# wusize/CLIPSelf

Measured on AMD Instinct MI355X. Metric: images/sec (student+teacher distill step), ViT-B/16 32 crops/img, higher is better.
Workload: dtype bf16; 1 GPU; EVA02-CLIP-B-16 CLIPSelf image-patches step, 64 images x 32 crops per GPU, 224^2 (BASELINE configs[1]); global_batch=64, crops_per_image=32, image_size=224, parallelism=dp1, teacher_chunk=2048, teacher_last_block=cls_query_only, teacher_schedule=one_batch_ahead_on_side_stream

## Files before the change

### clipself_amd/csrc/attention.hip

```cpp
#include <type_traits>
#include "cs_common.h"
#include <cstdlib>

namespace {

constexpr int HD = 64;
constexpr float LOG2E = 1.4426950408889634f;


#define Z16 (f32x16{0.f, 0.f, 0.f, 0.f, 0.f, 0.f, 0.f, 0.f, 0.f, 0.f, 0.f, 0.f, 0.f, 0.f, 0.f, 0.f})
__device__ __forceinline__ f32x16 zero16() {
    f32x16 z;
#pragma unroll
    for (int e = 0; e < 16; ++e) z[e] = 0.f;
    return z;
}

__device__ __forceinline__ void rope8(U128& v, const float* __restrict__ cs, const float* __restrict__ sn) {
    const float4 c0 = *(const float4*)cs, c1 = *(const float4*)(cs + 4);
    const float4 s0 = *(const float4*)sn, s1 = *(const float4*)(sn + 4);
    const float c[8] = {c0.x, c0.y, c0.z, c0.w, c1.x, c1.y, c1.z, c1.w};
    const float s[8] = {s0.x, s0.y, s0.z, s0.w, s1.x, s1.y, s1.z, s1.w};
#pragma unroll
    for (int j = 0; j < 4; ++j) {
// ... 89 lines not shown
__device__ __forceinline__ void stage_rows(const __bf16* __restrict__ src, size_t rowbase, int ld, int coloff, int tok0, int Ntok,
                                           const float* cos_t, const float* sin_t, char* tile, __bf16* tile_t, int ldt, int tid) {
    for (int idx = tid; idx < CHK * 8; idx += 512) {
        const int r = idx >> 3, c = idx & 7, tok = tok0 + r;
        U128 v;
        if (tok < Ntok) {
            v.u = *(const uint4*)(src + (rowbase + tok) * ld + coloff + c * 8);
            if (ROPE && tok > 0) rope8(v, cos_t + (size_t)(tok - 1) * HD + c * 8, sin_t + (size_t)(tok - 1) * HD + c * 8);
        } else {
            v.u = make_uint4(0, 0, 0, 0);
        }
        if (tile) *(uint4*)(tile + r * 128 + ((c ^ (r & 7)) << 4)) = v.u;
        if (WITH_T) {
#pragma unroll
            for (int e = 0; e < 8; ++e) tile_t[(c * 8 + e) * ldt + r] = v.e[e];
        }
    }
}

__device__ __forceinline__ bf16x8 lds_frag(const char* tile, int row, int ks, int hf) {
    return *(const bf16x8*)(tile + row * 128 + ((((ks << 1) + hf) ^ (row & 7)) << 4));
}

constexpr int VT_LD = 264;

__device__ __forceinline__ int k_off(int r, int c) { return ((r >> 1) << 8) + (((((r & 1) << 3) | c) ^ ((r >> 1) & 15)) << 4); }

typedef short s16x4v __attribute__((ext_vector_type(4)));

__device__ __forceinline__ int tr_lane_off(int rr, int d0, int lane) {
    const int li = lane & 15, g1 = (lane >> 4) & 1;
    const int col = d0 + 16 * g1 + 4 * (li & 3);
    return k_off(rr + (li >> 2), col >> 3) + ((col >> 2) & 1) * 8;
}
__device__ __forceinline__ bf16x8 tr_join2(s16x4v lo, s16x4v hi) {
    typedef short s16x8v __attribute__((ext_vector_type(8)));
    const s16x8v v = __builtin_shufflevector(lo, hi, 0, 1, 2, 3, 4, 5, 6, 7);
    return __builtin_bit_cast(bf16x8, v);
}
__device__ __forceinline__ s16x4v tr_read4(const char* addr) {
    return __builtin_amdgcn_ds_read_tr16_b64_v4i16((__attribute__((address_space(3))) s16x4v*)addr);
}

template <int CHK, int NT = 512>
struct RowRegs {
    static constexpr int ITEMS = (CHK * 8 + NT - 1) / NT;
    uint4 v[ITEMS];
    __device__ __forceinline__ void load(const __bf16* __restrict__ src, size_t rowbase, int ld, int coloff, int tok0, int Ntok, int tid) {
#pragma unroll
        for (int it = 0; it < ITEMS; ++it) {
            const int idx = min(tid + it * NT, CHK * 8 - 1), tok = min(tok0 + (idx >> 3), Ntok - 1);
            v[it] = *(const uint4*)(src + (rowbase + tok) * ld + coloff + (idx & 7) * 8);
        }
    }
    template <bool ROPE, bool ZPAD = false>
    __device__ __forceinline__ void store(char* tile, const float* rt, int g, float inv_g, int tok0, int Ntok, int tid) {
#pragma unroll
        for (int it = 0; it < ITEMS; ++it) {
            const int idx = tid + it * NT, r = idx >> 3, c = idx & 7, tok = tok0 + r;
            if (idx < CHK * 8) {
                U128 t;
                t.u = v[it];
                if (ROPE && tok > 0 && tok < Ntok) rope8_lds(t, rt, g, inv_g, tok, c);
                if (ZPAD && tok >= Ntok) t.u = make_uint4(0, 0, 0, 0);
                *(uint4*)(tile + k_off(r, c)) = t.u;
            }
        }
    }
};

__device__ __forceinline__ bf16x8 pack8_swapped(const f32x16& a, int c2) {
    union { bf16x2 h; unsigned u; } x0, x1, y0, y1;
    x0.h[0] = f2bf(a[c2 * 8 + 0]); x0.h[1] = f2bf(a[c2 * 8 + 1]);
    x1.h[0] = f2bf(a[c2 * 8 + 2]); x1.h[1] = f2bf(a[c2 * 8 + 3]);
    y0.h[0] = f2bf(a[c2 * 8 + 4]); y0.h[1] = f2bf(a[c2 * 8 + 5]);
    y1.h[0] = f2bf(a[c2 * 8 + 6]); y1.h[1] = f2bf(a[c2 * 8 + 7]);
    const auto r0 = __builtin_amdgcn_permlane32_swap(x0.u, y0.u, false, false);
    const auto r1 = __builtin_amdgcn_permlane32_swap(x1.u, y1.u, false, false);
    union { unsigned u[4]; bf16x8 v; } out;
    out.u[0] = r0[0]; out.u[1] = r1[0]; out.u[2] = r0[1]; out.u[3] = r1[1];
    return out.v;
}

__device__ __forceinline__ void load_q_frags(const AttnArgs& p, const float* rt, size_t rowbase, int qc, int h, int hf, bf16x8 (&qf)[4]) {
    U128 t[4];
#pragma unroll
    for (int ks = 0; ks < 4; ++ks) t[ks].u = *(const uint4*)(p.qkv + (rowbase + qc) * p.ldqkv + h * HD + ks * 16 + hf * 8);
#pragma unroll
    for (int ks = 0; ks < 4; ++ks) {
        if (qc > 0) rope8_lds(t[ks], rt, p.grid, p.inv_grid, qc, ks * 2 + hf);
        qf[ks] = t[ks].h;
    }
}

template <int CH, bool TAIL, bool VROW = false>
__device__ __forceinline__ void attend_chunk(const char* Kl, const __bf16* Vt, const bf16x8 (&qf)[4], int key0, int Ntok, float sl2,
                                             int lane, bool first, float& m, float& l, f32x16 (&o)[2], int t0 = 0) {
    const int hf = lane >> 5, l31 = lane & 31;
    const int k_base = (l31 >> 1) << 8, par8 = (l31 & 1) << 3, sw = l31 >> 1;
    f32x16 s[CH];
#pragma unroll
    for (int t = 0; t < CH; ++t) {
        s[t] = zero16();
#pragma unroll
        for (int ks = 0; ks < 4; ++ks) {
            const bf16x8 kfrag = *(const bf16x8*)(Kl + (t0 + t) * (16 * 256) + k_base + (((par8 | (ks * 2 + hf)) ^ sw) << 4));
            s[t] = __builtin_amdgcn_mfma_f32_32x32x16_bf16(kfrag, qf[ks], s[t], 0, 0, 0);
        }
    }
    const int rem_last = Ntok - key0 - (CH - 1) * 32;
    const bool short_tail = TAIL && rem_last <= 8;
    float mx = -INFINITY;
#pragma unroll
    for (int t = 0; t < CH; ++t) {
        if (TAIL && t == CH - 1 && short_tail) {
#pragma unroll
            for (int e = 0; e < 4; ++e) {
                if (e + 4 * hf >= rem_last) s[t][e] = -INFINITY;
                mx = fmaxf(mx, s[t][e]);
            }
            continue;
        }
        if ((!TAIL || t == CH - 1) && key0 + t * 32 + 32 > Ntok) {
#pragma unroll
            for (int e = 0; e < 16; ++e)
                if (key0 + t * 32 + mfma32_row(e, lane) >= Ntok) s[t][e] = -INFINITY;
        }
#pragma unroll
        for (int e = 0; e < 16; ++e) mx = fmaxf(mx, s[t][e]);
    }
    mx = fmaxf(mx, __shfl_xor(mx, 32, 64));
    const float m_new = fmaxf(m, mx);
    const float alpha = exp2f((m - m_new) * sl2);
    const float msc = m_new * sl2;
    float rs = 0.f;
#pragma unroll
    for (int t = 0; t < CH; ++t) {
        if (TAIL && t == CH - 1 && short_tail) {
#pragma unroll
            for (int e = 0; e < 4; ++e) {
                const float pv = __builtin_amdgcn_exp2f(s[t][e] * sl2 - msc);
                s[t][e] = pv;
                rs += pv;
            }
#pragma unroll
            for (int e = 4; e < 8; ++e) s[t][e] = 0.f;
            continue;
        }
#pragma unroll
        for (int e = 0; e < 16; ++e) {
            const float pv = __builtin_amdgcn_exp2f(s[t][e] * sl2 - msc);
            s[t][e] = pv;
            rs += pv;
        }
    }
    rs += __shfl_xor(rs, 32, 64);
    l = l * alpha + rs;
    m = m_new;
    if (!first) {
#pragma unroll
        for (int e = 0; e < 16; ++e) { o[0][e] *= alpha; o[1][e] *= alpha; }
    }
#pragma unroll
    for (int t = 0; t < CH; ++t)
#pragma unroll
        for (int c2 = 0; c2 < 2; ++c2) {
            if (TAIL && t == CH - 1 && c2 == 1 && rem_last <= 16) continue;
            const bf16x8 pb = pack8_swapped(s[t], c2);
            const int kb = (t0 + t) * 4 + c2 * 2 + hf;
#pragma unroll
            for (int dt = 0; dt < 2; ++dt) {
                bf16x8 vfrag;
                if constexpr (VROW) {
                    const char* Vl = (const char*)Vt + (t0 + t) * (16 * 256);
                    vfrag = tr_join2(tr_read4(Vl + tr_lane_off(c2 * 16 + 8 * hf, dt * 32, lane)), tr_read4(Vl + tr_lane_off(c2 * 16 + 8 * hf + 4, dt * 32, lane)));
                } else {
                    const int d = dt * 32 + l31;
                    vfrag = *(const bf16x8*)(Vt + d * VT_LD + ((kb ^ ((d >> 3) & 7)) << 3));
                }
                o[dt] = __builtin_amdgcn_mfma_f32_32x32x16_bf16(vfrag, pb, o[dt], 0, 0, 0);
            }
        }
}

__device__ __forceinline__ void store_o(const AttnArgs& p, size_t rowbase, int q, int h, int bh, int hf, float m, float l, const f32x16 (&o)[2]) {
    const float inv = 1.f / l;
    __bf16* orow = p.out + (rowbase + q) * p.ldo + h * HD;
    float ps = 0.f, pq = 0.f;
#pragma unroll
    for (int dt = 0; dt < 2; ++dt) {
        U64 t[4];
#pragma unroll
        for (int g4 = 0; g4 < 4; ++g4)
#pragma unroll
            for (int i = 0; i < 4; ++i) {
                t[g4].e[i] = f2bf(o[dt][g4 * 4 + i] * inv);
                const float r = bf2f(t[g4].e[i]);
                ps += r;
                pq += r * r;
            }
#pragma unroll
        for (int a = 0; a < 4; a += 2) {
            const auto r0 = __builtin_amdgcn_permlane32_swap(t[a].u.x, t[a + 1].u.x, false, false);
            const auto r1 = __builtin_amdgcn_permlane32_swap(t[a].u.y, t[a + 1].u.y, false, false);
            if (!ATT_ABL(p, 4)) *(uint4*)(orow + dt * 32 + (a + hf) * 8) = make_uint4(r0[0], r1[0], r0[1], r1[1]);
        }
    }
    if (p.lse_out && hf == 0) p.lse_out[(size_t)bh * p.Ntok + q] = m * p.scale + logf(l);
    if (p.stats_part) {
        ps += __shfl_xor(ps, 32);
        pq += __shfl_xor(pq, 32);
        if (hf == 0) *(float2*)(p.stats_part + ((size_t)h * p.Mtot + rowbase + q) * 2) = make_float2(ps, pq);
    }
}

template <int CH, int CH1>
__global__ __launch_bounds__(512, 2) void attn_fwd2_kernel(AttnArgs p) {
    constexpr int CHK = CH * 32;
    extern __shared__ __attribute__((aligned(16))) char smem[];
    char* Kl = smem;
    char* Vl = smem + CHK * 128;
    float* rt = (float*)(smem + 2 * CHK * 128);

    const int tid = threadIdx.x, lane = tid & 63, wave = tid >> 6, hf = lane >> 5, l31 = lane & 31;
    const RowBlock rb = map_block(p, 8);
    const int bh = rb.bh, b = bh / p.H, h = bh - b * p.H;
    const int C = p.H * HD;
    const size_t rowbase = (size_t)b * p.Ntok;
    const float sl2 = p.scale * LOG2E;
    const int q0 = (rb.tile0 + wave) * 32, q = q0 + l31, qc = min(q, p.Ntok - 1);
    const bool active = wave < rb.nt && q0 < p.Ntok;
    RowRegs<CHK> kr, vr;
    kr.load(p.qkv, rowbase, p.ldqkv, C + h * HD, 0, p.Ntok, tid);
    vr.load(p.qkv, rowbase, p.ldqkv, 2 * C + h * HD, 0, p.Ntok, tid);
    load_rope_tables<512>(rt, p.cos_t, p.sin_t, p.grid, tid);
    __syncthreads();
    bf16x8 qf[4];
    load_q_frags(p, rt, rowbase, qc, h, hf, qf);
    float m = -INFINITY, l = 0.f;
    f32x16 o[2] = {zero16(), zero16()};
    for (int key0 = 0; key0 < p.Ntok; key0 += CHK) {
        if (key0) __syncthreads();
        kr.template store<true>(Kl, rt, p.grid, p.inv_grid, key0, p.Ntok, tid);
        vr.template store<false>(Vl, rt, p.grid, p.inv_grid, key0, p.Ntok, tid);
        __syncthreads();
        if (key0 + CHK < p.Ntok) {
            kr.load(p.qkv, rowbase, p.ldqkv, C + h * HD, key0 + CHK, p.Ntok, tid);
            vr.load(p.qkv, rowbase, p.ldqkv, 2 * C + h * HD, key0 + CHK, p.Ntok, tid);
        }
        if (!active) continue;
        attend_chunk<CH1, false, true>(Kl, (const __bf16*)Vl, qf, key0, p.Ntok, sl2, lane, key0 == 0, m, l, o, 0);
        if (key0 + CH1 * 32 < p.Ntok)
            attend_chunk<CH - CH1, false, true>(Kl, (const __bf16*)Vl, qf, key0 + CH1 * 32, p.Ntok, sl2, lane, false, m, l, o, CH1);
    }
    if (active && q < p.Ntok) store_o(p, rowbase, q, h, bh, hf, m, l, o);
}

template <bool TAIL>
__global__ __launch_bounds__(512, 4) void attn_fwd8_kernel(AttnArgs p) {
    constexpr int CH = 7, CHK = CH * 32, NT = 512;
    extern __shared__ __attribute__((aligned(16))) char smem[];
    char* Kl = smem;
    __bf16* Vt = (__bf16*)(smem + CHK * 128);
    float* rt = (float*)(smem + CHK * 128 + HD * VT_LD * 2);
    const int tid = threadIdx.x, lane = tid & 63, wave = tid >> 6, hf = lane >> 5, l31 = lane & 31;
    const int bh = blockIdx.y, b = bh / p.H, h = bh - b * p.H;
    const int C = p.H * HD;
    const size_t rowbase = (size_t)b * p.Ntok;
    const float sl2 = p.scale * LOG2E;
    const int last = p.Ntok - 1;
    float tab[4];
    {
        const int i = min(tid, p.grid * 32 - 1), r = i >> 5, d = i & 31;
        tab[0] = p.cos_t[(size_t)(r * p.grid) * HD + d];
        tab[1] = p.sin_t[(size_t)(r * p.grid) * HD + d];
        tab[2] = p.cos_t[(size_t)r * HD + 32 + d];
        tab[3] = p.sin_t[(size_t)r * HD + 32 + d];
    }
    __builtin_amdgcn_sched_barrier(0);
    constexpr int KI = (CHK * 8 + NT - 1) / NT;
    U128 kr[KI], vin[8], qraw[4];
    const __bf16* kbase = p.qkv + C + h * HD;
    const __bf16* vbase = p.qkv + 2 * C + h * HD;
    const int vkb = min(tid, CHK - 1) >> 3, vc = tid & 7;
#pragma unroll
    for (int it = 0; it < KI; ++it) {
        const int idx = min(tid + it * NT, CHK * 8 - 1), tok = min(idx >> 3, last);
        kr[it].u = *(const uint4*)(kbase + (rowbase + tok) * p.ldqkv + (idx & 7) * 8);
    }
#pragma unroll
    for (int i = 0; i < 8; ++i) {
        const int tok = min(vkb * 8 + i, last);
        vin[i].u = *(const uint4*)(vbase + (rowbase + tok) * p.ldqkv + vc * 8);
    }
    const int q0 = wave * 32, q = q0 + l31, qc = min(q, last);
#pragma unroll
    for (int ks = 0; ks < 4; ++ks) qraw[ks].u = *(const uint4*)(p.qkv + (rowbase + qc) * p.ldqkv + h * HD + ks * 16 + hf * 8);
    if (tid < p.grid * 32) {
        rt[tid] = tab[0];
        rt[(p.grid << 5) + tid] = tab[1];
        rt[(2 * p.grid << 5) + tid] = tab[2];
        rt[(3 * p.grid << 5) + tid] = tab[3];
    }
    __syncthreads();
#pragma unroll
    for (int it = 0; it < KI; ++it) {
        const int idx = tid + it * NT, r = idx >> 3, c = idx & 7;
        if (idx < CHK * 8) {
            if (r > 0 && r < p.Ntok && !ATT_ABL(p, 2)) rope8_lds(kr[it], rt, p.grid, p.inv_grid, r, c);
            *(uint4*)(Kl + k_off(r, c)) = kr[it].u;
        }
    }
    if (tid < CHK) {
        const int pos = (vkb ^ vc) * 8;
#pragma unroll
        for (int j = 0; j < 8; ++j) {
            U128 o;
#pragma unroll
            for (int i = 0; i < 8; ++i) o.e[i] = vin[i].e[j];
            *(uint4*)(Vt + (vc * 8 + j) * VT_LD + pos) = o.u;
        }
    }
    __syncthreads();
    if (q0 >= p.Ntok) return;
    bf16x8 qf[4];
#pragma unroll
    for (int ks = 0; ks < 4; ++ks) {
        if (qc > 0 && !ATT_ABL(p, 2)) rope8_lds(qraw[ks], rt, p.grid, p.inv_grid, qc, ks * 2 + hf);
        qf[ks] = qraw[ks].h;
    }
    float m = -INFINITY, l = 0.f;
    f32x16 o[2] = {zero16(), zero16()};
    if (ATT_ABL(p, 1)) { l = 1.f; m = 0.f; o[0][0] = bf2f(qf[0][0]); }
    else if (TAIL) {
        attend_chunk<3, false>(Kl, Vt, qf, 0, p.Ntok, sl2, lane, true, m, l, o, 0);
        attend_chunk<3, false>(Kl, Vt, qf, 96, p.Ntok, sl2, lane, false, m, l, o, 3);
        attend_chunk<1, true>(Kl, Vt, qf, 192, p.Ntok, sl2, lane, false, m, l, o, 6);
    } else {
        attend_chunk<3, false>(Kl, Vt, qf, 0, p.Ntok, sl2, lane, true, m, l, o, 0);
        if (p.Ntok > 96) attend_chunk<3, false>(Kl, Vt, qf, 96, p.Ntok, sl2, lane, false, m, l, o, 3);
        if (p.Ntok > 192) attend_chunk<1, false>(Kl, Vt, qf, 192, p.Ntok, sl2, lane, false, m, l, o, 6);
    }
    if (q < p.Ntok) store_o(p, rowbase, q, h, bh, hf, m, l, o);
}

__global__ __launch_bounds__(256) void attn_bwd_prep_kernel(const __bf16* __restrict__ o, const __bf16* __restrict__ dout, float* __restrict__ dsum,
                                                            int B, int Ntok, int H, int ldo) {
    const long idx = (long)blockIdx.x * blockDim.x + threadIdx.x;
    const long total = (long)B * Ntok * H * 8;
    float s = 0.f;
    long row = 0; int h = 0;
    const bool ok = idx < total;
    if (ok) {
        const int c = (int)(idx & 7);
        h = (int)((idx >> 3) % H);
        row = (idx >> 3) / H;
        U128 a, g;
        a.u = *(const uint4*)(o + row * ldo + h * HD + c * 8);
        g.u = *(const uint4*)(dout + row * ldo + h * HD + c * 8);
#pragma unroll
        for (int e = 0; e < 8; ++e) s += bf2f(a.e[e]) * bf2f(g.e[e]);
    }
    s += __shfl_xor(s, 1, 64);
    s += __shfl_xor(s, 2, 64);
    s += __shfl_xor(s, 4, 64);
    if (ok && (idx & 7) == 0) {
        const long b = row / Ntok, n = row - b * Ntok;
        dsum[((size_t)b * H + h) * Ntok + n] = s;
    }
}

__global__ __launch_bounds__(256) void rope_qk_kernel(const __bf16* __restrict__ qkv, const float* __restrict__ cos_t, const float* __restrict__ sin_t,
                                                      __bf16* __restrict__ out, long rows, int Ntok, int C, int ldqkv) {
    const long idx = (long)blockIdx.x * blockDim.x + threadIdx.x;
    const int cpr = C >> 2;
    if (idx >= rows * cpr) return;
    const long row = idx / cpr;
    const int c = (int)(idx - row * cpr), col = c * 8, tok = (int)(row % Ntok);
    U128 v;
    v.u = *(const uint4*)(qkv + row * ldqkv + col);
    if (tok > 0) rope8(v, cos_t + (size_t)(tok - 1) * HD + (col & 63), sin_t + (size_t)(tok - 1) * HD + (col & 63));
    *(uint4*)(out + row * (2 * C) + col) = v.u;
}

__device__ __forceinline__ void store_grad_tile(const f32x16 (&g)[2], __bf16* dst, bool rope, const float* cs, const float* sn, int hf) {
#pragma unroll
    for (int dt = 0; dt < 2; ++dt)
#pragma unroll
        for (int g4 = 0; g4 < 4; ++g4) {
            const int d = dt * 32 + g4 * 8 + hf * 4;
            float v[4] = {g[dt][g4 * 4], g[dt][g4 * 4 + 1], g[dt][g4 * 4 + 2], g[dt][g4 * 4 + 3]};
            if (rope) {
                const float4 c = *(const float4*)(cs + d), s = *(const float4*)(sn + d);
                const float a0 = __builtin_fmaf(v[0], c.x, v[1] * s.y), a1 = __builtin_fmaf(v[1], c.y, -(v[0] * s.x));
                const float a2 = __builtin_fmaf(v[2], c.z, v[3] * s.w), a3 = __builtin_fmaf(v[3], c.w, -(v[2] * s.z));
                v[0] = a0; v[1] = a1; v[2] = a2; v[3] = a3;
            }
            U64 t;
#pragma unroll
            for (int i = 0; i < 4; ++i) t.e[i] = f2bf(v[i]);
            *(uint2*)(dst + d) = t.u;
        }
}

template <int CH>
__global__ __launch_bounds__(512) void attn_bwd_dq_kernel(AttnArgs p) {
    constexpr int CHK = CH * 32, VLD = CHK + 4;
    extern __shared__ __attribute__((aligned(16))) char smem[];
    char* Kl = smem;
    char* Vl = smem + CHK * 128;
    __bf16* Kt = (__bf16*)(smem + 2 * CHK * 128);
// ... 412 lines not shown
#pragma unroll
        for (int j = 0; j < 8; ++j) qf[h][j] = bf2f(t.e[j]);
    }
    const float sl2 = scale * LOG2E;
    for (int key = kg; key < Ntok; key += 32) {
        U128 kk[HG];
#pragma unroll
        for (int h = 0; h < HG; ++h) kk[h].u = *(const uint4*)(kbase + (size_t)key * ldkv + h * HD);
        if (key > 0 && cos_t) {
            const float* cs = cos_t + (size_t)(key - 1) * HD + c * 8;
            const float* sn = sin_t + (size_t)(key - 1) * HD + c * 8;
#pragma unroll
            for (int h = 0; h < HG; ++h) rope8(kk[h], cs, sn);
        }
#pragma unroll
        for (int h = 0; h < HG; ++h) {
            float dot = 0.f;
#pragma unroll
            for (int j = 0; j < 8; ++j) dot += qf[h][j] * bf2f(kk[h].e[j]);
            dot += __shfl_xor(dot, 1);
            dot += __shfl_xor(dot, 2);
            dot += __shfl_xor(dot, 4);
            if (c == 0) sm[h * Npad + key] = (arow && !arow[key]) ? -INFINITY : dot * sl2;
        }
    }
    __syncthreads();
    for (int h = wave; h < HG; h += 4) {
        float* row = sm + h * Npad;
        float mx = -INFINITY;
        for (int key = lane; key < Ntok; key += 64) mx = fmaxf(mx, row[key]);
        mx = wave_max(mx);
        if (mx == -INFINITY) mx = 0.f;
        float sum = 0.f;
        for (int key = lane; key < Ntok; key += 64) {
            const float e = __builtin_amdgcn_exp2f(row[key] - mx);
            sum += e;
            row[key] = bf2f(f2bf(e));
        }
        sum = wave_sum(sum);
        if (lane == 0) rsum[h] = sum > 0.f ? sum : 1.f;
    }
    __syncthreads();
    float acc[HG][8];
#pragma unroll
    for (int h = 0; h < HG; ++h)
#pragma unroll
        for (int j = 0; j < 8; ++j) acc[h][j] = 0.f;
    for (int key = kg; key < Ntok; key += 32) {
        U128 vv[HG];
#pragma unroll
        for (int h = 0; h < HG; ++h) vv[h].u = *(const uint4*)(vbase + (size_t)key * ldkv + h * HD);
#pragma unroll
        for (int h = 0; h < HG; ++h) {
            const float pk = sm[h * Npad + key];
#pragma unroll
            for (int j = 0; j < 8; ++j) acc[h][j] += pk * bf2f(vv[h].e[j]);
        }
    }
#pragma unroll
    for (int h = 0; h < HG; ++h)
#pragma unroll
        for (int j = 0; j < 8; ++j) {
            float v = acc[h][j];
            v += __shfl_xor(v, 8);
            v += __shfl_xor(v, 16);
            v += __shfl_xor(v, 32);
            if (lane < 8) part[wave * (HG * HD) + h * HD + c * 8 + j] = v;
        }
    __syncthreads();
    for (int o = tid; o < HG * HD; o += 256) {
        const float v = (part[o] + part[HG * HD + o]) + (part[2 * HG * HD + o] + part[3 * HG * HD + o]);
        out[(size_t)b * ldo + h0 * HD + o] = f2bf(v / rsum[o / HD]);
    }
}

}

static int attn_fwd_impl(const void* qkv, const float* cos_t, const float* sin_t, void* out, float* lse, float* stats_part, int B, int Ntok,
                         int H, int ldqkv, int ldo, float scale, hipStream_t stream) {
    if (check_common("cs_attn_fwd", B, Ntok, H, ldqkv, ldo)) return -1;
    AttnArgs a{};
    a.qkv = (const __bf16*)qkv; a.cos_t = cos_t; a.sin_t = sin_t; a.out = (__bf16*)out; a.lse_out = lse;
    a.stats_part = stats_part; a.Mtot = (long)B * Ntok;
    int g = (int)(sqrtf((float)(Ntok - 1)) + 0.5f);
    CS_CHECK_ARG(g * g == Ntok - 1, "cs_attn_fwd: Ntok - 1 = %d is not a square token grid (the RoPE tables are read separably)", Ntok - 1);
    a.grid = g; a.inv_grid = 1.f / (float)g;
#ifdef CS_ABLATION_SWITCHES
    static const int dbg_env = getenv("CS_ATTN_DBG") ? atoi(getenv("CS_ATTN_DBG")) : 0;
    a.dbg = dbg_env;
#else
    a.dbg = 0;
#endif
    a.Ntok = Ntok; a.H = H; a.ldqkv = ldqkv; a.ldo = ldo; a.scale = scale;
    constexpr int CH = 7;
    const size_t lds = (size_t)CH * 32 * 128 + (size_t)HD * VT_LD * 2 + (size_t)4 * g * 32 * sizeof(float);
    CS_CHECK_ARG(lds <= 160 * 1024, "cs_attn_fwd: token grid %d too large for the LDS RoPE tables", g);
    if (Ntok <= CH * 32) {
        static bool once = (set_lds(attn_fwd8_kernel<false>, 160 * 1024), set_lds(attn_fwd8_kernel<true>, 160 * 1024), true);
        (void)once;
        if (Ntok > (CH - 1) * 32) hipLaunchKernelGGL((attn_fwd8_kernel<true>), dim3(1, B * H), dim3(512), lds, stream, a);
        else hipLaunchKernelGGL((attn_fwd8_kernel<false>), dim3(1, B * H), dim3(512), lds, stream, a);
    } else {
        static bool once = (set_lds(attn_fwd2_kernel<CH, 4>, 160 * 1024), true);
        (void)once;
        const size_t lds2 = (size_t)2 * CH * 32 * 128 + (size_t)4 * g * 32 * sizeof(float);
        dim3 grid2;
        set_schedule(a, B, Ntok, H, grid2);
        hipLaunchKernelGGL((attn_fwd2_kernel<CH, 4>), grid2, dim3(512), lds2, stream, a);
    }
    CS_LAUNCH_CHECK();
    return 0;
}

extern "C" int cs_attn_fwd(const void* qkv, const float* cos_t, const float* sin_t, void* out, float* lse, int B, int Ntok, int H,
                           int ldqkv, int ldo, float scale, hipStream_t stream) {
    return attn_fwd_impl(qkv, cos_t, sin_t, out, lse, nullptr, B, Ntok, H, ldqkv, ldo, scale, stream);
}

extern "C" int cs_attn_fwd_stats(const void* qkv, const float* cos_t, const float* sin_t, void* out, float* lse, float* stats_part, int B,
                                 int Ntok, int H, int ldqkv, int ldo, float scale, hipStream_t stream) {
    CS_CHECK_ARG(stats_part != nullptr && ((uintptr_t)stats_part % 8) == 0, "cs_attn_fwd_stats: stats_part must be an 8-byte aligned buffer");
    return attn_fwd_impl(qkv, cos_t, sin_t, out, lse, stats_part, B, Ntok, H, ldqkv, ldo, scale, stream);
}

static size_t bwd_dsum_bytes(int B, int Ntok, int H) { return (((size_t)B * H * Ntok * sizeof(float)) + 255) & ~(size_t)255; }
extern "C" size_t cs_attn_bwd_workspace(int B, int Ntok, int H) {
    return bwd_dsum_bytes(B, Ntok, H) + (Ntok > 7 * 32 ? (size_t)B * Ntok * 2 * H * HD * sizeof(__bf16) : 0);
}

extern "C" int cs_attn_bwd(const void* qkv, const void* o, const void* dout, const float* lse, const float* cos_t, const float* sin_t,
                           void* dqkv, void* workspace, int B, int Ntok, int H, int ldqkv, int ldo, float scale, hipStream_t stream) {
    if (check_common("cs_attn_bwd", B, Ntok, H, ldqkv, ldo)) return -1;
    CS_CHECK_ARG(workspace != nullptr && lse != nullptr, "cs_attn_bwd: workspace and lse are required");
    float* dsum = (float*)workspace;
    const long total = (long)B * Ntok * H * 8;
    hipLaunchKernelGGL(attn_bwd_prep_kernel, dim3((int)((total + 255) / 256)), dim3(256), 0, stream, (const __bf16*)o, (const __bf16*)dout, dsum, B, Ntok, H, ldo);
    CS_LAUNCH_CHECK();
    AttnArgs a{};
    a.qkv = (const __bf16*)qkv; a.dout = (const __bf16*)dout; a.cos_t = cos_t; a.sin_t = sin_t; a.lse_in = lse; a.dsum = dsum;
    a.out = (__bf16*)dqkv; a.Ntok = Ntok; a.H = H; a.ldqkv = ldqkv; a.ldo = ldo; a.scale = scale;
    dim3 grid((Ntok + 255) / 256, B * H), block(512);
    constexpr int CH = 7;
    constexpr int CHK = CH * 32, VLD = CHK + 4;
    const int g = (int)(sqrtf((float)(Ntok - 1)) + 0.5f);
    const bool v1 = getenv("CS_ATTN_BWD_V1") != nullptr || g * g != Ntok - 1;
    if (!v1) {
        a.grid = g; a.inv_grid = 1.f / (float)g;
        const size_t rope = (size_t)4 * g * 32 * sizeof(float);
        const size_t lds_dq = (size_t)2 * CHK * 128 + rope, lds_dkv = (size_t)2 * CHK * 128 + (size_t)2 * CHK * sizeof(float) + rope;
        CS_CHECK_ARG(lds_dkv <= 160 * 1024, "cs_attn_bwd: token grid %d too large for the LDS RoPE tables", g);
        static bool once = (set_lds(attn_bwd_dq2_kernel<CH, true>, 160 * 1024), set_lds(attn_bwd_dkv2_kernel<CH, true>, 160 * 1024),
                            set_lds(attn_bwd_dq2_kernel<CH, false, true>, 160 * 1024), set_lds(attn_bwd_dkv2_kernel<CH, false, true>, 160 * 1024), true);
        (void)once;
        if (Ntok <= CHK) {
            hipLaunchKernelGGL((attn_bwd_dq2_kernel<CH, true>), grid, block, lds_dq, stream, a);
            CS_LAUNCH_CHECK();
            hipLaunchKernelGGL((attn_bwd_dkv2_kernel<CH, true>), grid, block, lds_dkv, stream, a);
        } else {
            dim3 grid2;
            set_schedule(a, B, Ntok, H, grid2);
            const int C2 = 2 * H * HD;
            __bf16* qk = (__bf16*)((char*)workspace + bwd_dsum_bytes(B, Ntok, H));
            const long items = (long)B * Ntok * (C2 / 8);
            hipLaunchKernelGGL(rope_qk_kernel, dim3((unsigned)((items + 255) / 256)), dim3(256), 0, stream, (const __bf16*)qkv, cos_t, sin_t, qk,
                               (long)B * Ntok, Ntok, H * HD, ldqkv);
            CS_LAUNCH_CHECK();
            a.qk = qk; a.ldqk = C2;
            hipLaunchKernelGGL((attn_bwd_dq2_kernel<CH, false, true>), grid2, block, lds_dq - rope, stream, a);
            CS_LAUNCH_CHECK();
            hipLaunchKernelGGL((attn_bwd_dkv2_kernel<CH, false, true>), grid2, block, lds_dkv - rope, stream, a);
        }
        CS_LAUNCH_CHECK();
        return 0;
    }
    const size_t lds_dq = (size_t)2 * CHK * 128 + (size_t)HD * VLD * 2;
    const size_t lds_dkv = (size_t)2 * CHK * 128 + (size_t)2 * HD * VLD * 2 + (size_t)2 * CHK * sizeof(float);
    static bool once = (set_lds(attn_bwd_dq_kernel<CH>, lds_dq), set_lds(attn_bwd_dkv_kernel<CH>, lds_dkv), true);
    (void)once;
    hipLaunchKernelGGL((attn_bwd_dq_kernel<CH>), grid, block, lds_dq, stream, a);
    CS_LAUNCH_CHECK();
    hipLaunchKernelGGL((attn_bwd_dkv_kernel<CH>), grid, block, lds_dkv, stream, a);
    CS_LAUNCH_CHECK();
    return 0;
}

static int attn_cls_launch(const void* q, const void* kv, const float* cos_t, const float* sin_t, void* out, int rows, int Ntok, int H,
                           int ldq, int ldkv, int ldo, float scale, int qpb, const unsigned char* allow, hipStream_t stream) {
    const int HG = H % 6 == 0 ? 6 : (H % 4 == 0 ? 4 : (H % 3 == 0 ? 3 : (H % 2 == 0 ? 2 : 1)));
    const size_t lds = ((size_t)HG * ((Ntok + 3) & ~3) + 8 + (size_t)4 * HG * HD) * sizeof(float);
    CS_CHECK_ARG(lds <= 160 * 1024, "cs_attn_cls_fwd: Ntok=%d too large", Ntok);
    const dim3 grid(rows, H / HG), block(256);
// ... 39 lines not shown
```

### clipself_amd/csrc/gemm.hip

```cpp
#include "gemm_common.h"
#include <hip/amd_detail/amd_hip_unsafe_atomics.h>

namespace {

constexpr int EP_LD = 68;
constexpr int EP_BYTES = 32 * EP_LD * 4;

template <int FM, int BN>
__device__ __forceinline__ void epilogue_swiglu(const GemmArgs& p, const f32x16 (&acc)[FM][2], char* slab_bytes, char* rowst_bytes, int lane,
                                                int row0, int tn, int wn) {
    const int l31 = lane & 31, hf = lane >> 5;
    uint32_t* slab = (uint32_t*)slab_bytes;
    const int hbase = tn * (BN / 2) + wn * 32;
    const int hl = hbase + l31;
    float b1 = 0.f, b2 = 0.f;
    if (p.bias && hl < p.group) { b1 = p.bias[hl]; b2 = p.bias[p.group + hl]; }
    const bool ln = p.ln_mean != nullptr;
    float c1 = 0.f, c2 = 0.f;
    float2* rowst = (float2*)rowst_bytes;
    if (ln) {
        if (hl < p.group) { c1 = p.ln_colsum[hl]; c2 = p.ln_colsum[p.group + hl]; }
        for (int r = lane; r < FM * 32; r += 64) {
            const int row = min(row0 + r, p.M - 1);
            const float rs = p.ln_rstd[row];
// ... 551 lines not shown
    double c1, c2, c3;
    const int sp[4] = {0, best_split(128, 128, 2, 1.3, c1), best_split(256, 128, 1, 0.95, c2), best_split(256, 256, 1, 1.4, c3)};
    int cfg = force_cfg;
    if (cfg == 0) {
        if (a.M < 256 || ncols < 256) c3 = 1e30;
        if (a.M < 256 || ncols < 128) c2 = 1e30;
        cfg = (c3 <= c2 && c3 <= c1) ? 3 : (c2 <= c1 ? 2 : 1);
        if (cfg == 3 && use_glds) cfg = 11;
    }
    if (cfg != 1 && cfg != 2 && cfg != 3 && cfg != 7 && cfg != 9 && cfg != 11) {
        cs_set_error("cs_gemm_nt: schedule %d does not exist (flags bits 4-7: 0 heuristic, 1, 2, 3, 7, 9, 11)", cfg);
        return -1;
    }
    const int ns = sp[cfg >= 7 ? 3 : cfg];
    a.ktiles_per_split = (ktiles + ns - 1) / ns;
    if (cfg == 11) {
        if (use_glds && ns == 1) {
            const int rc = cs_gemm_stream_launch(a, EPI, a.reserve, stream);
            if (rc <= 0) return rc;
        }
        cfg = 9;
    }
    switch (cfg) {
        case 9:
            if constexpr (epi_is_bf16(EPI) || EPI == EPI_SWIGLU_BF16 || EPI == EPI_RESID_F32 || EPI == EPI_RESID_LN_F32) {
                if (use_glds && ns == 1) return launch_persist<EPI>(a, stream);
            }
            return launch_cfg<EPI, 256, 256, 2, 4, 32>(a, ns, use_glds, stream);
        case 7: return launch_cfg<EPI, 256, 256, 2, 4, 32>(a, ns, use_glds, stream);
        case 3: return launch_cfg<EPI, 256, 256, 2, 4, 2>(a, ns, use_glds, stream);
        case 2: return launch_cfg<EPI, 256, 128, 4, 2, 2>(a, ns, use_glds, stream);
        default: return launch_cfg<EPI, 128, 128, 2, 2, 2>(a, ns, use_glds, stream);
    }
}

}

static int gemm_nt_impl(const void* A, const void* B, void* C, const float* bias, const float* extra, const float* ln_mean,
                        const float* ln_rstd, const float* ln_colsum, float* stats_part, void* xb_out, int ldxb, int M, int N, int K, int lda,
                        int ldb, int ldc, int epi, int splits, int group, int flags, hipStream_t stream) {
    CS_CHECK_ARG(M > 0 && N > 0 && K > 0, "cs_gemm_nt: empty problem M=%d N=%d K=%d", M, N, K);
    CS_CHECK_ARG(K % BK == 0, "cs_gemm_nt: K=%d must be a multiple of %d", K, BK);
    CS_CHECK_ARG((lda % 8) == 0 && (ldb % 8) == 0, "cs_gemm_nt: lda/ldb must be multiples of 8 (16-byte rows)");
    CS_CHECK_ARG(((uintptr_t)A % 16) == 0 && ((uintptr_t)B % 16) == 0, "cs_gemm_nt: operands must be 16-byte aligned");
    CS_CHECK_ARG(splits == 1 || epi == EPI_ATOMIC_F32, "cs_gemm_nt: split-K (splits != 1; <= 0 = automatic) needs the atomic epilogue");
    CS_CHECK_ARG((epi == EPI_SWIGLU_BF16 ? group : N) % 4 == 0 && ldc % 4 == 0 && ((uintptr_t)C % 16) == 0,
                 "cs_gemm_nt: N, ldc must be multiples of 4 and C 16-byte aligned (vector epilogue)");
    CS_CHECK_ARG(bias == nullptr || ((uintptr_t)bias % 16) == 0, "cs_gemm_nt: bias must be 16-byte aligned");
    GemmArgs a;
    a.A = (const __bf16*)A; a.B = (const __bf16*)B; a.C = C; a.bias = bias; a.extra = extra;
    a.M = M; a.N = N; a.K = K; a.lda = lda; a.ldb = ldb; a.ldc = ldc; a.group = group;
    a.split_stride = 0;
    a.ln_mean = ln_mean; a.ln_rstd = ln_rstd; a.ln_colsum = ln_colsum; a.stats_part = stats_part;
    a.xb_out = (__bf16*)xb_out; a.ldxb = ldxb;
    a.tiles_m = a.tiles_n = 0;
    a.gm = ((flags >> 8) & 15) ? ((flags >> 8) & 15) : 8;
    a.rm = (flags >> 16) & 3;
    a.nsplit = 1;
    if (a.rm == 1 || a.rm == 2) {
        const int f = (flags >> 8) & 15;
        CS_CHECK_ARG(f == 0 || f == 1 || f == 2 || f == 4 || f == 8, "cs_gemm_nt: B-stationary raster needs 1, 2, 4 or 8 N parts (got %d)", f);
        int parts = f;
        if (parts == 0) for (parts = 1; parts < 8 && (double)N * K * 2 / parts > 3.3e6; parts *= 2) {}
        a.nsplit = parts;
        a.gm = 8;
    }
    if (epi == EPI_SWIGLU_BF16) CS_CHECK_ARG(group > 0 && N == 2 * group, "cs_gemm_nt: swiglu epilogue needs N == 2*group");
    if (epi == EPI_RESID_LN_F32) CS_CHECK_ARG(ln_mean && ln_rstd && ln_colsum && ((uintptr_t)ln_colsum % 16) == 0, "cs_gemm_nt_ln: epilogue 6 needs mean, rstd and a 16-byte aligned column-sum vector");
    CS_CHECK_ARG(stats_part == nullptr || epi == EPI_SWIGLU_BF16 || epi == EPI_RESID_F32 || epi == EPI_RESID_LN_F32,
                 "cs_gemm_nt_ln: statistics output exists for the SwiGLU and residual epilogues");
    CS_CHECK_ARG(xb_out == nullptr || ((epi == EPI_RESID_F32 || epi == EPI_RESID_LN_F32) && ldxb % 4 == 0 && ((uintptr_t)xb_out % 8) == 0),
                 "cs_gemm_nt_ln: the bf16 copy exists for the residual epilogues (8-byte aligned, ldxb %% 4 == 0)");
    CS_CHECK_ARG((ln_mean == nullptr) == (ln_rstd == nullptr) && (ln_mean == nullptr || ln_colsum != nullptr),
                 "cs_gemm_nt_ln: mean, rstd and the column-sum vector come together");
    CS_CHECK_ARG(ln_mean == nullptr || epi_is_bf16(epi) || epi == EPI_SWIGLU_BF16 || epi == EPI_RESID_LN_F32,
                 "cs_gemm_nt_ln: a folded LayerNorm exists for epilogues 0, 3, 6, 7 and 8");
    if (epi == EPI_PATCH_F32 || epi == EPI_RESID_F32 || epi == EPI_RESID_LN_F32) CS_CHECK_ARG(extra != nullptr && ((uintptr_t)extra % 16) == 0, "cs_gemm_nt: epilogue %d needs 16-byte aligned extra", epi);
    if (epi == EPI_PATCH_F32) CS_CHECK_ARG(group > 0, "cs_gemm_nt: patch epilogue needs group");
    a.ktiles_per_split = K / BK;
    const int glds = (flags & 1) ? 0 : 1;
    const int force = (flags >> 4) & 15;
    a.dbg = (flags >> 12) & 15;
    a.reserve = (flags >> 20) & 255;
    switch (epi) {
        case EPI_BF16: return launch<EPI_BF16>(a, splits, glds, force, stream);
        case EPI_F32: return launch<EPI_F32>(a, splits, glds, force, stream);
        case EPI_RESID_F32: return launch<EPI_RESID_F32>(a, splits, glds, force, stream);
        case EPI_SWIGLU_BF16: return launch<EPI_SWIGLU_BF16>(a, splits, glds, force, stream);
        case EPI_ATOMIC_F32: return launch<EPI_ATOMIC_F32>(a, splits, glds, force, stream);
        case EPI_PATCH_F32: return launch<EPI_PATCH_F32>(a, splits, glds, force, stream);
        case EPI_RESID_LN_F32: return launch<EPI_RESID_LN_F32>(a, splits, glds, force, stream);
        case EPI_GELU_BF16: return launch<EPI_GELU_BF16>(a, splits, glds, force, stream);
        case EPI_QGELU_BF16: return launch<EPI_QGELU_BF16>(a, splits, glds, force, stream);
    }
    cs_set_error("cs_gemm_nt: unknown epilogue %d", epi);
    return -1;
}

static int gemm_nt_split_f32(const void* A, const void* B, float* C, int M, int N, int K, int lda, int ldb, int cfg, int splits, hipStream_t stream) {
    CS_CHECK_ARG(M > 0 && N > 0 && K > 0 && K % BK == 0 && N % 4 == 0, "cs_gemm_wgrad: bad problem M=%d N=%d K=%d", M, N, K);
    CS_CHECK_ARG((lda % 8) == 0 && (ldb % 8) == 0 && ((uintptr_t)A % 16) == 0 && ((uintptr_t)B % 16) == 0, "cs_gemm_wgrad: operands must be 16-byte aligned rows");
    GemmArgs a;
    a.A = (const __bf16*)A; a.B = (const __bf16*)B; a.C = C; a.bias = nullptr; a.extra = nullptr;
    a.M = M; a.N = N; a.K = K; a.lda = lda; a.ldb = ldb; a.ldc = N; a.group = 0;
    a.split_stride = (long)M * N;
    a.ln_mean = a.ln_rstd = a.ln_colsum = nullptr; a.stats_part = nullptr; a.xb_out = nullptr; a.ldxb = 0;
    a.tiles_m = a.tiles_n = 0; a.gm = 8; a.dbg = 0; a.rm = 0; a.nsplit = 1; a.reserve = 0;
    a.ktiles_per_split = K / BK;
    return launch<EPI_F32>(a, splits, 1, cfg, stream);
}

extern "C" int cs_gemm_nt(const void* A, const void* B, void* C, const float* bias, const float* extra, int M, int N, int K,
                          int lda, int ldb, int ldc, int epi, int splits, int group, int flags, hipStream_t stream) {
    CS_CHECK_ARG(epi != EPI_RESID_LN_F32, "cs_gemm_nt: epilogue 6 (folded LayerNorm) is reached through cs_gemm_nt_ln");
    return gemm_nt_impl(A, B, C, bias, extra, nullptr, nullptr, nullptr, nullptr, nullptr, 0, M, N, K, lda, ldb, ldc, epi, splits, group, flags, stream);
}

extern "C" int cs_gemm_nt_ln(const void* A, const void* B, void* C, const float* bias, const float* extra, const float* ln_mean,
                             const float* ln_rstd, const float* ln_colsum, float* stats_part, void* xb_out, int ldxb, int M, int N, int K,
                             int lda, int ldb, int ldc, int epi, int splits, int group, int flags, hipStream_t stream) {
    return gemm_nt_impl(A, B, C, bias, extra, ln_mean, ln_rstd, ln_colsum, stats_part, xb_out, ldxb, M, N, K, lda, ldb, ldc, epi, splits, group,
                        flags, stream);
}


namespace {

__global__ __launch_bounds__(256) void splitk_reduce_kernel(const float* __restrict__ ws, int splits, long stride, float* __restrict__ dst,
                                                            int M, int N, int ldc) {
    const long i = (long)blockIdx.x * 256 + threadIdx.x;
    const int n4 = N >> 2;
    if (i >= (long)M * n4) return;
    const int row = (int)(i / n4), c = (int)(i - (long)row * n4) * 4;
    float4 acc = *(const float4*)(ws + (size_t)row * N + c);
    for (int s = 1; s < splits; ++s) {
        const float4 t = *(const float4*)(ws + (size_t)s * stride + (size_t)row * N + c);
        acc.x += t.x; acc.y += t.y; acc.z += t.z; acc.w += t.w;
    }
    float4* d = (float4*)(dst + (size_t)row * ldc + c);
    const float4 o = *d;
    *d = make_float4(o.x + acc.x, o.y + acc.y, o.z + acc.z, o.w + acc.w);
}

typedef __attribute__((ext_vector_type(4))) short s16x4;

__device__ __forceinline__ int tn_swz(int tok) { return (tok & 3) << 1; }
typedef short s16x8 __attribute__((ext_vector_type(8)));
struct TrFrag { s16x4 lo, hi; };
__device__ __forceinline__ void tr_read(TrFrag& f, const char* tile, int tok, int colbyte) {
    const int a0 = tok * 512 + (colbyte ^ (tn_swz(tok) << 5)), a1 = (tok + 4) * 512 + (colbyte ^ (tn_swz(tok + 4) << 5));
    const unsigned base = (unsigned)(uintptr_t)(__attribute__((address_space(3))) const char*)tile;
    asm volatile("ds_read_b64_tr_b16 %0, %1" : "=v"(f.lo) : "v"(base + (unsigned)a0));
    asm volatile("ds_read_b64_tr_b16 %0, %1" : "=v"(f.hi) : "v"(base + (unsigned)a1));
}
__device__ __forceinline__ bf16x8 tr_join(const TrFrag& f) {
    const s16x8 v = __builtin_shufflevector(f.lo, f.hi, 0, 1, 2, 3, 4, 5, 6, 7);
    return __builtin_bit_cast(bf16x8, v);
}

template <bool RAGGED>
__global__ __launch_bounds__(512) void gemm_tn_kernel(GemmArgs p) {
    constexpr int BM = 256, BN = 256, WN = 4, TM = 128, TN = 64, FM = 4, FN = 2;
    constexpr int T_BYTES = 64 * 512;
    extern __shared__ __attribute__((aligned(16))) char smem[];
    const int tid = threadIdx.x, lane = tid & 63;
    const int wave = __builtin_amdgcn_readfirstlane(tid >> 6);
// ... 193 lines not shown
```

### clipself_amd/csrc/gemm_common.h

```cpp
#pragma once
#include "cs_common.h"
#include <cstdio>
#include <cstdlib>
#include <type_traits>

#ifdef CS_ABLATION_SWITCHES
#define CS_ABL(p, bit) ((p).dbg & (bit))
#else
#define CS_ABL(p, bit) false
#endif

constexpr int BK = 64;
enum Epi { EPI_BF16 = 0, EPI_F32 = 1, EPI_RESID_F32 = 2, EPI_SWIGLU_BF16 = 3, EPI_ATOMIC_F32 = 4, EPI_PATCH_F32 = 5, EPI_RESID_LN_F32 = 6,
           EPI_GELU_BF16 = 7, EPI_QGELU_BF16 = 8 };
constexpr bool epi_is_bf16(int e) { return e == EPI_BF16 || e == EPI_GELU_BF16 || e == EPI_QGELU_BF16; }
constexpr int epi_act(int e) { return e == EPI_GELU_BF16 ? 1 : (e == EPI_QGELU_BF16 ? 2 : 0); }

struct GemmArgs {
    const __bf16* A;
    const __bf16* B;
    void* C;
    const float* bias;
    const float* extra;
    int M, N, K;
    int lda, ldb, ldc;
    int tiles_m, tiles_n;
    int ktiles_per_split;
    long split_stride;
    int group;
    int gm;
    int rm;
    int nsplit;
    const float* ln_mean;
    const float* ln_rstd;
    const float* ln_colsum;
    float* stats_part;
    __bf16* xb_out;
    int ldxb;
    unsigned short* lo = nullptr;
    int split = 0;
    int reserve;
    int dbg;
};

inline int cs_num_cus() {
    static const int n = [] {
        int dev = 0, v = 0;
        if (hipGetDevice(&dev) != hipSuccess || hipDeviceGetAttribute(&v, hipDeviceAttributeMultiprocessorCount, dev) != hipSuccess || v <= 0) v = 256;
        return v;
    }();
    return n;
}
inline long cs_persistent_cap(int reserve) {
    const int n = cs_num_cus();
    return n - (reserve > 0 && reserve <= n - 8 ? reserve : 0);
}

int cs_gemm_stream_launch(GemmArgs a, int epi, int reserve, hipStream_t stream);
int cs_gemm_stream_launch_f8(GemmArgs a, int epi, int reserve, hipStream_t stream);

namespace {

__device__ __forceinline__ void lane_source(int rg, int lane, int& tile_row, int& chunk) {
    const int lrow = rg * 4 + (lane >> 4);
    const int c16 = (lane & 15) ^ (lrow & 15);
    tile_row = lrow * 2 + (c16 >> 3);
    chunk = c16 & 7;
}

template <int NINSTR, bool GLDS, int AUX = 0>
__device__ __forceinline__ void stage_tile(const __bf16* __restrict__ src, int ld, int k0, char* lds_tile, int rg0, int lane,
                                           const int (&grow)[NINSTR], const int (&gchunk)[NINSTR]) {
#pragma unroll
    for (int i = 0; i < NINSTR; ++i) {
        const __bf16* g = src + (size_t)grow[i] * ld + k0 + gchunk[i] * 8;
        char* dst = lds_tile + (rg0 + i) * 1024;
        if (GLDS) {
            __builtin_amdgcn_global_load_lds((const __attribute__((address_space(1))) void*)g,
                                             (__attribute__((address_space(3))) void*)dst, 16, 0, AUX);
        } else {
            *(uint4*)(dst + lane * 16) = *(const uint4*)g;
        }
    }
}

__device__ __forceinline__ void tile_of_id(const GemmArgs& p, int bid, int nwg, int& tm, int& tn);
__device__ __forceinline__ void tile_of_block(const GemmArgs& p, int& tm, int& tn) { tile_of_id(p, blockIdx.x, gridDim.x, tm, tn); }
__device__ __forceinline__ void tile_of_id(const GemmArgs& p, int bid, int nwg, int& tm, int& tn) {
    const int xcd = bid & 7, q = nwg >> 3, r = nwg & 7;
    const int swz = (xcd < r ? xcd * (q + 1) : r * (q + 1) + (xcd - r) * q) + (bid >> 3);
    const int per_group = p.gm * p.tiles_n;
    const int grp = swz / per_group, rem = swz - grp * per_group;
    const int rows = min(p.gm, p.tiles_m - grp * p.gm);
    tn = rem / rows;
    tm = grp * p.gm + (rem - tn * rows);
}

__device__ __forceinline__ bool tile_bstat(const GemmArgs& p, int xcd, int lt, int& tm, int& tn) {
    const int NP = p.nsplit, MP = 8 / NP;
    const int np = xcd % NP, mp = xcd / NP;
    const int n_lo = np * p.tiles_n / NP, nn = (np + 1) * p.tiles_n / NP - n_lo;
    const int m_lo = mp * p.tiles_m / MP, mm = (mp + 1) * p.tiles_m / MP - m_lo;
    if (lt >= mm * nn) return false;
    const int q = lt / nn;
    tm = m_lo + q;
    tn = n_lo + (lt - q * nn);
    return true;
}

template <int EPI, int BM, int BN, int NW, int A_INSTR, int B_INSTR>
__device__ __forceinline__ void source_rows(const GemmArgs& p, int wave, int lane, int m0, int n0, int tn, int (&arow)[A_INSTR],
                                            int (&achk)[A_INSTR], int (&brow)[B_INSTR], int (&bchk)[B_INSTR]) {
#pragma unroll
    for (int i = 0; i < A_INSTR; ++i) {
        int tr;
        lane_source(wave * A_INSTR + i, lane, tr, achk[i]);
        arow[i] = min(m0 + tr, p.M - 1);
    }
#pragma unroll
    for (int i = 0; i < B_INSTR; ++i) {
        int tr;
        lane_source(wave * B_INSTR + i, lane, tr, bchk[i]);
        if (EPI == EPI_SWIGLU_BF16) {
            const int hidx = tn * (BN / 2) + (tr >> 6) * 32 + (tr & 31);
            brow[i] = ((tr >> 5) & 1) * p.group + min(hidx, p.group - 1);
        } else {
            brow[i] = min(n0 + tr, p.N - 1);
        }
    }
}

}
```

### clipself_amd/csrc/gemm_stream.hip

```cpp
#include <vector>
#include <cstdio>
#include "gemm_common.h"

namespace {

typedef __attribute__((ext_vector_type(2))) unsigned u32x2;
typedef __attribute__((ext_vector_type(4))) unsigned u32x4;

constexpr unsigned OOB = 0xfffffff0u;

__device__ __forceinline__ float lane_bcast(int src_lane_x4, float v) {
    return __int_as_float(__builtin_amdgcn_ds_bpermute(src_lane_x4, __float_as_int(v)));
}
__device__ __forceinline__ unsigned pack2(float a, float b) {
    union { bf16x2 v; unsigned u; } pk;
    pk.v[0] = f2bf(a);
    pk.v[1] = f2bf(b);
    return pk.u;
}
__device__ __forceinline__ void swap32(unsigned& x, unsigned& y) {
    const u32x2 r = __builtin_amdgcn_permlane32_swap(x, y, false, false);
    x = r[0];
    y = r[1];
}
// ... 25 lines not shown
    return v;
}

struct EpiOps {
    float mean[4], rstd[4];
    float cb, cc;
};

template <bool LN, bool AUX, int CP, int FM = 4>
__device__ __forceinline__ void epi_swiglu(const GemmArgs& p, const f32x16 (&acc)[FM][2], int lane, int row0, int tn, int wn, const EpiOps& eo) {
    const int l31 = lane & 31, hf = lane >> 5;
    const int hbase = tn * 128 + wn * 32;
    const bool colok = hbase < p.group;
    float nm[FM], rs[FM];
#pragma unroll
    for (int i = 0; i < FM; ++i) {
        rs[i] = LN ? eo.rstd[i] : 1.f;
        nm[i] = LN ? -eo.rstd[i] * eo.mean[i] : 0.f;
    }
    unsigned pk[FM][4][2];
    float ssum[4] = {0.f, 0.f, 0.f, 0.f}, ssq[4] = {0.f, 0.f, 0.f, 0.f};
    const int sl0 = hf << 4;
#pragma unroll
    for (int q = 0; q < 4; ++q) {
        float hv[FM][4];
#pragma unroll
        for (int r = 0; r < 4; ++r) {
            const int e = q * 4 + r;
            const int sl = sl0 + ((8 * q + r) << 2);
            const float b1 = lane_bcast(sl, eo.cb), b2 = lane_bcast(sl + 128, eo.cb);
            float c1 = 0.f, c2 = 0.f;
            if (LN) { c1 = lane_bcast(sl, eo.cc); c2 = lane_bcast(sl + 128, eo.cc); }
#pragma unroll
            for (int i = 0; i < FM; ++i) {
                float u = acc[i][0][e], v = acc[i][1][e];
                if (LN) {
                    u = fmaf(rs[i], u, fmaf(nm[i], c1, b1));
                    v = fmaf(rs[i], v, fmaf(nm[i], c2, b2));
                } else {
                    u += b1;
                    v += b2;
                }
                hv[i][r] = silu_mul(u, v);
            }
        }
#pragma unroll
        for (int i = 0; i < FM; ++i) {
            pk[i][q][0] = pack2(hv[i][0], hv[i][1]);
            pk[i][q][1] = pack2(hv[i][2], hv[i][3]);
            if (AUX) {
#pragma unroll
                for (int d = 0; d < 2; ++d) {
                    ssum[i] = dot2_bf16(pk[i][q][d], 0x3f803f80u, ssum[i]);
                    ssq[i] = dot2_bf16(pk[i][q][d], pk[i][q][d], ssq[i]);
                }
            }
        }
    }
    const __amdgpu_buffer_rsrc_t rc = make_rsrc((const __bf16*)p.C + (size_t)row0 * p.ldc + hbase);
#pragma unroll
    for (int i = 0; i < FM; ++i) {
        const bool ok = colok && row0 + i * 32 + l31 < p.M && !CS_ABL(p, 8);
        const unsigned rowoff = (unsigned)((i * 32 + l31) * p.ldc + 8 * hf) * 2u;
#pragma unroll
        for (int pr = 0; pr < 2; ++pr) {
            unsigned x0 = pk[i][2 * pr][0], x1 = pk[i][2 * pr][1], y0 = pk[i][2 * pr + 1][0], y1 = pk[i][2 * pr + 1][1];
            swap32(x0, y0);
            swap32(x1, y1);
            store16<CP>(u32x4{x0, x1, y0, y1}, rc, ok ? rowoff + 32u * pr : OOB);
        }
    }
    if (AUX) {
        const size_t slice = (size_t)tn * 4 + wn;
        const __amdgpu_buffer_rsrc_t rst = make_rsrc(p.stats_part + (slice * p.M + row0) * 2);
#pragma unroll
        for (int i = 0; i < FM; ++i) {
            const float s = both_halves(ssum[i]), q2 = both_halves(ssq[i]);
            const bool ok = colok && hf == 0 && row0 + i * 32 + l31 < p.M;
            store8<CP>(u32x2{__float_as_uint(s), __float_as_uint(q2)}, rst, ok ? (unsigned)(i * 32 + l31) * 8u : OOB);
        }
    }
}

template <int ACT, bool LN, int CP, bool F8 = false, int FM = 4>
__device__ __forceinline__ void epi_bf16(const GemmArgs& p, const f32x16 (&acc)[FM][2], int lane, int row0, int colw, const EpiOps& eo) {
    const int l31 = lane & 31, hf = lane >> 5;
    float nm[FM], rs[FM];
#pragma unroll
    for (int i = 0; i < FM; ++i) {
        rs[i] = (LN || F8) ? eo.rstd[i] : 1.f;
        nm[i] = LN ? -eo.rstd[i] * eo.mean[i] : 0.f;
    }
    const __amdgpu_buffer_rsrc_t rc = make_rsrc((const __bf16*)p.C + (size_t)row0 * p.ldc + colw);
    const int sl0 = hf << 4;
    unsigned pk[2][FM][4][2];
#pragma unroll
    for (int j = 0; j < 2; ++j) {
#pragma unroll
        for (int q = 0; q < 4; ++q) {
            float ov[FM][4];
#pragma unroll
            for (int r = 0; r < 4; ++r) {
                const int sl = sl0 + ((j * 32 + 8 * q + r) << 2);
                const float b = lane_bcast(sl, eo.cb);
                const float c = (LN || F8) ? lane_bcast(sl, eo.cc) : 0.f;
#pragma unroll
                for (int i = 0; i < FM; ++i) {
                    const float a = acc[i][j][q * 4 + r];
                    ov[i][r] = activate_s<ACT>(F8 ? fmaf(rs[i] * c, a, b) : LN ? fmaf(rs[i], a, fmaf(nm[i], c, b)) : a + b);
                }
            }
#pragma unroll
            for (int i = 0; i < FM; ++i) {
                pk[j][i][q][0] = pack2(ov[i][0], ov[i][1]);
                pk[j][i][q][1] = pack2(ov[i][2], ov[i][3]);
            }
        }
    }
#pragma unroll
    for (int i = 0; i < FM; ++i) {
        const bool rowok = row0 + i * 32 + l31 < p.M && !CS_ABL(p, 8);
#pragma unroll
        for (int j = 0; j < 2; ++j) {
            const bool ok = rowok && colw + j * 32 < p.N;
            const unsigned rowoff = (unsigned)((i * 32 + l31) * p.ldc + j * 32 + 8 * hf) * 2u;
#pragma unroll
            for (int pr = 0; pr < 2; ++pr) {
                unsigned x0 = pk[j][i][2 * pr][0], x1 = pk[j][i][2 * pr][1], y0 = pk[j][i][2 * pr + 1][0], y1 = pk[j][i][2 * pr + 1][1];
                swap32(x0, y0);
                swap32(x1, y1);
                store16<CP>(u32x4{x0, x1, y0, y1}, rc, ok ? rowoff + 32u * pr : OOB);
            }
        }
    }
}


template <int ACT, bool LN, int CP>
__device__ __forceinline__ void epi_bf16_slab(const GemmArgs& p, const f32x16 (&acc)[4][2], int lane, int row0, int colw, const EpiOps& eo, char* slab) {
    const int l31 = lane & 31, hf = lane >> 5;
    float nm[4], rs[4];
#pragma unroll
    for (int i = 0; i < 4; ++i) {
        rs[i] = LN ? eo.rstd[i] : 1.f;
        nm[i] = LN ? -eo.rstd[i] * eo.mean[i] : 0.f;
    }
    const __amdgpu_buffer_rsrc_t rc = make_rsrc((const __bf16*)p.C + (size_t)row0 * p.ldc + colw);
    const int sl0 = hf << 4;
    const int piece = lane & 7, col = colw + piece * 8;
#pragma unroll
    for (int half = 0; half < 2; ++half) {
#pragma unroll
        for (int j = 0; j < 2; ++j)
#pragma unroll
            for (int q = 0; q < 4; ++q) {
                float bq[4], cq[4];
#pragma unroll
                for (int r = 0; r < 4; ++r) {
                    const int sl = sl0 + ((j * 32 + 8 * q + r) << 2);
                    bq[r] = lane_bcast(sl, eo.cb);
                    cq[r] = LN ? lane_bcast(sl, eo.cc) : 0.f;
                }
#pragma unroll
                for (int ii = 0; ii < 2; ++ii) {
                    const int i = half * 2 + ii, lrow = ii * 32 + l31;
                    float ov[4];
#pragma unroll
                    for (int r = 0; r < 4; ++r) {
                        const float a = acc[i][j][q * 4 + r];
                        ov[r] = activate_s<ACT>(LN ? fmaf(rs[i], a, fmaf(nm[i], cq[r], bq[r])) : a + bq[r]);
                    }
                    const int s8 = (j * 8 + 2 * q + hf) ^ ((lrow & 7) << 1);
                    *(uint2*)(slab + lrow * 128 + s8 * 8) = make_uint2(pack2(ov[0], ov[1]), pack2(ov[2], ov[3]));
                }
            }
#pragma unroll
        for (int k = 0; k < 8; ++k) {
            const int lrow = (lane >> 3) + 8 * k, rrel = half * 64 + lrow;
            const uint4 w = *(const uint4*)(slab + lrow * 128 + ((piece ^ (lrow & 7)) << 4));
            const bool ok = row0 + rrel < p.M && col < p.N && !CS_ABL(p, 8);
            store16<CP>(u32x4{w.x, w.y, w.z, w.w}, rc, ok ? (unsigned)(rrel * p.ldc + piece * 8) * 2u : OOB);
        }
    }
}

template <bool LN, bool AUX, int CP>
__device__ __forceinline__ void epi_swiglu_slab(const GemmArgs& p, const f32x16 (&acc)[4][2], int lane, int row0, int tn, int wn, const EpiOps& eo,
                                                char* slab) {
    const int l31 = lane & 31, hf = lane >> 5;
    const int hbase = tn * 128 + wn * 32;
    const bool colok = hbase < p.group;
    float nm[4], rs[4];
#pragma unroll
    for (int i = 0; i < 4; ++i) {
        rs[i] = LN ? eo.rstd[i] : 1.f;
        nm[i] = LN ? -eo.rstd[i] * eo.mean[i] : 0.f;
    }
    float ssum[4] = {0.f, 0.f, 0.f, 0.f}, ssq[4] = {0.f, 0.f, 0.f, 0.f};
    const int sl0 = hf << 4;
#pragma unroll
// ... 121 lines not shown
        EPI_TRACE(1 + 3 * i);
        EPI_TRACE_WAIT();
        EPI_TRACE(2 + 3 * i);
        const int sel = lane & 7;
        float st_s = 0.f, st_q = 0.f;
#pragma unroll
        for (int it = 0; it < 4; ++it) {
            const int lrow = rrow + 8 * it, rrel = i * 32 + lrow;
            const bool ok = colok && row0 + rrel < p.M;
            float rs = 1.f, nm = 0.f;
            if (LN || F8) rs = lane_bcast(lrow << 2, rs_row);
            if (LN) nm = lane_bcast(lrow << 2, nm_row);
            f32x4 o[2];
#pragma unroll
            for (int h = 0; h < 2; ++h) {
                const f32x4 sv = *(const f32x4*)(slab + lrow * 256 + (((2 * piece + h) ^ (lrow & 15)) << 4));
                if (LN) {
#pragma unroll
                    for (int t = 0; t < 4; ++t) o[h][t] = xin[it][h][t] + fmaf(rs, sv[t], fmaf(nm, cc4[h][t], cb4[h][t]));
                } else if (F8) {
#pragma unroll
                    for (int t = 0; t < 4; ++t) o[h][t] = xin[it][h][t] + fmaf(rs * cc4[h][t], sv[t], cb4[h][t]);
                } else {
                    o[h] = xin[it][h] + (sv + cb4[h]);
                }
            }
            if constexpr (SPLIT & 2) {
                const unsigned off = ok ? (unsigned)(rrel * p.ldxb + piece * 8) * 2u : OOB;
                unsigned y[8];
#pragma unroll
                for (int t = 0; t < 8; ++t) y[t] = __float_as_uint(o[t >> 2][t & 3]) + 0x8000u;
                store16<CP>(u32x4{__builtin_amdgcn_perm(y[1], y[0], 0x07060302u), __builtin_amdgcn_perm(y[3], y[2], 0x07060302u),
                                  __builtin_amdgcn_perm(y[5], y[4], 0x07060302u), __builtin_amdgcn_perm(y[7], y[6], 0x07060302u)}, rb, off);
                store16<CP>(u32x4{__builtin_amdgcn_perm(y[1], y[0], 0x05040100u), __builtin_amdgcn_perm(y[3], y[2], 0x05040100u),
                                  __builtin_amdgcn_perm(y[5], y[4], 0x05040100u), __builtin_amdgcn_perm(y[7], y[6], 0x05040100u)}, rl, off);
            } else {
                const unsigned off = ok ? (unsigned)(rrel * p.ldc + piece * 8) * 4u : OOB;
                store16<CP>(__builtin_bit_cast(u32x4, o[0]), rc, off);
                store16<CP>(__builtin_bit_cast(u32x4, o[1]), rc, ok ? off + 16u : OOB);
            }
            if (AUX) {
                if constexpr (!(SPLIT & 2))
                    store16<CP>(u32x4{pack2(o[0][0], o[0][1]), pack2(o[0][2], o[0][3]), pack2(o[1][0], o[1][1]), pack2(o[1][2], o[1][3])}, rb,
                                ok ? (unsigned)(rrel * p.ldxb + piece * 8) * 2u : OOB);
                float ps = 0.f, pq = 0.f;
                if (colok) {
#pragma unroll
                    for (int t = 0; t < 8; ++t) { ps += o[t >> 2][t & 3]; pq = fmaf(o[t >> 2][t & 3], o[t >> 2][t & 3], pq); }
                }
                const float a = sum_lanes8(ps), b = sum_lanes8(pq);
                if (sel == it) { st_s = a; st_q = b; }
            }
        }
        if (AUX) {
            const int rrel = i * 32 + rrow + 8 * sel;
            const bool ok = sel < 4 && row0 + rrel < p.M && colw < p.N;
            store8<CP>(u32x2{__float_as_uint(st_s), __float_as_uint(st_q)}, rst, ok ? (unsigned)rrel * 8u : OOB);
        }
        EPI_TRACE(3 + 3 * i);
        __builtin_amdgcn_sched_barrier(0);
    }
}

template <int EPI, bool AUX, bool SLAB, int SPLIT = 0, int FM = 4>
constexpr int epi_stores() {
    if (EPI == EPI_SWIGLU_BF16) return FM * (2 + (AUX ? 1 : 0));
    if (EPI == EPI_RESID_F32) return FM * (8 + (AUX ? ((SPLIT & 2) ? 0 : 4) + 1 : 0));
    return FM * 4;
}

#ifndef CS_DMA_AUX_A
#define CS_DMA_AUX_A 0
#endif
#ifndef CS_DMA_AUX_B
#define CS_DMA_AUX_B 0
#endif
#define CS_VMCNT(N) asm volatile("s_waitcnt vmcnt(%0)" ::"n"(N) : "memory")

inline bool getenv_flag(const char* name) {
    const char* v = getenv(name);
    return v && v[0] && v[0] != '0';
}

template <int EPI, bool LN, bool AUX, bool SLAB, bool F8 = false, int SPLIT = 0, int BMT = 256>
__global__ __launch_bounds__(512) void gemm_stream_kernel(GemmArgs p) {
    static_assert(BMT == 256 || (BMT == 192 && !F8 && SPLIT == 0 && !LN && !AUX), "192-row tiles: the training schedule's plain epilogues");
    static_assert(SPLIT == 0 || (EPI == EPI_RESID_F32 && LN && !F8), "the split stream belongs to the folded-LayerNorm residual epilogue");
    static_assert(SLAB || EPI != EPI_RESID_F32, "the fp32 residual epilogue exists in the slab form only (whole-line traffic)");
    static_assert(!F8 || (!LN && !AUX && (EPI == EPI_BF16 || EPI == EPI_RESID_F32)), "fp8 operands: bf16 and fp32-residual outputs");
    constexpr int ES = F8 ? 1 : 2;
    constexpr int CP = 0;
    constexpr bool SWI = EPI == EPI_SWIGLU_BF16, RES = EPI == EPI_RESID_F32;
    static_assert(SWI || RES || epi_is_bf16(EPI), "register epilogues");
    constexpr int BM = BMT, BN = 256, WN = 4, TM = BM / 2, TN = 64, FM = TM / 32, FN = 2;
    constexpr int A_BYTES = BM * BK * 2, B_BYTES = BN * BK * 2;
    constexpr int NPA = BM / 32;
    constexpr int NM = FM * FN, NR = FM + FN;
    constexpr int S = epi_stores<EPI, AUX, SLAB, SPLIT, FM>() < 55 ? epi_stores<EPI, AUX, SLAB, SPLIT, FM>() : 55;
    extern __shared__ __attribute__((aligned(16))) char smem[];
    const int tid = threadIdx.x, lane = tid & 63;
    const int wave = __builtin_amdgcn_readfirstlane(tid >> 6);
    const int wm = wave / WN, wn = wave - wm * WN;
    const int hf = lane >> 5, l31 = lane & 31;
    char* const b_ring = smem + 3 * A_BYTES;
    const int ntiles = p.tiles_m * p.tiles_n, ktiles = p.K / (F8 ? 128 : BK);
    const int a_base = ((wm * TM + l31) >> 1) << 8, b_base = ((wn * TN + l31) >> 1) << 8;
    const int par8 = (l31 & 1) << 3, sw = l31 >> 1;
    const int G = gridDim.x;
#ifndef CS_NO_DMA_ROLES
    constexpr bool ROLES = !F8;
#else
    constexpr bool ROLES = false;
#endif
    const bool role_a = ROLES && wave >= 4;
#ifndef CS_NO_MID_BARRIER
    constexpr bool MID = ROLES && !SLAB && !F8;
#else
    constexpr bool MID = false;
#endif

    unsigned avoff[ROLES ? 8 : 4], bvoff[ROLES ? 1 : 4];
    const char *a_src = nullptr, *b_src = nullptr;
    int a_tile = blockIdx.x, a_kt = 0, b_tile = blockIdx.x, b_kt = 0;
    auto set_a = [&](int tile) {
        int tm, tn;
        tile_of_id(p, tile, ntiles, tm, tn);
        a_src = (const char*)p.A + (size_t)tm * BM * p.lda * ES;
#pragma unroll
        for (int i = 0; i < (ROLES ? NPA : 4); ++i) {
            int tr, chk;
            lane_source(ROLES ? (wave & 3) * NPA + i : wave * 4 + i, lane, tr, chk);
            avoff[i] = (unsigned)(min(tr, p.M - 1 - tm * BM) * p.lda * ES + chk * 16);
        }
    };
    auto set_b = [&](int tile) {
        int tm, tn;
        tile_of_id(p, tile, ntiles, tm, tn);
        if (SWI) {
            b_src = (const char*)p.B + (size_t)tn * (BN / 2) * p.ldb * ES;
        } else {
            b_src = (const char*)p.B + (size_t)tn * BN * p.ldb * ES;
        }
#pragma unroll
        for (int i = 0; i < (ROLES ? 8 : 4); ++i) {
            int tr, chk;
            lane_source(ROLES ? (wave & 3) * 8 + i : wave * 4 + i, lane, tr, chk);
            int rel;
            if (SWI) {
                const int hrel = (tr >> 6) * 32 + (tr & 31);
                rel = ((tr >> 5) & 1) * p.group + min(hrel, p.group - 1 - tn * (BN / 2));
            } else {
                rel = min(tr, p.N - 1 - tn * BN);
            }
            (ROLES ? avoff : bvoff)[i] = (unsigned)(rel * p.ldb * ES + chk * 16);
        }
    };
    auto adv_a = [&]() {
        if (++a_kt == ktiles) {
            a_kt = 0;
            if (a_tile + G < ntiles) {
                a_tile += G;
                set_a(a_tile);
            }
        }
    };
    auto adv_b = [&]() {
        if (++b_kt == ktiles) {
            b_kt = 0;
// ... 280 lines not shown
                constexpr int SS = S + KEEP > 63 ? 63 - KEEP : S;
                if (after_epi) CS_VMCNT(KEEP + SS);
                else CS_VMCNT(KEEP);
                after_epi = false;
                asm volatile("s_waitcnt lgkmcnt(0)" ::: "memory");
                __builtin_amdgcn_s_barrier();
            }
            {
                const int off = ((par8 | hf) ^ sw) << 4;
#pragma unroll
                for (int x = 0; x < 8; ++x) {
                    if (x < FM) fa[0][x] = *(const bf16x8*)(la_n + x * (16 * 256) + off);
                    else if (x < NR) fb[0][x - FM] = *(const bf16x8*)(lb_n + (x - FM) * (16 * 256) + off);
                    if constexpr (ROLE == 1) ISSUE_RB(x, slot_b2);
                }
            }
            mfmas(1, false);
#pragma unroll
            for (int m = 0; m < NM; ++m) {
                __builtin_amdgcn_sched_group_barrier(0x008, 1, 0);
                if (m < NR) __builtin_amdgcn_sched_group_barrier(0x100, 1, 0);
                if (ROLE == 1 && m < NM - 1) __builtin_amdgcn_sched_group_barrier(0x010, 1, 0);
                if (ROLE == 1 && m == NM - 1) __builtin_amdgcn_sched_group_barrier(0x010, 1 + 8 - NM, 0);
            }
            if (ROLE == 1) adv_b();
            else adv_a();
            curA = nextA;
            gpar ^= 1;
        };
        if constexpr (MID) {
            if (role_a) {
                ktile_mid(std::true_type{}, std::integral_constant<int, 2>{});
                for (int kt = 1; kt < ktiles; ++kt) ktile_mid(std::false_type{}, std::integral_constant<int, 2>{});
            } else {
                ktile_mid(std::true_type{}, std::integral_constant<int, 1>{});
                for (int kt = 1; kt < ktiles; ++kt) ktile_mid(std::false_type{}, std::integral_constant<int, 1>{});
            }
        } else if constexpr (ROLES) {
            if (role_a) {
                ktile(std::true_type{}, std::integral_constant<int, 2>{});
                for (int kt = 1; kt < ktiles; ++kt) ktile(std::false_type{}, std::integral_constant<int, 2>{});
            } else {
                ktile(std::true_type{}, std::integral_constant<int, 1>{});
                for (int kt = 1; kt < ktiles; ++kt) ktile(std::false_type{}, std::integral_constant<int, 1>{});
            }
        } else {
            ktile(std::true_type{}, std::integral_constant<int, 0>{});
            for (int kt = 1; kt < ktiles; ++kt) ktile(std::false_type{}, std::integral_constant<int, 0>{});
        }
        if (CS_ABL(p, 4)) continue;
        after_epi = true;
        int lane_e = lane;
        asm volatile("" : "+v"(lane_e));
        if constexpr (SLAB) {
            asm volatile("s_waitcnt lgkmcnt(0)" ::: "memory");
            __builtin_amdgcn_s_barrier();
            char* const slab = wave >= 4 ? b_ring + (gpar ^ 1) * B_BYTES + (wave - 4) * 8192
                               : (BM == 192 && wave == 3) ? b_ring + 2 * B_BYTES
                                                          : smem + (curA == 0 ? 2 : curA - 1) * A_BYTES + wave * 8192;
            load_epi_ops(lane_e);
#ifndef CS_NO_KERNARG_RELOAD
            constexpr bool RELOAD = RES && LN && AUX;
#else
            constexpr bool RELOAD = false;
#endif
            if constexpr (RELOAD) {
                const __attribute__((address_space(4))) GemmArgs* pk = (const __attribute__((address_space(4))) GemmArgs*)__builtin_amdgcn_kernarg_segment_ptr();
                asm volatile("" : "+s"(pk));
                GemmArgs pe;
                pe.A = pk->A; pe.C = pk->C; pe.bias = pk->bias; pe.extra = pk->extra; pe.M = pk->M; pe.N = pk->N; pe.ldc = pk->ldc;
                pe.ln_colsum = pk->ln_colsum; pe.stats_part = pk->stats_part; pe.xb_out = pk->xb_out; pe.ldxb = pk->ldxb; pe.lo = pk->lo;
                pe.dbg = pk->dbg;
                epi_resid_slab<LN, AUX, CP, F8, SPLIT, FM>(pe, acc, lane_e, row0, colw, tn, wn, eo, slab);
            } else if constexpr (RES) {
                epi_resid_slab<LN, AUX, CP, F8, SPLIT, FM>(p, acc, lane_e, row0, colw, tn, wn, eo, slab);
            } else {
                static_assert(FM == 4, "the slab forms of the bf16 / SwiGLU epilogues exist for 256-row tiles");
                if constexpr (SWI) epi_swiglu_slab<LN, AUX, CP>(p, acc, lane_e, row0, tn, wn, eo, slab);
                else epi_bf16_slab<epi_act(EPI), LN, CP>(p, acc, lane_e, row0, colw, eo, slab);
            }
        } else {
            load_epi_ops(lane_e);
            if constexpr (SWI) epi_swiglu<LN, AUX, CP, FM>(p, acc, lane_e, row0, tn, wn, eo);
            else epi_bf16<epi_act(EPI), LN, CP, F8, FM>(p, acc, lane_e, row0, colw, eo);
        }
    }
    CS_VMCNT(0);
#undef ISSUE_A
#undef ISSUE_B
#undef ISSUE_RA
#undef ISSUE_RB
}

template <int EPI, bool LN, bool AUX, bool SLAB, int BMT = 256>
int launch_stream_v(const GemmArgs& a, unsigned grid, hipStream_t stream) {
    constexpr size_t lds = 160 * 1024;
    static bool once = ((void)hipFuncSetAttribute((const void*)gemm_stream_kernel<EPI, LN, AUX, SLAB, false, 0, BMT>, hipFuncAttributeMaxDynamicSharedMemorySize, (int)lds), true);
    (void)once;
    hipLaunchKernelGGL((gemm_stream_kernel<EPI, LN, AUX, SLAB, false, 0, BMT>), dim3(grid), dim3(512), lds, stream, a);
    CS_LAUNCH_CHECK();
    return 0;
}

template <int EPI, bool LN, bool AUX>
int launch_stream_t(const GemmArgs& a, unsigned grid, hipStream_t stream) {
    if constexpr (EPI == EPI_RESID_F32) return launch_stream_v<EPI, LN, AUX, true>(a, grid, stream);
    else return (a.dbg & 1) ? launch_stream_v<EPI, LN, AUX, true>(a, grid, stream) : launch_stream_v<EPI, LN, AUX, false>(a, grid, stream);
}

template <bool AUX, int SPLIT>
int launch_stream_split(const GemmArgs& a, unsigned grid, hipStream_t stream) {
    constexpr size_t lds = 160 * 1024;
    static bool once = ((void)hipFuncSetAttribute((const void*)gemm_stream_kernel<EPI_RESID_F32, true, AUX, true, false, SPLIT>,
                                                  hipFuncAttributeMaxDynamicSharedMemorySize, (int)lds), true);
    (void)once;
    hipLaunchKernelGGL((gemm_stream_kernel<EPI_RESID_F32, true, AUX, true, false, SPLIT>), dim3(grid), dim3(512), lds, stream, a);
    CS_LAUNCH_CHECK();
    return 0;
}

template <int EPI>
int launch_stream_bf16(const GemmArgs& a, unsigned grid, hipStream_t stream) {
    return a.ln_mean ? launch_stream_t<EPI, true, false>(a, grid, stream) : launch_stream_t<EPI, false, false>(a, grid, stream);
}

template <int EPI, bool SLAB>
int launch_stream_f8(const GemmArgs& a, unsigned grid, hipStream_t stream) {
    constexpr size_t lds = 160 * 1024;
    static bool once = ((void)hipFuncSetAttribute((const void*)gemm_stream_kernel<EPI, false, false, SLAB, true>, hipFuncAttributeMaxDynamicSharedMemorySize, (int)lds), true);
    (void)once;
    hipLaunchKernelGGL((gemm_stream_kernel<EPI, false, false, SLAB, true>), dim3(grid), dim3(512), lds, stream, a);
    CS_LAUNCH_CHECK();
    return 0;
}

}

int cs_gemm_stream_launch_f8(GemmArgs a, int epi, int reserve, hipStream_t stream) {
    a.tiles_m = (a.M + 255) / 256;
    a.tiles_n = (a.N + 255) / 256;
    const long ntiles = (long)a.tiles_m * a.tiles_n;
    const long cap = cs_persistent_cap(reserve);
    const unsigned grid = (unsigned)(ntiles < cap ? ntiles : cap);
    if (epi == EPI_BF16) return launch_stream_f8<EPI_BF16, false>(a, grid, stream);
    return launch_stream_f8<EPI_RESID_F32, true>(a, grid, stream);
}

#ifdef CS_ABLATION_SWITCHES
static int stream_launch_impl(GemmArgs a, int epi, int reserve, hipStream_t stream);
int cs_gemm_stream_launch(GemmArgs a, int epi, int reserve, hipStream_t stream) {
    static const char* path = getenv("CS_GEMM_TRACE");
    static unsigned long long* buf = nullptr;
    constexpr size_t WORDS = 256 * 8 * 16;
    if (path && !buf && hipMalloc((void**)&buf, WORDS * 8) == hipSuccess) {
        (void)hipMemset(buf, 0, WORDS * 8);
        (void)hipMemcpyToSymbol(HIP_SYMBOL(g_epi_trace), &buf, sizeof(buf));
    }
    const int rc = stream_launch_impl(a, epi, reserve, stream);
    if (path && buf && rc == 0 && (epi == EPI_RESID_F32 || epi == EPI_RESID_LN_F32)) {
        (void)hipStreamSynchronize(stream);
        std::vector<unsigned long long> host(WORDS);
        (void)hipMemcpy(host.data(), buf, WORDS * 8, hipMemcpyDeviceToHost);
        if (FILE* f = fopen(path, "wb")) { fwrite(host.data(), 8, WORDS, f); fclose(f); }
    }
    return rc;
}
static int stream_launch_impl(GemmArgs a, int epi, int reserve, hipStream_t stream) {
#else
int cs_gemm_stream_launch(GemmArgs a, int epi, int reserve, hipStream_t stream) {
#endif
    const bool swi = epi == EPI_SWIGLU_BF16, res = epi == EPI_RESID_F32 || epi == EPI_RESID_LN_F32;
    if (!(swi || res || epi == EPI_BF16 || epi == EPI_QGELU_BF16)) return 1;
    if (a.M < 1 || a.K % BK != 0) return 1;
    if (swi ? (a.group % 32 != 0) : (a.N % 32 != 0)) return 1;
    if ((long)a.ldc * 128 * 4 >= 0x70000000L || (long)a.ldxb * 128 * 2 >= 0x70000000L) return 1;
    const bool ln = a.ln_mean != nullptr;
    if ((epi == EPI_RESID_LN_F32) != (res && ln)) return 1;
    bool aux = false;
    if (swi) aux = a.stats_part != nullptr;
    else if (res) {
        if ((a.stats_part != nullptr) != (a.xb_out != nullptr)) return 1;
        aux = a.stats_part != nullptr;
        if (aux && (a.ldxb % 8 != 0 || ((uintptr_t)a.xb_out % 16) != 0)) return 1;
    } else if (a.stats_part || a.xb_out) return 1;
    a.tiles_m = (a.M + 255) / 256;
    a.tiles_n = swi ? (a.group + 127) / 128 : (a.N + 255) / 256;
    long ntiles = (long)a.tiles_m * a.tiles_n;
    const long cap = cs_persistent_cap(reserve);
    unsigned grid = (unsigned)(ntiles < cap ? ntiles : cap);
    if (!ln && !aux && !(a.dbg & 1) && a.M >= 192 && (swi || res || epi == EPI_BF16) && !getenv_flag("CS_NO_BM192")) {
        const long t192 = (long)((a.M + 191) / 192) * a.tiles_n;
        const long c256 = ((ntiles + cap - 1) / cap) * 256, c192 = ((t192 + cap - 1) / cap) * 192;
        if (c192 * 10 < c256 * 9) {
            a.tiles_m = (a.M + 191) / 192;
            ntiles = t192;
            grid = (unsigned)(ntiles < cap ? ntiles : cap);
            if (swi) return launch_stream_v<EPI_SWIGLU_BF16, false, false, false, 192>(a, grid, stream);
            if (res) return launch_stream_v<EPI_RESID_F32, false, false, true, 192>(a, grid, stream);
            return launch_stream_v<EPI_BF16, false, false, false, 192>(a, grid, stream);
        }
    }
    if (swi) {
        if (ln) return aux ? launch_stream_t<EPI_SWIGLU_BF16, true, true>(a, grid, stream) : launch_stream_t<EPI_SWIGLU_BF16, true, false>(a, grid, stream);
        return aux ? launch_stream_t<EPI_SWIGLU_BF16, false, true>(a, grid, stream) : launch_stream_t<EPI_SWIGLU_BF16, false, false>(a, grid, stream);
    }
    if (res) {
        if (ln) return aux ? launch_stream_t<EPI_RESID_F32, true, true>(a, grid, stream) : launch_stream_t<EPI_RESID_F32, true, false>(a, grid, stream);
        if (aux) return 1;
        return launch_stream_t<EPI_RESID_F32, false, false>(a, grid, stream);
    }
    if (epi == EPI_BF16) return launch_stream_bf16<EPI_BF16>(a, grid, stream);
    return launch_stream_bf16<EPI_QGELU_BF16>(a, grid, stream);
}

extern "C" int cs_gemm_nt_ln_split(const void* A, const void* B, const float* bias, const float* ln_mean, const float* ln_rstd,
                                   const float* ln_colsum, const float* x_in, float* x_out, void* hi, void* lo, int ldxb, float* stats_part,
                                   int M, int N, int K, int lda, int ldb, int ldc, int flags, hipStream_t stream) {
    CS_CHECK_ARG(M > 0 && N > 0 && K > 0 && K % BK == 0 && N % 32 == 0, "cs_gemm_nt_ln_split: M=%d N=%d (%% 32) K=%d (%% 64)", M, N, K);
    CS_CHECK_ARG((lda % 8) == 0 && (ldb % 8) == 0 && ((uintptr_t)A % 16) == 0 && ((uintptr_t)B % 16) == 0, "cs_gemm_nt_ln_split: operands must be 16-byte aligned rows");
    CS_CHECK_ARG(ln_mean && ln_rstd && ln_colsum && bias && ((uintptr_t)ln_colsum % 16) == 0 && ((uintptr_t)bias % 16) == 0,
                 "cs_gemm_nt_ln_split: mean, rstd, column sums and bias are required (16-byte aligned vectors)");
    CS_CHECK_ARG(x_in == nullptr || x_out == nullptr, "cs_gemm_nt_ln_split: fp32 in and fp32 out is cs_gemm_nt_ln");
    CS_CHECK_ARG(hi && lo && ((uintptr_t)hi % 16) == 0 && ((uintptr_t)lo % 16) == 0 && ldxb % 8 == 0 && ldxb >= N, "cs_gemm_nt_ln_split: hi / lo planes: 16-byte aligned, ldxb %% 8 == 0");
    CS_CHECK_ARG((x_in == nullptr || (((uintptr_t)x_in % 16) == 0 && ldc % 4 == 0)) && (x_out == nullptr || (((uintptr_t)x_out % 16) == 0 && ldc % 4 == 0)),
                 "cs_gemm_nt_ln_split: the fp32 stream must be 16-byte aligned with ldc %% 4 == 0");
    CS_CHECK_ARG(x_out != nullptr || stats_part != nullptr, "cs_gemm_nt_ln_split: a stream that leaves split leaves with its row statistics");
    CS_CHECK_ARG(x_out == nullptr || stats_part == nullptr, "cs_gemm_nt_ln_split: fp32 out takes no stats_part (hi / lo are only read then; the statistics epilogue would overwrite hi)");
    CS_CHECK_ARG(!(x_in != nullptr && stats_part == nullptr), "cs_gemm_nt_ln_split: fp32 in -> split out needs stats_part");
    CS_CHECK_ARG((long)ldc * 128 * 4 < 0x70000000L && (long)ldxb * 128 * 2 < 0x70000000L, "cs_gemm_nt_ln_split: row stride too large");
    GemmArgs a;
    a.A = (const __bf16*)A; a.B = (const __bf16*)B; a.C = x_out; a.bias = bias; a.extra = x_in;
    a.M = M; a.N = N; a.K = K; a.lda = lda; a.ldb = ldb; a.ldc = ldc; a.group = 0;
    a.ktiles_per_split = K / BK; a.split_stride = 0; a.gm = 8; a.rm = 0; a.nsplit = 1;
    a.ln_mean = ln_mean; a.ln_rstd = ln_rstd; a.ln_colsum = ln_colsum; a.stats_part = stats_part; a.xb_out = (__bf16*)hi; a.ldxb = ldxb;
    a.lo = (unsigned short*)lo;
    a.split = (x_in == nullptr ? 1 : 0) | (x_out == nullptr ? 2 : 0);
    a.reserve = (flags >> 20) & 255;
    a.dbg = (flags >> 12) & 15;
    a.tiles_m = (M + 255) / 256;
    a.tiles_n = (N + 255) / 256;
    const long ntiles = (long)a.tiles_m * a.tiles_n;
    const long cap = cs_persistent_cap(a.reserve);
    const unsigned grid = (unsigned)(ntiles < cap ? ntiles : cap);
    if (a.split == 3) return launch_stream_split<true, 3>(a, grid, stream);
    if (a.split == 2) return launch_stream_split<true, 2>(a, grid, stream);
    return launch_stream_split<false, 1>(a, grid, stream);
}

extern "C" int cs_gemm_nt_f8(const void* A8, const void* B8, void* C, const float* bias, const float* extra, const float* row_scale,
                             const float* col_scale, int M, int N, int K8, int lda, int ldb, int ldc, int epi, int flags, hipStream_t stream) {
    CS_CHECK_ARG(M > 0 && N > 0 && K8 > 0 && K8 % 128 == 0, "cs_gemm_nt_f8: K8=%d must be a positive multiple of 128 (M=%d N=%d)", K8, M, N);
    CS_CHECK_ARG(epi == EPI_BF16 || epi == EPI_RESID_F32, "cs_gemm_nt_f8: epilogue %d (0 = bf16 out, 2 = fp32 residual)", epi);
    CS_CHECK_ARG(N % 32 == 0 && ldc % 4 == 0 && lda >= K8 && ldb >= K8 && lda % 16 == 0 && ldb % 16 == 0,
                 "cs_gemm_nt_f8: N %% 32, ldc %% 4, lda/ldb >= K8 and multiples of 16 bytes");
    CS_CHECK_ARG(((uintptr_t)A8 % 16) == 0 && ((uintptr_t)B8 % 16) == 0 && ((uintptr_t)C % 16) == 0, "cs_gemm_nt_f8: operands must be 16-byte aligned");
    CS_CHECK_ARG(row_scale && col_scale, "cs_gemm_nt_f8: row and column scales are required");
    CS_CHECK_ARG(epi != EPI_RESID_F32 || (extra && ((uintptr_t)extra % 16) == 0), "cs_gemm_nt_f8: epilogue 2 needs 16-byte aligned extra");
    CS_CHECK_ARG((long)ldc * 128 * 4 < 0x70000000L, "cs_gemm_nt_f8: ldc too large");
    GemmArgs a;
    a.A = (const __bf16*)A8; a.B = (const __bf16*)B8; a.C = C; a.bias = bias; a.extra = extra;
    a.M = M; a.N = N; a.K = K8; a.lda = lda; a.ldb = ldb; a.ldc = ldc; a.group = 0;
    a.tiles_m = a.tiles_n = 0; a.ktiles_per_split = K8 / 128; a.split_stride = 0; a.gm = 8; a.rm = 0; a.nsplit = 1;
    a.ln_mean = nullptr; a.ln_rstd = row_scale; a.ln_colsum = col_scale; a.stats_part = nullptr; a.xb_out = nullptr; a.ldxb = 0;
    a.reserve = (flags >> 20) & 255;
    a.dbg = (flags >> 12) & 15;
    return cs_gemm_stream_launch_f8(a, epi, a.reserve, stream);
}
```

### clipself_amd/engine.py

```python
from __future__ import annotations

import math
import os
from collections import OrderedDict

import torch
import torch.nn.functional as F

from .config import TowerCfg

BF16, F32 = torch.bfloat16, torch.float32
EPI_BF16, EPI_F32, EPI_RESID_F32, EPI_SWIGLU_BF16, EPI_ATOMIC_F32, EPI_PATCH_F32, EPI_RESID_LN_F32, EPI_GELU_BF16, EPI_QGELU_BF16 = range(9)
DX_BF16, DX_F32_ASSIGN, DX_F32_ACCUM = range(3)
ALIGN = 64


def _round_up(x: int, m: int) -> int:
    return (x + m - 1) // m * m


def padded_hidden(cfg: TowerCfg) -> int:
    return _round_up(cfg.hidden, 64)


# ... 7 lines not shown
        b = f"{prefix}blocks.{i}."
        groups += [
            [t(b + "norm1.weight", (C,))], [t(b + "norm1.bias", (C,))],
            [t(b + "attn.q_proj.weight", (C, C)), t(b + "attn.k_proj.weight", (C, C)), t(b + "attn.v_proj.weight", (C, C))],
            [t(b + "attn.q_bias", (C,)), t(b + "attn._k_bias_zero", (C,)), t(b + "attn.v_bias", (C,))],
            [t(b + "attn.inner_attn_ln.weight", (C,))], [t(b + "attn.inner_attn_ln.bias", (C,))],
            [t(b + "attn.proj.weight", (C, C))], [t(b + "attn.proj.bias", (C,))],
            [t(b + "norm2.weight", (C,))], [t(b + "norm2.bias", (C,))],
            [t(b + "mlp.w1.weight", (Hd, C), (Hp, C)), t(b + "mlp.w2.weight", (Hd, C), (Hp, C))],
            [t(b + "mlp.w1.bias", (Hd,), (Hp,)), t(b + "mlp.w2.bias", (Hd,), (Hp,))],
            [t(b + "mlp.ffn_ln.weight", (Hd,), (Hp,))], [t(b + "mlp.ffn_ln.bias", (Hd,), (Hp,))],
            [t(b + "mlp.w3.weight", (C, Hd), (C, Hp))], [t(b + "mlp.w3.bias", (C,))],
        ]
    groups += [[t(prefix + "norm.weight", (C,))], [t(prefix + "norm.bias", (C,))],
               [t(prefix + "head.weight", (E, C))], [t(prefix + "head.bias", (E,))]]
    return groups


def is_no_decay(name: str, ndim: int) -> bool:
    return ndim < 2 or "bn" in name or "ln" in name or "bias" in name or "logit_scale" in name


class EvaEngine:
    BLOCK_TAG = "blocks."
    FP8_MAX_ROW = 8192

    def _layout(self):
        return param_groups_layout(self.cfg, self.prefix)

    def block_index(self, name: str):
        tag = self.prefix + self.BLOCK_TAG
        return int(name[len(tag):].split(".")[0]) if name.startswith(tag) else None

    def _never_reached(self, i: int, name: str) -> bool:
        return i == self.cfg.layers - 1 and (name.rsplit(".", 2)[-2:] in (["q_proj", "weight"], ["k_proj", "weight"])
                                             or name.endswith("attn.q_bias"))

    def __init__(self, cfg: TowerCfg, ops, trainable: bool = False, prefix: str = "visual."):
        self.cfg, self.ops, self.prefix, self.trainable = cfg, ops, prefix, trainable
        self.offsets = OrderedDict()
        self.logical = {}
        off = 0
        self.block_ranges = []
        cur_block, blk_begin = None, 0
        for grp in self._layout():
            off = _round_up(off, ALIGN)
            blk = self.block_index(grp[0][0])
            if blk != cur_block:
                if cur_block is not None:
                    self.block_ranges.append((blk_begin, off))
                cur_block, blk_begin = blk, off
            for name, shape, storage in grp:
                self.offsets[name] = (off, storage)
                self.logical[name] = shape
                off += math.prod(storage)
        self.numel = _round_up(off, 256)
        self.stem_range = (0, self.block_ranges[0][0]) if self.block_ranges else (0, 0)
        self.head_range = (self.block_ranges[-1][1], self.numel) if self.block_ranges else (0, self.numel)
        self.master = ops.zeros((self.numel,), F32)
        self.shadow = ops.zeros((self.numel,), BF16)
        self.device = self.master.device
        self.Hp = padded_hidden(cfg)
        self.Kpe = _round_up(3 * cfg.patch_size * cfg.patch_size, 64)
        self.p = {n: self.view_of(self.master, n) for n in self.offsets}
        self.w = {n: self.view_of(self.shadow, n) for n in self.offsets}
        self._tables = {}
        self._pos_cache = {}
        self.grad = self.exp_avg = self.exp_avg_sq = self.flags = None
        self.g = {}
        self.wt = {}
        self.first_trainable = cfg.layers
        self.train_all = False
        self.flags_version = 0
        self.grad_ready_hook = None
        self._ctx = None
        self._wgrad_ws = None
        self.cls_only_last_block = True
        self.fold_sub_ln = not trainable
        self.fold_block_ln = not trainable
        self.block_fold_guard = not trainable
        self.block_fold_limit = 2.0
        self.block_fold_ratio = None
        self.split_stream = not trainable
        self.fold = {}
        self.fp8_forward = False
        self.w8 = {}
        self.fp8_dgrad = False
        self.wt8 = {}
        self.rccl_window = (0, 0)
        self.wgrad_tn = True
        self.fused_swiglu_colsum = os.environ.get("CLIPSELF_NO_FUSED_SWIGLU_COLSUM") != "1"
        if trainable:
            self.grad = ops.zeros((self.numel,), F32)
            self.exp_avg = ops.zeros((self.numel,), F32)
            self.exp_avg_sq = ops.zeros((self.numel,), F32)
            self.g = {n: self.view_of(self.grad, n) for n in self.offsets}
            self.flags = torch.zeros(self.numel // 64, dtype=torch.uint8, device=self.device)

    def storage_of(self, buf, name):
        o, st = self.offsets[name]
        return buf[o:o + math.prod(st)].view(st)

    def view_of(self, buf, name):
        o, st = self.offsets[name]
        shape = self.logical[name]
        flat = buf[o:o + math.prod(st)]
        if tuple(st) == tuple(shape) or math.prod(st) == math.prod(shape):
            return flat.view(shape)
        if len(st) == 1:
            return flat[:shape[0]]
        if len(shape) == 2:
            return flat.view(st)[:shape[0], :shape[1]]
        inner = [1]
        for d in reversed(shape[2:]):
            inner.insert(0, inner[0] * d)
        return torch.as_strided(flat, shape, (st[1], *inner))

    def public_names(self):
        return [n for n in self.offsets if "._" not in n]

    def load_state(self, sd: dict, strict: bool = True):
        missing = []
        with torch.no_grad():
            for n in self.public_names():
                if n in sd:
                    self.p[n].copy_(sd[n].to(self.device, F32).reshape(self.p[n].shape))
                else:
                    missing.append(n)
        if strict and missing:
            raise KeyError(f"missing keys: {missing[:5]}... ({len(missing)})")
        self.sync_shadow()
        return missing

    def sync_shadow(self):
        self.ops.cast_f32_bf16(self.master, self.shadow)
        self._pos_cache.clear()
        self.block_fold_ratio = None
        if self.trainable:
            self.sync_transposed()
        if self.fold_sub_ln:
            self._build_folds()
        if self.fp8_forward:
            self.sync_fp8()

    def _build_folds(self):
        cfg, C, Hl = self.cfg, self.cfg.width, self.cfg.hidden
        self.fold = {}
        with torch.no_grad():
            for i in range(cfg.layers):
                b = f"{self.prefix}blocks.{i}."
                out = {}
                for key, wname, ln, bname, K in (("proj", "attn.proj.weight", "attn.inner_attn_ln", "attn.proj.bias", C),
                                                 ("w3", "mlp.w3.weight", "mlp.ffn_ln", "mlp.w3.bias", Hl)):
                    W = self.storage_of(self.master, b + wname)
                    g, beta = self.p[b + ln + ".weight"][:K], self.p[b + ln + ".bias"][:K]
                    Wf = torch.zeros_like(W, dtype=BF16)
                    Wf[:, :K] = (W[:, :K] * g[None, :]).to(BF16)
                    out[key] = (Wf, Wf.float().sum(dim=1).contiguous(), (W[:, :K] @ beta + self.p[b + bname]).contiguous())
                if self.fold_block_ln:
                    Hd = self.Hp
                    for key, wname, bias_name, ln, rows in (("qkv", "attn.q_proj.weight", "attn.q_bias", "norm1", 3 * C),
                                                           ("w12", "mlp.w1.weight", "mlp.w1.bias", "norm2", 2 * Hd)):
                        o, ob = self.offsets[b + wname][0], self.offsets[b + bias_name][0]
                        W, bias = self.master[o:o + rows * C].view(rows, C), self.master[ob:ob + rows]
                        g, beta = self.p[b + ln + ".weight"], self.p[b + ln + ".bias"]
                        Wf = (W * g[None, :]).to(BF16).contiguous()
# ... 68 lines not shown

    def _ln(self, x, gamma, beta, y, mean, rstd, eps):
        if not self.fp8_forward:
            self.ops.layernorm_fwd(x, gamma, beta, y, mean, rstd, eps)
            return None
        M = x.shape[0]
        q = self.ops.empty((M, _round_up(y.shape[1], 128)), torch.uint8)
        sc = self.ops.empty((M,), F32)
        self.ops.layernorm_fwd(x, gamma, beta, y, mean, rstd, eps, q8=q, q_scale=sc)
        return q, sc

    def _linear(self, i, key, X, W, out, bias, extra=None, epi=EPI_BF16, rows=None, xq=None):
        if not self.fp8_forward:
            self.ops.gemm_nt(X, W, out, bias=bias, extra=extra, epi=epi)
            return
        xq, sx = xq if xq is not None else self._fp8_rows(X)
        w8, sw = self.w8[(i, key)]
        if rows is not None:
            w8, sw = w8[rows[0]:rows[1]], sw[rows[0]:rows[1]]
        self.ops.gemm_nt_f8(xq, w8, out, sx, sw, bias=bias, extra=extra, epi=epi)

    def set_trainable_blocks(self, unlocked_groups: int):
        L = self.cfg.layers
        self.first_trainable = L - unlocked_groups if 0 < unlocked_groups <= L else 0
        self.train_all = False
        self._set_flags()

    def set_trainable_all(self):
        self.first_trainable = 0
        self.train_all = True
        self._set_flags()

    def _set_flags(self):
        if not self.trainable:
            return
        self.flags.zero_()
        names = list(self.offsets)
        for k, name in enumerate(names):
            o, s = self.offsets[name]
            i = self.block_index(name)
            if "._" in name or (i is None and not self._nonblock_trains(name)) or (i is not None and (i < self.first_trainable or self._never_reached(i, name))):
                continue
            n = math.prod(s)
            nxt = self.offsets[names[k + 1]][0] if k + 1 < len(names) else self.numel
            n64 = _round_up(n, 64)
            assert o % 64 == 0 and (n % 64 == 0 or o + n64 <= nxt), f"{name}: flag granularity"
            self.flags[o // 64:(o + n64) // 64] = 1 | (0 if is_no_decay(name, len(self.logical[name])) else 2)
        self.flags_version += 1
        for key in [k for k in self.wt if isinstance(k, tuple) and k[0] < self.first_trainable]:
            del self.wt[key]
        for key in [k for k in self.wt8 if k[0] < self.first_trainable]:
            del self.wt8[key]
        self.sync_transposed()
        if self.fp8_forward and self.fp8_dgrad:
            self.sync_fp8(range(self.first_trainable, self.cfg.layers))

    def _nonblock_trains(self, name):
        return self.train_all

    def _pos_trains(self):
        return self.train_all

    def trainable_names(self):
        if self.train_all:
            return self.public_names()
        return [n for n in self.public_names()
                if (self.block_index(n) >= self.first_trainable if self.block_index(n) is not None else self._nonblock_trains(n))]

    def bucket_range(self, key):
        return self.head_range if key == "head" else self.stem_range if key == "stem" else self.block_ranges[key]

    def rope_tables(self, grid: int):
        key = ("rope", grid)
        if key not in self._tables:
            half = self.cfg.head_width // 2
            freqs = 1.0 / (10000.0 ** (torch.arange(0, half, 2)[: half // 2].float() / half))
            t = torch.arange(grid).float() / grid * self.cfg.pt_hw_seq_len
            ang = (t[:, None] * freqs[None, :]).repeat_interleave(2, dim=-1)
            full = torch.cat([ang[:, None, :].expand(grid, grid, half), ang[None, :, :].expand(grid, grid, half)], dim=-1)
            full = full.reshape(grid * grid, self.cfg.head_width)
            self._tables[key] = (full.cos().contiguous().to(self.device), full.sin().contiguous().to(self.device))
        return self._tables[key]

    def pos_for(self, grid: int):
        if grid not in self._pos_cache:
            pe = self.p[self.prefix + "pos_embed"][0]
            if grid != self.cfg.grid:
                C = pe.shape[1]
                pe2 = pe[1:].T.contiguous().view(1, C, self.cfg.grid, self.cfg.grid)
                pe2 = F.interpolate(pe2, (grid, grid), mode="bicubic", align_corners=False).view(C, grid * grid)
                pe = torch.cat([pe[:1], pe2.T], dim=0)
            self._pos_cache[grid] = pe.contiguous()
        return self._pos_cache[grid]

    def _stem(self, images, keep=None):
        ops, cfg, P = self.ops, self.cfg, self.prefix
        B, _, S, _ = images.shape
        p, C = cfg.patch_size, cfg.width
        g = S // p
        N, Kpe = g * g + 1, self.Kpe
        A = ops.empty((B * g * g, Kpe), BF16)
        ops.im2row(images.contiguous(), A, p)
        x = ops.empty((B, N, C), F32)
        pos = self.pos_for(g)
        ops.gemm_nt(A, self.storage_of(self.shadow, P + "patch_embed.proj.weight"), x.view(B * N, C),
                    bias=self.p[P + "patch_embed.proj.bias"], extra=pos, epi=EPI_PATCH_F32, group=g * g)
        ops.cls_row(x, self.p[P + "cls_token"].view(C), pos)
        if keep is not None:
            keep["patches"] = A
        return x, g

    def _qkv_w(self, b):
        C = self.cfg.width
        o = self.offsets[b + "attn.q_proj.weight"][0]
        ob = self.offsets[b + "attn.q_bias"][0]
        return self.shadow[o:o + 3 * C * C].view(3 * C, C), self.master[ob:ob + 3 * C]

    def _w12(self, b):
        C, Hd = self.cfg.width, self.Hp
        o = self.offsets[b + "mlp.w1.weight"][0]
        ob = self.offsets[b + "mlp.w1.bias"][0]
        return self.shadow[o:o + 2 * Hd * C].view(2 * Hd, C), self.master[ob:ob + 2 * Hd]

    def _block_fwd(self, i, x, B, N, cos, sin, with_attn=True, save=None, inplace=True):
        ops, cfg = self.ops, self.cfg
        C, Hd, Hl, H, eps = cfg.width, self.Hp, cfg.hidden, cfg.heads, cfg.ln_eps
        padded = Hd != Hl
        b = f"{self.prefix}blocks.{i}."
        M = B * N
        keep = save is not None
        st = (lambda: (ops.empty((M,), F32), ops.empty((M,), F32))) if keep else (lambda: (None, None))

        ln1 = ops.empty((M, C), BF16)
        m1, r1 = st()
        q1 = self._ln(x, self.p[b + "norm1.weight"], self.p[b + "norm1.bias"], ln1, m1, r1, eps)
        wqkv, bqkv = self._qkv_w(b)
        qkv = lse = None
        if with_attn and not keep and inplace and self.fold_sub_ln:
            qkv = ops.empty((M, 3 * C), BF16)
            ops.gemm_nt(ln1, wqkv, qkv, bias=bqkv, epi=EPI_BF16)
            att = ops.empty((M, C), BF16)
            part = ops.empty((H, M, 2), F32)
            ops.attn_fwd_stats(qkv, cos, sin, att, None, part, B, N, H, cfg.head_width ** -0.5)
            return self._block_post_folded(i, b, x, att, part, M)
        if with_attn:
            qkv = ops.empty((M, 3 * C), BF16)
            self._linear(i, "qkv", ln1, wqkv, qkv, bqkv, xq=q1)
            att = ops.empty((M, C), BF16)
            lse = ops.empty((B * H, N), F32) if keep else None
            ops.attn_fwd(qkv, cos, sin, att, lse, B, N, H, cfg.head_width ** -0.5)
        else:
            att = ops.empty((M, C), BF16)
            self._linear(i, "qkv", ln1, wqkv[2 * C:], att, bqkv[2 * C:], rows=(2 * C, 3 * C), xq=q1)
        x2 = self._block_post(i, b, x, att, M, st, save, inplace)
        if keep:
            save.update(x0=x, ln1=ln1, st1=(m1, r1), qkv=qkv, lse=lse, att=att, with_attn=with_attn)
        return x2

    def _block_post(self, i, b, x, att, M, st, save, inplace):
        ops, cfg = self.ops, self.cfg
        C, Hd, Hl, eps = cfg.width, self.Hp, cfg.hidden, cfg.ln_eps
        padded = Hd != Hl
        keep = save is not None
        iln = ops.empty((M, C), BF16)
        m2, r2 = st()
        q2 = self._ln(att, self.p[b + "attn.inner_attn_ln.weight"], self.p[b + "attn.inner_attn_ln.bias"], iln, m2, r2, eps)
        x1 = x if inplace else ops.empty((M, C), F32)
        self._linear(i, "proj", iln, self.w[b + "attn.proj.weight"], x1, self.p[b + "attn.proj.bias"], extra=x, epi=EPI_RESID_F32, xq=q2)

        ln2 = ops.empty((M, C), BF16)
        m3, r3 = st()
        q3 = self._ln(x1, self.p[b + "norm2.weight"], self.p[b + "norm2.bias"], ln2, m3, r3, eps)
        w12, b12 = self._w12(b)
        hid = ops.empty((M, Hd), BF16)
        x12 = None
        if keep or self.fp8_forward:
            x12 = ops.empty((M, 2 * Hd), BF16)
            self._linear(i, "w12", ln2, w12, x12, b12, xq=q3)
            ops.swiglu_fwd(x12, hid)
        else:
            ops.gemm_nt(ln2, w12, hid, bias=b12, epi=EPI_SWIGLU_BF16, group=Hd)
        fln = (ops.zeros if padded else ops.empty)((M, Hd), BF16)
        m4, r4 = st()
        q4 = self._ln(hid[:, :Hl], self.p[b + "mlp.ffn_ln.weight"], self.p[b + "mlp.ffn_ln.bias"], fln[:, :Hl], m4, r4, eps)
        x2 = x1 if inplace else ops.empty((M, C), F32)
        self._linear(i, "w3", fln, self.storage_of(self.shadow, b + "mlp.w3.weight"), x2, self.p[b + "mlp.w3.bias"], extra=x1,
                     epi=EPI_RESID_F32, xq=q4)
        if keep:
            save.update(iln=iln, st2=(m2, r2), x1=x1, ln2=ln2, st3=(m3, r3), x12=x12, hid=hid, fln=fln, st4=(m4, r4))
        return x2

    def _block_post_folded(self, i, b, x, att, att_part, M):
        ops, cfg = self.ops, self.cfg
        C, Hd, Hl, eps = cfg.width, self.Hp, cfg.hidden, cfg.ln_eps
        f = self.fold[i]
        mean, rstd = ops.empty((M,), F32), ops.empty((M,), F32)
        ops.ln_stats_finalize(att_part, 64, C, mean, rstd, eps)
        Wp, cp, dp = f["proj"]
        ops.gemm_nt_ln(att, Wp, x, bias=dp, extra=x, ln_mean=mean, ln_rstd=rstd, ln_colsum=cp, epi=EPI_RESID_LN_F32)

        ln2 = ops.empty((M, C), BF16)
        ops.layernorm_fwd(x, self.p[b + "norm2.weight"], self.p[b + "norm2.bias"], ln2, None, None, eps)
        w12, b12 = self._w12(b)
        hid = ops.empty((M, Hd), BF16)
        part = ops.empty((4 * ((Hd + 127) // 128), M, 2), F32)
        ops.gemm_nt_ln(ln2, w12, hid, bias=b12, stats_part=part, epi=EPI_SWIGLU_BF16, group=Hd)
        ops.ln_stats_finalize(part, 32, Hl, mean, rstd, eps)
        W3, c3, d3 = f["w3"]
        ops.gemm_nt_ln(hid, W3, x, bias=d3, extra=x, ln_mean=mean, ln_rstd=rstd, ln_colsum=c3, epi=EPI_RESID_LN_F32)
        return x

    def _teacher_block_folded(self, i, x, xb, st, B, N, cos, sin, emit_next, lo=None):
        ops, cfg = self.ops, self.cfg
        C, Hd, Hl, H, eps = cfg.width, self.Hp, cfg.hidden, cfg.heads, cfg.ln_eps
        b = f"{self.prefix}blocks.{i}."
        M = B * N
        f = self.fold[i]
        qkv = ops.empty((M, 3 * C), BF16)
        first = xb is None
        if first:
            ln1 = ops.empty((M, C), BF16)
            ops.layernorm_fwd(x, self.p[b + "norm1.weight"], self.p[b + "norm1.bias"], ln1, None, None, eps)
            wqkv, bqkv = self._qkv_w(b)
            ops.gemm_nt(ln1, wqkv, qkv, bias=bqkv, epi=EPI_BF16)
        else:
            Wq, cq, dq = f["qkv"]
            ops.gemm_nt_ln(xb, Wq, qkv, bias=dq, ln_mean=st[0], ln_rstd=st[1], ln_colsum=cq, epi=EPI_BF16)
        att = ops.empty((M, C), BF16)
        part_a = ops.empty((H, M, 2), F32)
        ops.attn_fwd_stats(qkv, cos, sin, att, None, part_a, B, N, H, cfg.head_width ** -0.5)
        mean, rstd = ops.empty((M,), F32), ops.empty((M,), F32)
        ops.ln_stats_finalize(part_a, 64, C, mean, rstd, eps)
        Wp, cp, dp = f["proj"]
        part_x = ops.empty(((C + 63) // 64, M, 2), F32)
        xb2 = xb if (lo is not None and not first) else ops.empty((M, C), BF16)
        if lo is not None:
            ops.gemm_nt_ln_split(att, Wp, xb2, lo, dp, mean, rstd, cp, x_in=x if first else None, stats_part=part_x)
        else:
            ops.gemm_nt_ln(att, Wp, x, bias=dp, extra=x, ln_mean=mean, ln_rstd=rstd, ln_colsum=cp, stats_part=part_x, xb_out=xb2,
                           epi=EPI_RESID_LN_F32)
        mean2, rstd2 = ops.empty((M,), F32), ops.empty((M,), F32)
        ops.ln_stats_finalize(part_x, 64, C, mean2, rstd2, eps)
        W12, c12, d12 = f["w12"]
        hid = ops.empty((M, Hd), BF16)
        part_h = ops.empty((4 * ((Hd + 127) // 128), M, 2), F32)
        ops.gemm_nt_ln(xb2, W12, hid, bias=d12, ln_mean=mean2, ln_rstd=rstd2, ln_colsum=c12, stats_part=part_h, epi=EPI_SWIGLU_BF16,
                       group=Hd)
        ops.ln_stats_finalize(part_h, 32, Hl, mean, rstd, eps)
        W3, c3, d3 = f["w3"]
        if lo is not None:
            if not emit_next:
                ops.gemm_nt_ln_split(hid, W3, xb2, lo, d3, mean, rstd, c3, x_out=x)
                return None, None
            ops.gemm_nt_ln_split(hid, W3, xb2, lo, d3, mean, rstd, c3, stats_part=part_x)
        else:
            if not emit_next:
                ops.gemm_nt_ln(hid, W3, x, bias=d3, extra=x, ln_mean=mean, ln_rstd=rstd, ln_colsum=c3, epi=EPI_RESID_LN_F32)
                return None, None
            ops.gemm_nt_ln(hid, W3, x, bias=d3, extra=x, ln_mean=mean, ln_rstd=rstd, ln_colsum=c3, stats_part=part_x, xb_out=xb2,
                           epi=EPI_RESID_LN_F32)
        ops.ln_stats_finalize(part_x, 64, C, mean2, rstd2, eps)
        return xb2, (mean2, rstd2)

    @staticmethod
    def _join_planes(hi, lo):
        y = (hi.contiguous().view(torch.int16).to(torch.int32) << 16) | (lo.to(torch.int32) & 0xFFFF)
        return (y - 0x8000).view(torch.float32)

    def _block_fwd_cls(self, i, x, B, N, cos, sin, xb=None, st=None, lo=None):
        ops, cfg = self.ops, self.cfg
        C, H, eps = cfg.width, cfg.heads, cfg.ln_eps
        b = f"{self.prefix}blocks.{i}."
        M = B * N
        wqkv, bqkv = self._qkv_w(b)
        kv = ops.empty((M, 2 * C), BF16)
        q = ops.empty((B, C), BF16)
        if xb is not None:
            Wq, cq, dq = self.fold[i]["qkv"]
            ops.gemm_nt_ln(xb, Wq[C:], kv, bias=dq[C:], ln_mean=st[0], ln_rstd=st[1], ln_colsum=cq[C:], epi=EPI_BF16)
            xc = (self._join_planes(xb.view(B, N, C)[:, 0, :], lo.view(B, N, C)[:, 0, :]) if lo is not None
                  else x.view(B, N, C)[:, 0, :].contiguous())
            ln1c = ops.empty((B, C), BF16)
            ops.layernorm_fwd(xc, self.p[b + "norm1.weight"], self.p[b + "norm1.bias"], ln1c, None, None, eps)
            ops.gemm_nt(ln1c, wqkv[:C], q, bias=bqkv[:C], epi=EPI_BF16)
        else:
            ln1 = ops.empty((M, C), BF16)
            ops.layernorm_fwd(x, self.p[b + "norm1.weight"], self.p[b + "norm1.bias"], ln1, None, None, eps)
            ops.gemm_nt(ln1, wqkv[C:], kv, bias=bqkv[C:], epi=EPI_BF16)
            ops.gemm_nt(ln1.view(B, N, C)[:, 0, :], wqkv[:C], q, bias=bqkv[:C], epi=EPI_BF16)
            xc = x.view(B, N, C)[:, 0, :].contiguous()
        att = ops.empty((B, C), BF16)
        ops.attn_cls_fwd(q, kv, cos, sin, att, B, N, H, cfg.head_width ** -0.5)
        return self._block_post(i, b, xc, att, B, lambda: (None, None), None, True)

    def fold_probe(self, crops: int = 16, kind: str = "white"):
        import numpy as np
        S = self.cfg.image_size
        g = np.random.Generator(np.random.PCG64(20250927 if kind == "white" else 20251001))
        x = g.standard_normal((crops, 3, S, S), dtype=np.float32)
        if kind == "natural":
            f = np.hypot(np.fft.fftfreq(S)[:, None], np.fft.rfftfreq(S)[None, :]).astype(np.float32)
            f[0, 0] = 1.0
            x = np.fft.irfft2(np.fft.rfft2(x) / f, s=(S, S)).astype(np.float32)
            x -= x.mean(axis=(2, 3), keepdims=True)
            x /= x.std(axis=(2, 3), keepdims=True) + 1e-6
            x = 0.5 * x + g.standard_normal((crops, 3, 1, 1), dtype=np.float32)
        elif kind != "white":
            raise ValueError(kind)
        return torch.from_numpy(np.ascontiguousarray(x)).to(self.device)

    def block_fold_statistic(self, images=None, crops: int = 16):
        if images is None:
            return max(self.block_fold_statistic(self.fold_probe(crops, kind), crops) for kind in ("white", "natural"))
# ... 292 lines not shown
```

### clipself_amd/engine_openai.py

```python
from __future__ import annotations

import torch
import torch.nn.functional as F

from .config import TowerCfg
from .engine import (BF16, DX_F32_ACCUM, DX_F32_ASSIGN, EPI_BF16, EPI_F32, EPI_GELU_BF16, EPI_PATCH_F32, EPI_QGELU_BF16,
                     EPI_RESID_F32, F32, EvaEngine, _round_up)


def clip_vit_layout(cfg: TowerCfg, prefix: str = "visual."):
    C, Hd, E, p = cfg.width, cfg.hidden, cfg.embed_dim, cfg.patch_size
    Kp = _round_up(3 * p * p, 64)
    t = lambda name, shape, storage=None: (name, shape, storage if storage is not None else shape)
    groups = [[t(prefix + "class_embedding", (C,))], [t(prefix + "positional_embedding", (cfg.tokens, C))],
              [t(prefix + "conv1.weight", (C, 3, p, p), (C, Kp))], [t(prefix + "ln_pre.weight", (C,))], [t(prefix + "ln_pre.bias", (C,))]]
    for i in range(cfg.layers):
        b = f"{prefix}transformer.resblocks.{i}."
        groups += [[t(b + "ln_1.weight", (C,))], [t(b + "ln_1.bias", (C,))],
                   [t(b + "attn.in_proj_weight", (3 * C, C))], [t(b + "attn.in_proj_bias", (3 * C,))],
                   [t(b + "attn.out_proj.weight", (C, C))], [t(b + "attn.out_proj.bias", (C,))],
                   [t(b + "ln_2.weight", (C,))], [t(b + "ln_2.bias", (C,))],
                   [t(b + "mlp.c_fc.weight", (Hd, C))], [t(b + "mlp.c_fc.bias", (Hd,))],
                   [t(b + "mlp.c_proj.weight", (C, Hd))], [t(b + "mlp.c_proj.bias", (C,))]]
    groups += [[t(prefix + "ln_post.weight", (C,))], [t(prefix + "ln_post.bias", (C,))], [t(prefix + "proj", (C, E))]]
    return groups


class ClipVitEngine(EvaEngine):
    BLOCK_TAG = "transformer.resblocks."

    def __init__(self, cfg: TowerCfg, ops, trainable: bool = False, prefix: str = "visual."):
        if cfg.hidden % 64 or cfg.width % 64 or cfg.embed_dim % 64:
            raise NotImplementedError(f"{cfg.name}: width, MLP width and embed_dim must be multiples of 64")
        super().__init__(cfg, ops, trainable=trainable, prefix=prefix)
        self.fold_sub_ln = False
        self.fold_block_ln = not trainable
        self.cls_only_last_block = True
        self.fold_cls_block = True
        self.stem_level = 0

    def _layout(self):
        return clip_vit_layout(self.cfg, self.prefix)

    def _never_reached(self, i, name):
        return False

    def sync_transposed(self, blocks=None):
        cfg, C, Hd = self.cfg, self.cfg.width, self.cfg.hidden
        pairs = [(self.w[self.prefix + "proj"], self._wt_alloc("head_fwd", C, cfg.embed_dim))]
        if self.trainable:
            for i in (range(self.first_trainable, cfg.layers) if blocks is None else blocks):
                b = f"{self.prefix}{self.BLOCK_TAG}{i}."
                pairs.append((self.w[b + "attn.in_proj_weight"], self._wt_alloc((i, "qkv"), 3 * C, C)))
                pairs.append((self.w[b + "attn.out_proj.weight"], self._wt_alloc((i, "proj"), C, C)))
                pairs.append((self.w[b + "mlp.c_fc.weight"], self._wt_alloc((i, "fc"), Hd, C)))
                pairs.append((self.w[b + "mlp.c_proj.weight"], self._wt_alloc((i, "cproj"), C, Hd)))
        self.ops.transpose_bf16_batched(pairs)

    def sync_shadow(self):
        self.ops.cast_f32_bf16(self.master, self.shadow)
        self._pos_cache.clear()
        self.block_fold_ratio = None
        self.sync_transposed()
        if self.fold_block_ln:
            self._build_folds()

    def _build_folds(self):
        self.fold = {}
        with torch.no_grad():
            for i in range(self.cfg.layers):
                b = f"{self.prefix}{self.BLOCK_TAG}{i}."
                out = {}
                for key, wname, bname, ln in (("qkv", "attn.in_proj_weight", "attn.in_proj_bias", "ln_1"), ("fc", "mlp.c_fc.weight", "mlp.c_fc.bias", "ln_2")):
                    W, bias = self.p[b + wname], self.p[b + bname]
                    Wf = (W * self.p[b + ln + ".weight"][None, :]).to(BF16).contiguous()
                    out[key] = (Wf, Wf.float().sum(dim=1).contiguous(), (W @ self.p[b + ln + ".bias"] + bias).contiguous())
                self.fold[i] = out

    def set_trainable_blocks(self, unlocked_groups: int):
        L = self.cfg.layers
        self.stem_level = min(max(unlocked_groups - L, 0), 2)
        super().set_trainable_blocks(min(unlocked_groups, L))
        if unlocked_groups <= 0:
            self.first_trainable = L
            if self.trainable:
                self.flags.zero_()

    def set_trainable_all(self):
        self.stem_level = 2
        super().set_trainable_all()

    def _nonblock_trains(self, name):
        if self.train_all:
            return True
        tail = name[len(self.prefix):]
        if tail == "positional_embedding":
            return self.stem_level >= 1
        return self.stem_level >= 2 and tail in ("conv1.weight", "class_embedding", "ln_pre.weight", "ln_pre.bias")

    def _pos_trains(self):
        return self.stem_level >= 1

    def rope_tables(self, grid: int):
        key = ("rope", grid)
        if key not in self._tables:
            shape = (grid * grid, self.cfg.head_width)
            self._tables[key] = (torch.ones(shape, dtype=F32, device=self.device), torch.zeros(shape, dtype=F32, device=self.device))
        return self._tables[key]

    def pos_for(self, grid: int):
        if grid not in self._pos_cache:
            pe = self.p[self.prefix + "positional_embedding"]
            if grid != self.cfg.grid:
                C = pe.shape[1]
                pe2 = pe[1:].T.contiguous().view(1, C, self.cfg.grid, self.cfg.grid)
                pe2 = F.interpolate(pe2, (grid, grid), mode="bicubic", align_corners=False).view(C, grid * grid)
                pe = torch.cat([pe[:1], pe2.T], dim=0)
            self._pos_cache[grid] = pe.contiguous()
        return self._pos_cache[grid]

    def _stem(self, images, keep=None):
        ops, cfg, P = self.ops, self.cfg, self.prefix
        B, _, S, _ = images.shape
        p, C = cfg.patch_size, cfg.width
        g = S // p
        N = g * g + 1
        A = ops.empty((B * g * g, self.Kpe), BF16)
        ops.im2row(images.contiguous(), A, p)
        x = ops.empty((B, N, C), F32)
        pos = self.pos_for(g)
        ops.gemm_nt(A, self.storage_of(self.shadow, P + "conv1.weight"), x.view(B * N, C), extra=pos, epi=EPI_PATCH_F32, group=g * g)
        ops.cls_row(x, self.p[P + "class_embedding"], pos)
        y = ops.empty((B, N, C), F32)
        mean = rstd = None
        if keep is not None:
            mean, rstd = ops.empty((B * N,), F32), ops.empty((B * N,), F32)
            keep.update(patches=A, x_pre=x.view(B * N, C), st=(mean, rstd))
        ops.layernorm_fwd_f32(x.view(B * N, C), self.p[P + "ln_pre.weight"], self.p[P + "ln_pre.bias"], y.view(B * N, C), mean, rstd, cfg.ln_eps)
        return y, g

    def _block_fwd(self, i, x, B, N, cos, sin, with_attn=True, save=None, inplace=True):
        ops, cfg = self.ops, self.cfg
        C, Hd, H, eps = cfg.width, cfg.hidden, cfg.heads, cfg.ln_eps
        b = f"{self.prefix}{self.BLOCK_TAG}{i}."
        M = B * N
        keep = save is not None
        st = (lambda: (ops.empty((M,), F32), ops.empty((M,), F32))) if keep else (lambda: (None, None))

        ln1 = ops.empty((M, C), BF16)
        m1, r1 = st()
        ops.layernorm_fwd(x, self.p[b + "ln_1.weight"], self.p[b + "ln_1.bias"], ln1, m1, r1, eps)
        wqkv, bqkv = self.w[b + "attn.in_proj_weight"], self.p[b + "attn.in_proj_bias"]
        qkv = lse = None
        att = ops.empty((M, C), BF16)
        if with_attn:
            qkv = ops.empty((M, 3 * C), BF16)
            ops.gemm_nt(ln1, wqkv, qkv, bias=bqkv, epi=EPI_BF16)
            lse = ops.empty((B * H, N), F32) if keep else None
            ops.attn_fwd(qkv, cos, sin, att, lse, B, N, H, cfg.head_width ** -0.5)
        else:
            ops.gemm_nt(ln1, wqkv[2 * C:], att, bias=bqkv[2 * C:], epi=EPI_BF16)
        x1 = x if inplace else ops.empty((M, C), F32)
        ops.gemm_nt(att, self.w[b + "attn.out_proj.weight"], x1, bias=self.p[b + "attn.out_proj.bias"], extra=x, epi=EPI_RESID_F32)

        ln2 = ops.empty((M, C), BF16)
        m2, r2 = st()
        ops.layernorm_fwd(x1, self.p[b + "ln_2.weight"], self.p[b + "ln_2.bias"], ln2, m2, r2, eps)
        hid = ops.empty((M, Hd), BF16)
        fc = None
        if keep:
            fc = ops.empty((M, Hd), BF16)
            ops.gemm_nt(ln2, self.w[b + "mlp.c_fc.weight"], fc, bias=self.p[b + "mlp.c_fc.bias"], epi=EPI_BF16)
            ops.gelu_fwd(fc, hid, cfg.quick_gelu)
        else:
            ops.gemm_nt(ln2, self.w[b + "mlp.c_fc.weight"], hid, bias=self.p[b + "mlp.c_fc.bias"],
                        epi=EPI_QGELU_BF16 if cfg.quick_gelu else EPI_GELU_BF16)
        x2 = x1 if inplace else ops.empty((M, C), F32)
        ops.gemm_nt(hid, self.w[b + "mlp.c_proj.weight"], x2, bias=self.p[b + "mlp.c_proj.bias"], extra=x1, epi=EPI_RESID_F32)
        if keep:
            save.update(x0=x, ln1=ln1, st1=(m1, r1), qkv=qkv, lse=lse, att=att, with_attn=with_attn, x1=x1, ln2=ln2, st2=(m2, r2),
                        fc=fc, hid=hid)
        return x2

    def _teacher_block_folded(self, i, x, xb, st, B, N, cos, sin, emit_next, lo=None):
        ops, cfg = self.ops, self.cfg
        C, Hd, H, eps = cfg.width, cfg.hidden, cfg.heads, cfg.ln_eps
        b = f"{self.prefix}{self.BLOCK_TAG}{i}."
        M = B * N
        f = self.fold[i]
        qkv = ops.empty((M, 3 * C), BF16)
        first = xb is None
        if first:
            ln1 = ops.empty((M, C), BF16)
            ops.layernorm_fwd(x, self.p[b + "ln_1.weight"], self.p[b + "ln_1.bias"], ln1, None, None, eps)
            ops.gemm_nt(ln1, self.w[b + "attn.in_proj_weight"], qkv, bias=self.p[b + "attn.in_proj_bias"], epi=EPI_BF16)
        else:
            Wq, cq, dq = f["qkv"]
            ops.gemm_nt_ln(xb, Wq, qkv, bias=dq, ln_mean=st[0], ln_rstd=st[1], ln_colsum=cq, epi=EPI_BF16)
        att = ops.empty((M, C), BF16)
        ops.attn_fwd(qkv, cos, sin, att, None, B, N, H, cfg.head_width ** -0.5)
        part = ops.empty(((C + 63) // 64, M, 2), F32)
        xb2 = xb if (lo is not None and not first) else ops.empty((M, C), BF16)
        ident = self._identity_stats(M, C) if lo is not None else None
        wo, bo = self.w[b + "attn.out_proj.weight"], self.p[b + "attn.out_proj.bias"]
        if lo is not None:
            ops.gemm_nt_ln_split(att, wo, xb2, lo, bo, *ident, x_in=x if first else None, stats_part=part)
        else:
            ops.gemm_nt_ln(att, wo, x, bias=bo, extra=x, stats_part=part, xb_out=xb2, epi=EPI_RESID_F32)
        mean, rstd = ops.empty((M,), F32), ops.empty((M,), F32)
        ops.ln_stats_finalize(part, 64, C, mean, rstd, eps)
        Wf, cf, df = f["fc"]
        hid = ops.empty((M, Hd), BF16)
        ops.gemm_nt_ln(xb2, Wf, hid, bias=df, ln_mean=mean, ln_rstd=rstd, ln_colsum=cf, epi=EPI_QGELU_BF16 if cfg.quick_gelu else EPI_GELU_BF16)
        wp, bp = self.w[b + "mlp.c_proj.weight"], self.p[b + "mlp.c_proj.bias"]
        if lo is not None:
            if not emit_next:
                ops.gemm_nt_ln_split(hid, wp, xb2, lo, bp, *ident, x_out=x)
                return None, None
            ops.gemm_nt_ln_split(hid, wp, xb2, lo, bp, *ident, stats_part=part)
        else:
            if not emit_next:
                ops.gemm_nt(hid, wp, x, bias=bp, extra=x, epi=EPI_RESID_F32)
                return None, None
            ops.gemm_nt_ln(hid, wp, x, bias=bp, extra=x, stats_part=part, xb_out=xb2, epi=EPI_RESID_F32)
        ops.ln_stats_finalize(part, 64, C, mean, rstd, eps)
        return xb2, (mean, rstd)

    def _identity_stats(self, M, C):
        key = ("ident", M, C)
        if key not in self._tables:
            self._tables[key] = (torch.zeros(M, dtype=F32, device=self.device), torch.ones(M, dtype=F32, device=self.device),
                                 torch.zeros(C, dtype=F32, device=self.device))
        return self._tables[key]

    def _block_fwd_cls(self, i, x, B, N, cos, sin, xb=None, st=None, lo=None):
        ops, cfg = self.ops, self.cfg
        C, Hd, H, eps = cfg.width, cfg.hidden, cfg.heads, cfg.ln_eps
        b = f"{self.prefix}{self.BLOCK_TAG}{i}."
        M = B * N
        wqkv, bqkv = self.w[b + "attn.in_proj_weight"], self.p[b + "attn.in_proj_bias"]
        kv = ops.empty((M, 2 * C), BF16)
        q = ops.empty((B, C), BF16)
        if xb is not None:
            Wq, cq, dq = self.fold[i]["qkv"]
            ops.gemm_nt_ln(xb, Wq[C:], kv, bias=dq[C:], ln_mean=st[0], ln_rstd=st[1], ln_colsum=cq[C:], epi=EPI_BF16)
            xc = (self._join_planes(xb.view(B, N, C)[:, 0, :], lo.view(B, N, C)[:, 0, :]) if lo is not None
                  else x.view(B, N, C)[:, 0, :].contiguous())
            ln1c = ops.empty((B, C), BF16)
            ops.layernorm_fwd(xc, self.p[b + "ln_1.weight"], self.p[b + "ln_1.bias"], ln1c, None, None, eps)
            ops.gemm_nt(ln1c, wqkv[:C], q, bias=bqkv[:C], epi=EPI_BF16)
        else:
            ln1 = ops.empty((M, C), BF16)
            ops.layernorm_fwd(x, self.p[b + "ln_1.weight"], self.p[b + "ln_1.bias"], ln1, None, None, eps)
            ops.gemm_nt(ln1, wqkv[C:], kv, bias=bqkv[C:], epi=EPI_BF16)
            ops.gemm_nt(ln1.view(B, N, C)[:, 0, :], wqkv[:C], q, bias=bqkv[:C], epi=EPI_BF16)
            xc = x.view(B, N, C)[:, 0, :].contiguous()
        att = ops.empty((B, C), BF16)
        ops.attn_cls_fwd(q, kv, cos, sin, att, B, N, H, cfg.head_width ** -0.5)
        ops.gemm_nt(att, self.w[b + "attn.out_proj.weight"], xc, bias=self.p[b + "attn.out_proj.bias"], extra=xc, epi=EPI_RESID_F32)
        ln2 = ops.empty((B, C), BF16)
        ops.layernorm_fwd(xc, self.p[b + "ln_2.weight"], self.p[b + "ln_2.bias"], ln2, None, None, eps)
        hid = ops.empty((B, Hd), BF16)
        ops.gemm_nt(ln2, self.w[b + "mlp.c_fc.weight"], hid, bias=self.p[b + "mlp.c_fc.bias"], epi=EPI_QGELU_BF16 if cfg.quick_gelu else EPI_GELU_BF16)
        ops.gemm_nt(hid, self.w[b + "mlp.c_proj.weight"], xc, bias=self.p[b + "mlp.c_proj.bias"], extra=xc, epi=EPI_RESID_F32)
        return xc

    def _head(self, rows, out):
        self.ops.gemm_nt(rows, self.wt["head_fwd"][:, :self.cfg.width], out, epi=EPI_F32)

    def encode_image(self, images, chunk: int = 256):
        ops, cfg, P = self.ops, self.cfg, self.prefix
        K = images.shape[0]
        out = ops.empty((K, cfg.embed_dim), F32)
        fold_blocks = self.block_folds_active(images)
        for k0 in range(0, K, chunk):
            img = images[k0:k0 + chunk]
            B = img.shape[0]
            x, g = self._stem(img)
            N = g * g + 1
            cos, sin = self.rope_tables(g)
            xf = x.view(B * N, cfg.width)
            last = cfg.layers - 1 if self.cls_only_last_block else cfg.layers
            xb = st = None
            cls_folded = fold_blocks and self.fold_cls_block and last < cfg.layers and last > 0
            lo = ops.empty((B * N, cfg.width), torch.int16) if fold_blocks and self.split_stream and (last > 1 or cls_folded) else None
            try:
                for i in range(last):
                    self._rccl_window_step(i, k0)
                    if fold_blocks:
                        xb, st = self._teacher_block_folded(i, xf, xb, st, B, N, cos, sin, emit_next=i + 1 < last or cls_folded, lo=lo)
                    else:
                        self._block_fwd(i, xf, B, N, cos, sin, True, None, True)
            finally:
                self._rccl_window_close(k0)
            if last < cfg.layers:
                xc = self._block_fwd_cls(last, xf, B, N, cos, sin, xb if cls_folded else None, st, lo)
            else:
                xc = x[:, 0, :]
            cls = ops.empty((B, cfg.width), BF16)
            ops.layernorm_fwd(xc, self.p[P + "ln_post.weight"], self.p[P + "ln_post.bias"], cls, None, None, cfg.ln_eps)
            self._head(cls, out[k0:k0 + B])
        return out

    def mask_attn_pool(self, images, masks, chunk: int = 64):
        ops, cfg, P = self.ops, self.cfg, self.prefix
        C, Hd, H, eps, E = cfg.width, cfg.hidden, cfg.heads, cfg.ln_eps, cfg.embed_dim
        counts = [int(m.shape[0]) for m in masks]
        assert len(masks) == images.shape[0], "one mask list per image"
        Q = max(counts) if counts else 0
        if Q == 0:
            return torch.zeros((0, E), dtype=F32, device=self.device)
        outs = []
        act = EPI_QGELU_BF16 if cfg.quick_gelu else EPI_GELU_BF16
        for k0 in range(0, images.shape[0], chunk):
            img = images[k0:k0 + chunk]
            B = img.shape[0]
            x, g = self._stem(img)
            N = g * g + 1
            cos, sin = self.rope_tables(g)
            allow = torch.ones((B, Q, N), dtype=torch.uint8, device=self.device)
            for b, m in enumerate(masks[k0:k0 + B]):
                assert tuple(m.shape[1:]) == (g, g), f"masks live on the {g}x{g} token grid, got {tuple(m.shape[1:])}"
                allow[b, :m.shape[0], 1:] = m.reshape(m.shape[0], -1).to(device=self.device, dtype=torch.uint8)
            allow = allow.view(B * Q, N)
            xf = x.view(B * N, C)
            xm = x[:, :1, :].expand(B, Q, C).reshape(B * Q, C).contiguous()
            MQ = B * Q
            for i in range(cfg.layers):
                b_ = f"{P}{self.BLOCK_TAG}{i}."
                wqkv, bqkv = self.w[b_ + "attn.in_proj_weight"], self.p[b_ + "attn.in_proj_bias"]
                ln1 = ops.empty((B * N, C), BF16)
                ops.layernorm_fwd(xf, self.p[b_ + "ln_1.weight"], self.p[b_ + "ln_1.bias"], ln1, None, None, eps)
                qkv = ops.empty((B * N, 3 * C), BF16)
                ops.gemm_nt(ln1, wqkv, qkv, bias=bqkv, epi=EPI_BF16)
                lnm = ops.empty((MQ, C), BF16)
                ops.layernorm_fwd(xm, self.p[b_ + "ln_1.weight"], self.p[b_ + "ln_1.bias"], lnm, None, None, eps)
                qm = ops.empty((MQ, C), BF16)
                ops.gemm_nt(lnm, wqkv[:C], qm, bias=bqkv[:C], epi=EPI_BF16)
                attm = ops.empty((MQ, C), BF16)
                ops.attn_query_fwd(qm, qkv[:, C:], allow, attm, B, Q, N, H, cfg.head_width ** -0.5)
                ops.gemm_nt(attm, self.w[b_ + "attn.out_proj.weight"], xm, bias=self.p[b_ + "attn.out_proj.bias"], extra=xm, epi=EPI_RESID_F32)
                ln2 = ops.empty((MQ, C), BF16)
                ops.layernorm_fwd(xm, self.p[b_ + "ln_2.weight"], self.p[b_ + "ln_2.bias"], ln2, None, None, eps)
                hid = ops.empty((MQ, Hd), BF16)
                ops.gemm_nt(ln2, self.w[b_ + "mlp.c_fc.weight"], hid, bias=self.p[b_ + "mlp.c_fc.bias"], epi=act)
                ops.gemm_nt(hid, self.w[b_ + "mlp.c_proj.weight"], xm, bias=self.p[b_ + "mlp.c_proj.bias"], extra=xm, epi=EPI_RESID_F32)
                if i + 1 < cfg.layers:
                    att = ops.empty((B * N, C), BF16)
                    ops.attn_fwd(qkv, cos, sin, att, None, B, N, H, cfg.head_width ** -0.5)
                    ops.gemm_nt(att, self.w[b_ + "attn.out_proj.weight"], xf, bias=self.p[b_ + "attn.out_proj.bias"], extra=xf, epi=EPI_RESID_F32)
                    ln2i = ops.empty((B * N, C), BF16)
                    ops.layernorm_fwd(xf, self.p[b_ + "ln_2.weight"], self.p[b_ + "ln_2.bias"], ln2i, None, None, eps)
                    hidi = ops.empty((B * N, Hd), BF16)
                    ops.gemm_nt(ln2i, self.w[b_ + "mlp.c_fc.weight"], hidi, bias=self.p[b_ + "mlp.c_fc.bias"], epi=act)
                    ops.gemm_nt(hidi, self.w[b_ + "mlp.c_proj.weight"], xf, bias=self.p[b_ + "mlp.c_proj.bias"], extra=xf, epi=EPI_RESID_F32)
            lnp = ops.empty((MQ, C), BF16)
            ops.layernorm_fwd(xm, self.p[P + "ln_post.weight"], self.p[P + "ln_post.bias"], lnp, None, None, eps)
            pooled = ops.empty((MQ, E), F32)
            self._head(lnp, pooled)
            pooled = pooled.view(B, Q, E)
            outs += [pooled[b, :n] for b, n in enumerate(counts[k0:k0 + B])]
        return torch.cat(outs)

    def encode_dense(self, images, need_grad: bool = False):
        ops, cfg, P = self.ops, self.cfg, self.prefix
        B = images.shape[0]
        stem_keep = {} if (need_grad and self.stem_level > 0) else None
        x, g = self._stem(images, stem_keep)
        N, C, E = g * g + 1, cfg.width, cfg.embed_dim
        cos, sin = self.rope_tables(g)
        xf = x.view(B * N, C)
        saves = {}
        for i in range(cfg.layers):
            keep = need_grad and i >= self.first_trainable
            save = {} if keep else None
            xf = self._block_fwd(i, xf, B, N, cos, sin, with_attn=(i < cfg.layers - 1), save=save, inplace=not keep)
            if keep:
                saves[i] = save
        M = B * N
        lnf = ops.empty((M, C), BF16)
        mean = ops.empty((M,), F32) if need_grad else None
        rstd = ops.empty((M,), F32) if need_grad else None
        ops.layernorm_fwd(xf, self.p[P + "ln_post.weight"], self.p[P + "ln_post.bias"], lnf, mean, rstd, cfg.ln_eps)
        feats = ops.empty((M, E), F32)
        self._head(lnf, feats)
        dense = ops.empty((M, E), F32)
        inv = ops.empty((M,), F32)
        ops.l2norm_fwd(feats, dense, inv)
        if need_grad:
            self._ctx = dict(B=B, N=N, g=g, saves=saves, xL=xf, stf=(mean, rstd), dense=dense, inv=inv, cos=cos, sin=sin, stem=stem_keep,
                             lnf=lnf if self.train_all else None)
        return dense.view(B, N, E), g

    def _block_bwd(self, i, s, g, gb, B, N, cos, sin, ws, next_bias=None):
        ops, cfg = self.ops, self.cfg
        C, Hd, H = cfg.width, cfg.hidden, cfg.heads
        b = f"{self.prefix}{self.BLOCK_TAG}{i}."
        M = B * N
        G = self.g
        self._wgrad(gb, s["hid"], G[b + "mlp.c_proj.weight"])
        d_hid = ops.empty((M, Hd), BF16)
        ops.gemm_nt(gb, self.wt[(i, "cproj")][:, :C], d_hid, epi=EPI_BF16)
        d_fc = ops.empty((M, Hd), BF16)
        ops.gelu_bwd(d_hid, s["fc"], d_fc, cfg.quick_gelu)
        ops.colsum_bf16(d_fc, G[b + "mlp.c_fc.bias"], ws[1])
        self._wgrad(d_fc, s["ln2"], G[b + "mlp.c_fc.weight"])
        d_ln2 = ops.empty((M, C), BF16)
        ops.gemm_nt(d_fc, self.wt[(i, "fc")][:, :Hd], d_ln2, epi=EPI_BF16)
        ops.layernorm_bwd(d_ln2, s["x1"], self.p[b + "ln_2.weight"], *s["st2"], g, DX_F32_ACCUM,
                          G[b + "ln_2.weight"], G[b + "ln_2.bias"], True, ws[0], dx_copy=gb, copy_colsum=G[b + "attn.out_proj.bias"])
        self._wgrad(gb, s["att"], G[b + "attn.out_proj.weight"])
        d_att = ops.empty((M, C), BF16)
        ops.gemm_nt(gb, self.wt[(i, "proj")][:, :C], d_att, epi=EPI_BF16)
        d_ln1 = ops.empty((M, C), BF16)
        Gw, Gb = G[b + "attn.in_proj_weight"], G[b + "attn.in_proj_bias"]
        if s["with_attn"]:
            d_qkv = ops.empty((M, 3 * C), BF16)
            ops.attn_bwd(s["qkv"], s["att"], d_att, s["lse"], cos, sin, d_qkv, ws[0], B, N, H, cfg.head_width ** -0.5)
            ops.colsum_bf16(d_qkv, Gb, ws[1])
            self._wgrad(d_qkv, s["ln1"], Gw)
            ops.gemm_nt(d_qkv, self.wt[(i, "qkv")][:, :3 * C], d_ln1, epi=EPI_BF16)
        else:
            ops.colsum_bf16(d_att, Gb[2 * C:], ws[1])
            self._wgrad(d_att, s["ln1"], Gw[2 * C:])
            ops.gemm_nt(d_att, self.wt[(i, "qkv")][:, 2 * C:3 * C], d_ln1, epi=EPI_BF16)
        ops.layernorm_bwd(d_ln1, s["x0"], self.p[b + "ln_1.weight"], *s["st1"], g, DX_F32_ACCUM,
                          G[b + "ln_1.weight"], G[b + "ln_1.bias"], True, ws[0], dx_copy=gb if next_bias is not None else None,
                          copy_colsum=next_bias)

    def backward_dense(self, d_dense):
        ops, cfg, P = self.ops, self.cfg, self.prefix
        c = self._ctx
# ... 57 lines not shown
```

### clipself_amd/hip.py

```python
from __future__ import annotations

import ctypes
import os
import subprocess
from pathlib import Path

import torch

_CSRC = Path(__file__).resolve().parent / "csrc"
_LIB_PATH = Path(os.environ["CLIPSELF_HIP_LIB"]) if os.environ.get("CLIPSELF_HIP_LIB") else _CSRC / "libclipself_hip.so"

EPI_BF16, EPI_F32, EPI_RESID_F32, EPI_SWIGLU_BF16, EPI_ATOMIC_F32, EPI_PATCH_F32, EPI_RESID_LN_F32, EPI_GELU_BF16, EPI_QGELU_BF16 = range(9)
DX_BF16, DX_F32_ASSIGN, DX_F32_ACCUM = range(3)

_vp, _i, _l, _f, _sz = ctypes.c_void_p, ctypes.c_int, ctypes.c_long, ctypes.c_float, ctypes.c_size_t

SIGNATURES = {
    "cs_last_error": (ctypes.c_char_p, []),
    "cs_gemm_nt": (_i, [_vp, _vp, _vp, _vp, _vp, _i, _i, _i, _i, _i, _i, _i, _i, _i, _i, _vp]),
    "cs_crop_resize_workspace": (_sz, [_i, _i, _i]),
    "cs_crop_resize_u8": (_i, [_vp, _i, _i, _vp, _i, _i, _i, _vp, _vp, _vp, _vp, _vp]),
    "cs_quant_rows_fp8": (_i, [_vp, _l, _vp, _l, _vp, _i, _i, _vp]),
    "cs_gemm_nt_f8": (_i, [_vp, _vp, _vp, _vp, _vp, _vp, _vp, _i, _i, _i, _i, _i, _i, _i, _i, _vp]),
    "cs_resize_bilinear_f32": (_i, [_vp, _vp, _i, _i, _i, _i, _i, _vp]),
    "cs_gemm_wgrad_workspace": (_sz, [_i, _i, _i]),
    "cs_gemm_wgrad": (_i, [_vp, _vp, _vp, _vp, _i, _i, _i, _i, _i, _i, _vp]),
    "cs_gemm_wgrad_tn_workspace": (_sz, [_i, _i, _i]),
    "cs_gemm_wgrad_tn": (_i, [_vp, _vp, _vp, _vp, _i, _i, _i, _i, _i, _i, _vp]),
    "cs_gemm_nt_ln": (_i, [_vp, _vp, _vp, _vp, _vp, _vp, _vp, _vp, _vp, _vp, _i, _i, _i, _i, _i, _i, _i, _i, _i, _i, _i, _vp]),
    "cs_gemm_nt_ln_split": (_i, [_vp, _vp, _vp, _vp, _vp, _vp, _vp, _vp, _vp, _vp, _i, _vp, _i, _i, _i, _i, _i, _i, _i, _vp]),
    "cs_ln_stats_finalize": (_i, [_vp, _i, _i, _i, _i, _f, _vp, _vp, _vp]),
    "cs_attn_fwd_stats": (_i, [_vp, _vp, _vp, _vp, _vp, _vp, _i, _i, _i, _i, _i, _f, _vp]),
    "cs_layernorm_fwd": (_i, [_vp, _i, _l, _vp, _vp, _vp, _l, _vp, _vp, _i, _i, _f, _vp]),
    "cs_layernorm_fwd_q8": (_i, [_vp, _i, _l, _vp, _vp, _vp, _l, _vp, _vp, _vp, _l, _vp, _i, _i, _f, _vp]),
    "cs_layernorm_fwd_f32": (_i, [_vp, _l, _vp, _vp, _vp, _l, _vp, _vp, _i, _i, _f, _vp]),
    "cs_layernorm_bwd_workspace": (_sz, [_i, _i]),
    "cs_layernorm_bwd": (_i, [_vp, _l, _vp, _i, _l, _vp, _vp, _vp, _vp, _i, _l, _vp, _vp, _i, _vp, _vp, _l, _vp, _i, _i, _vp]),
    "cs_layernorm_bwd_q8": (_i, [_vp, _l, _vp, _i, _l, _vp, _vp, _vp, _vp, _i, _l, _vp, _vp, _i, _vp, _vp, _l, _vp, _vp, _l, _vp, _i, _i, _vp]),
    "cs_l2norm_fwd": (_i, [_vp, _vp, _vp, _i, _i, _f, _vp]),
    "cs_l2norm_bwd": (_i, [_vp, _vp, _vp, _vp, _i, _i, _vp]),
    "cs_attn_fwd": (_i, [_vp, _vp, _vp, _vp, _vp, _i, _i, _i, _i, _i, _f, _vp]),
    "cs_attn_cls_fwd": (_i, [_vp, _vp, _vp, _vp, _vp, _i, _i, _i, _i, _i, _i, _f, _vp]),
    "cs_attn_query_fwd": (_i, [_vp, _vp, _vp, _vp, _i, _i, _i, _i, _i, _i, _i, _f, _vp]),
    "cs_attn_bwd_workspace": (_sz, [_i, _i, _i]),
    "cs_attn_bwd": (_i, [_vp, _vp, _vp, _vp, _vp, _vp, _vp, _vp, _i, _i, _i, _i, _i, _f, _vp]),
    "cs_swiglu_fwd": (_i, [_vp, _l, _vp, _l, _i, _i, _vp]),
    "cs_swiglu_bwd": (_i, [_vp, _l, _vp, _l, _vp, _l, _i, _i, _vp]),
    "cs_swiglu_bwd_colsum": (_i, [_vp, _l, _vp, _l, _vp, _l, _vp, _vp, _i, _i, _vp]),
    "cs_swiglu_bwd_q8": (_i, [_vp, _l, _vp, _l, _vp, _l, _vp, _l, _vp, _i, _i, _vp]),
    "cs_gelu_fwd": (_i, [_vp, _l, _vp, _l, _i, _i, _i, _vp]),
    "cs_gelu_bwd": (_i, [_vp, _l, _vp, _l, _vp, _l, _i, _i, _i, _vp]),
    "cs_cast_f32_bf16": (_i, [_vp, _vp, _l, _vp]),
    "cs_transpose_bf16": (_i, [_vp, _l, _vp, _l, _i, _i, _vp]),
    "cs_transpose_bf16_batched": (_i, [_vp, _i, _i, _vp]),
    "cs_colsum_workspace": (_sz, [_i, _i]),
    "cs_colsum_bf16": (_i, [_vp, _l, _vp, _vp, _i, _i, _vp]),
    "cs_im2row": (_i, [_vp, _i, _vp, _i, _i, _i, _i, _vp]),
    "cs_cls_row": (_i, [_vp, _vp, _vp, _i, _i, _i, _vp]),
    "cs_roialign_fwd": (_i, [_vp, _vp, _vp, _i, _i, _i, _i, _i, _i, _vp]),
    "cs_roialign_bwd": (_i, [_vp, _vp, _vp, _i, _i, _i, _i, _i, _i, _i, _vp]),
    "cs_cosine_loss_fwd": (_i, [_vp, _vp, _vp, _vp, _i, _i, _f, _vp]),
    "cs_cosine_loss_bwd": (_i, [_vp, _vp, _vp, _vp, _i, _i, _f, _f, _vp, _vp]),
    "cs_fed_bce_fwd": (_i, [_vp, _l, _vp, _vp, _vp, _i, _i, _f, _f, _vp]),
    "cs_fed_bce_bwd": (_i, [_vp, _l, _vp, _vp, _l, _i, _i, _f, _f, _vp, _vp]),
    "cs_num_compute_units": (_i, []),
    "cs_stream_create_cu_mask": (_i, [_i, _i, ctypes.POINTER(_vp)]),
    "cs_stream_destroy": (_i, [_vp]),
    "cs_adamw_step": (_i, [_vp, _vp, _vp, _vp, _vp, _vp, _l, _f, _f, _f, _f, _f, _i, _f, _vp]),
}


def library_path() -> Path:
    return _LIB_PATH


def build_library(force: bool = False) -> Path:
    if force:
        for o in _CSRC.glob("_obj_*.o"):
            o.unlink()
    subprocess.run(["bash", str(_CSRC / "build.sh")], check=True)
    return _LIB_PATH


_lib = None


def load_library():
    global _lib
    if _lib is None:
        if not _LIB_PATH.exists():
            raise RuntimeError(
                f"{_LIB_PATH} is missing: build it with clipself_amd/csrc/build.sh (or __graft_entry__.build()). "
                "There is no CPU fallback for the CLIPSelf hot path.")
        lib = ctypes.CDLL(str(_LIB_PATH))
        for name, (res, args) in SIGNATURES.items():
            fn = getattr(lib, name)
            fn.restype, fn.argtypes = res, args
        _lib = lib
    return _lib


def _p(t):
    return None if t is None else t.data_ptr()


def _dt(t) -> int:
    if t.dtype == torch.float32:
        return 0
    if t.dtype == torch.bfloat16:
        return 1
    raise TypeError(f"unsupported dtype {t.dtype}")


class HipOps:

    name = "hip"

    def __init__(self):
        self.lib = load_library()
        if not torch.cuda.is_available():
            raise RuntimeError("HipOps needs a ROCm device (torch.cuda.is_available() is False); no CPU fallback exists")
        self.gemm_flags = 0
        self._rccl_reserve = 0
        self._share = 0
        self._cap = 0
        self.num_cus = int(self.lib.cs_num_compute_units())

    def _update_flags(self):
        n = self._rccl_reserve + self._share
        if self._cap:
            n = max(n, self.num_cus - self._cap)
        if not (0 <= n <= self.num_cus - 8 and n < 256):
            raise ValueError(f"persistent GEMM grids keep at least 8 workgroups and can leave at most 255 compute units free "
                             f"(asked to leave {n} of {self.num_cus} CUs: RCCL reserve {self._rccl_reserve}, tower share {self._share}, cap {self._cap})")
        self.gemm_flags = (self.gemm_flags & ~(255 << 20)) | (int(n) << 20)

    def reserve_compute_units(self, n: int):
        self._rccl_reserve = int(n)
        self._update_flags()

    def share_compute_units(self, n: int):
        self._share = int(n)
        self._update_flags()

    def cap_compute_units(self, n: int):
        self._cap = int(n)
        self._update_flags()

    def persistent_grid(self) -> int:
        return self.num_cus - ((self.gemm_flags >> 20) & 255)

    def num_compute_units(self) -> int:
        return self.num_cus

    def stream_create_cu_mask(self, first_cu: int, n_cus: int):
        h = ctypes.c_void_p()
        self._ok(self.lib.cs_stream_create_cu_mask(int(first_cu), int(n_cus), ctypes.byref(h)), "cs_stream_create_cu_mask")
        s = torch.cuda.ExternalStream(h.value)
        s._cs_handle = h.value
        return s

    def stream_destroy(self, stream):
        torch.cuda.synchronize()
        self._ok(self.lib.cs_stream_destroy(ctypes.c_void_p(stream._cs_handle)), "cs_stream_destroy")

    def _stream(self):
        return torch.cuda.current_stream().cuda_stream

    def _ok(self, rc, who):
        if rc != 0:
            raise RuntimeError(f"{who} failed ({rc}): {self.lib.cs_last_error().decode()}")

    @staticmethod
    def _chk(*ts):
        for t in ts:
            if t is not None and not t.is_cuda:
                raise RuntimeError("HipOps received a non-GPU tensor; the hot path has no CPU fallback")

    def empty(self, shape, dtype):
        return torch.empty(shape, dtype=dtype, device="cuda")

    def zeros(self, shape, dtype):
        return torch.zeros(shape, dtype=dtype, device="cuda")

    def gemm_nt(self, A, B, C, bias=None, extra=None, epi=EPI_BF16, splits=1, group=0, flags=0):
        self._chk(A, B, C, bias, extra)
        M, K = A.shape
        N = B.shape[0]
        assert B.shape[1] == K and A.stride(1) == 1 and B.stride(1) == 1 and C.stride(-1) == 1
        if extra is not None and epi in (EPI_RESID_F32, EPI_PATCH_F32):
            assert extra.stride(0) == C.stride(0), "extra must share C's row stride"
        self._ok(self.lib.cs_gemm_nt(_p(A), _p(B), _p(C), _p(bias), _p(extra), M, N, K, A.stride(0), B.stride(0),
                                     C.stride(0), epi, splits, group, flags | self.gemm_flags, self._stream()), "cs_gemm_nt")

    def gemm_nt_ln(self, A, B, C, bias=None, extra=None, ln_mean=None, ln_rstd=None, ln_colsum=None, stats_part=None, xb_out=None,
                   epi=EPI_RESID_LN_F32, group=0, flags=0):
        self._chk(A, B, C, bias, extra, ln_mean, ln_rstd, ln_colsum, stats_part, xb_out)
        M, K = A.shape
        N = B.shape[0]
        assert B.shape[1] == K and A.stride(1) == 1 and B.stride(1) == 1 and C.stride(-1) == 1
        if extra is not None and epi in (EPI_RESID_F32, EPI_RESID_LN_F32):
            assert extra.stride(0) == C.stride(0), "extra must share C's row stride"
        if stats_part is not None:
            slices = 4 * ((group + 127) // 128) if epi == EPI_SWIGLU_BF16 else (N + 63) // 64
            assert stats_part.is_contiguous() and stats_part.shape[0] >= slices and stats_part.shape[1] == M
        if xb_out is not None:
            assert xb_out.dtype == torch.bfloat16 and xb_out.stride(1) == 1 and xb_out.shape[0] == M
        self._ok(self.lib.cs_gemm_nt_ln(_p(A), _p(B), _p(C), _p(bias), _p(extra), _p(ln_mean), _p(ln_rstd), _p(ln_colsum), _p(stats_part),
                                        _p(xb_out), xb_out.stride(0) if xb_out is not None else 0, M, N, K, A.stride(0), B.stride(0),
                                        C.stride(0), epi, 1, group, flags | self.gemm_flags, self._stream()), "cs_gemm_nt_ln")

    def gemm_nt_ln_split(self, A, B, hi, lo, bias, ln_mean, ln_rstd, ln_colsum, x_in=None, x_out=None, stats_part=None, flags=0):
        self._chk(A, B, hi, lo, bias, ln_mean, ln_rstd, ln_colsum, x_in, x_out, stats_part)
        M, K = A.shape
        N = B.shape[0]
        assert hi.dtype == torch.bfloat16 and lo.dtype == torch.int16 and hi.shape == (M, N) and lo.shape == (M, N)
        assert hi.stride(1) == 1 and lo.stride(1) == 1 and hi.stride(0) == lo.stride(0) and hi.stride(0) % 8 == 0
        assert x_out is None or stats_part is None, "fp32 out: hi / lo are only read, no statistics epilogue"
        x = x_in if x_in is not None else x_out
        assert x is None or (x.dtype == torch.float32 and x.shape == (M, N) and x.stride(1) == 1)
        self._ok(self.lib.cs_gemm_nt_ln_split(_p(A), _p(B), _p(bias), _p(ln_mean), _p(ln_rstd), _p(ln_colsum), _p(x_in), _p(x_out), _p(hi), _p(lo),
                                              hi.stride(0), _p(stats_part), M, N, K, A.stride(0), B.stride(0), x.stride(0) if x is not None else N,
                                              flags | self.gemm_flags, self._stream()), "cs_gemm_nt_ln_split")

    def quant_rows_fp8(self, x, q, scale):
        self._chk(x, q, scale)
        M, K = x.shape
        assert x.dtype == torch.bfloat16 and x.stride(1) == 1 and q.element_size() == 1 and q.stride(1) == 1 and q.shape[1] == (K + 127) // 128 * 128
        self._ok(self.lib.cs_quant_rows_fp8(_p(x), x.stride(0), _p(q), q.stride(0), _p(scale), M, K, self._stream()), "cs_quant_rows_fp8")

    def gemm_nt_f8(self, A8, B8, C, row_scale, col_scale, bias=None, extra=None, epi=EPI_BF16, flags=0):
        self._chk(A8, B8, C, row_scale, col_scale, bias, extra)
        M, K8 = A8.shape
        N = B8.shape[0]
        assert B8.shape[1] == K8 and A8.element_size() == 1 and B8.element_size() == 1 and C.stride(-1) == 1
        if extra is not None:
            assert extra.stride(0) == C.stride(0), "extra must share C's row stride"
        self._ok(self.lib.cs_gemm_nt_f8(_p(A8), _p(B8), _p(C), _p(bias), _p(extra), _p(row_scale), _p(col_scale), M, N, K8, A8.stride(0), B8.stride(0),
                                        C.stride(0), epi, flags | self.gemm_flags, self._stream()), "cs_gemm_nt_f8")

    def crop_resize(self, image_u8, boxes, size, pad_center=True, mean=(0.48145466, 0.4578275, 0.40821073),
                    std=(0.26862954, 0.26130258, 0.27577711), out=None):
        self._chk(image_u8, boxes, out)
        assert image_u8.dtype == torch.uint8 and image_u8.dim() == 3 and image_u8.shape[2] == 3 and image_u8.is_contiguous()
        boxes = boxes.to(torch.float32).contiguous()
        H, W, K = image_u8.shape[0], image_u8.shape[1], boxes.shape[0]
        if out is None:
            out = torch.empty((K, 3, size, size), dtype=torch.float32, device=image_u8.device)
        need = int(self.lib.cs_crop_resize_workspace(H, K, size))
        ws = getattr(self, "_crop_ws", None)
        if ws is None or ws.numel() < need:
            ws = self._crop_ws = torch.empty(need, dtype=torch.uint8, device=image_u8.device)
        m3, s3 = (ctypes.c_float * 3)(*mean), (ctypes.c_float * 3)(*std)
        self._ok(self.lib.cs_crop_resize_u8(_p(image_u8), H, W, _p(boxes), K, size, int(bool(pad_center)), m3, s3, _p(out), _p(ws),
                                            self._stream()), "cs_crop_resize_u8")
        return out

    def resize_bilinear(self, x, size):
        self._chk(x)
        assert x.dtype == torch.float32 and x.dim() == 4
        x = x.contiguous()
        B, C, H, W = x.shape
        out = torch.empty((B, C, size, size), dtype=torch.float32, device=x.device)
        self._ok(self.lib.cs_resize_bilinear_f32(_p(x), _p(out), B * C, H, W, size, size, self._stream()), "cs_resize_bilinear_f32")
        return out

    def gemm_wgrad_workspace(self, M, N, K) -> int:
        return int(self.lib.cs_gemm_wgrad_workspace(M, N, K))

    def gemm_wgrad(self, A, B, dW, workspace):
        self._chk(A, B, dW, workspace)
        M, K = A.shape
        N = B.shape[0]
        assert B.shape[1] == K and A.stride(1) == 1 and B.stride(1) == 1 and dW.stride(1) == 1 and dW.dtype == torch.float32
        assert workspace.numel() * workspace.element_size() >= self.gemm_wgrad_workspace(M, N, K)
        self._ok(self.lib.cs_gemm_wgrad(_p(A), _p(B), _p(dW), _p(workspace), M, N, K, A.stride(0), B.stride(0), dW.stride(0),
                                        self._stream()), "cs_gemm_wgrad")

    def gemm_wgrad_tn_workspace(self, N, K, tokens) -> int:
        return int(self.lib.cs_gemm_wgrad_tn_workspace(N, K, tokens))

    def gemm_wgrad_tn(self, dY, X, dW, workspace):
        self._chk(dY, X, dW, workspace)
        T, N = dY.shape
        K = X.shape[1]
        assert X.shape[0] == T and dY.stride(1) == 1 and X.stride(1) == 1 and dW.stride(1) == 1 and dW.dtype == torch.float32
        assert workspace.numel() * workspace.element_size() >= self.gemm_wgrad_tn_workspace(N, K, T) > 0
        rc = self.lib.cs_gemm_wgrad_tn(_p(dY), _p(X), _p(dW), _p(workspace), N, K, T, dY.stride(0), X.stride(0), dW.stride(0), self._stream())
        if rc == 1:
            raise RuntimeError("cs_gemm_wgrad_tn: shape outside the kernel's coverage (check gemm_wgrad_tn_workspace first)")
        self._ok(rc, "cs_gemm_wgrad_tn")

    def ln_stats_finalize(self, part, npp, C, mean, rstd, eps=1e-6):
        self._chk(part, mean, rstd)
        P, M = part.shape[0], part.shape[1]
        assert part.is_contiguous() and part.shape[2] == 2
        self._ok(self.lib.cs_ln_stats_finalize(_p(part), P, npp, C, M, eps, _p(mean), _p(rstd), self._stream()), "cs_ln_stats_finalize")

    def _check_rope_tables(self, cos, sin, Ntok):
        def ver(t):
            try:
                return t._version
            except RuntimeError:
                return -1
        key = (cos.data_ptr(), sin.data_ptr(), ver(cos), ver(sin), Ntok)
        seen = self.__dict__.setdefault("_rope_ok", set())
        if key in seen:
            return
        g = int(round((Ntok - 1) ** 0.5))
        if g * g != Ntok - 1 or tuple(cos.shape) != (Ntok - 1, 64) or tuple(sin.shape) != (Ntok - 1, 64):
            raise ValueError(f"rotary tables must be [g*g, 64] for a square token grid, got {tuple(cos.shape)} for {Ntok} tokens")
        for t in (cos, sin):
            v = t.view(g, g, 64)
            ok = (torch.equal(v[:, :, :32], v[:, :1, :32].expand(g, g, 32)) and torch.equal(v[:, :, 32:], v[:1, :, 32:].expand(g, g, 32))
                  and torch.equal(v[:, 0, :32], v[0, :, 32:]) and torch.equal(v[..., 0::2], v[..., 1::2]))
            if not ok:
                raise ValueError("rotary tables are not in the layout of rope.py:118-142 (separable, row part == column part, one entry per "
                                 "rotation pair): the attention kernels cannot read them")
        if len(seen) > 64:
            seen.clear()
        seen.add(key)

    def attn_fwd_stats(self, qkv, cos, sin, out, lse, stats_part, B, Ntok, H, scale):
        self._chk(qkv, cos, sin, out, lse, stats_part)
        self._check_rope_tables(cos, sin, Ntok)
        assert stats_part.is_contiguous() and tuple(stats_part.shape) == (H, B * Ntok, 2)
        self._ok(self.lib.cs_attn_fwd_stats(_p(qkv), _p(cos), _p(sin), _p(out), _p(lse), _p(stats_part), B, Ntok, H, qkv.stride(0),
                                            out.stride(0), scale, self._stream()), "cs_attn_fwd_stats")

    def layernorm_fwd(self, x, gamma, beta, y, mean=None, rstd=None, eps=1e-6, q8=None, q_scale=None):
        if q8 is not None:
            return self.layernorm_fwd_q8(x, gamma, beta, y, q8, q_scale, mean, rstd, eps)
        self._chk(x, gamma, beta, y, mean, rstd)
        M, C = x.shape
        self._ok(self.lib.cs_layernorm_fwd(_p(x), _dt(x), x.stride(0), _p(gamma), _p(beta), _p(y), y.stride(0) if y is not None else 0,
                                           _p(mean), _p(rstd), M, C, eps, self._stream()), "cs_layernorm_fwd")

    def layernorm_fwd_q8(self, x, gamma, beta, y, q8, q_scale, mean=None, rstd=None, eps=1e-6):
        self._chk(x, gamma, beta, y, mean, rstd, q8, q_scale)
        M, C = x.shape
        assert q8.element_size() == 1 and q8.stride(1) == 1 and q8.shape[1] >= (C + 127) // 128 * 128 and q_scale is not None and y is not None
        self._ok(self.lib.cs_layernorm_fwd_q8(_p(x), _dt(x), x.stride(0), _p(gamma), _p(beta), _p(y), y.stride(0), _p(mean), _p(rstd),
                                              _p(q8), q8.stride(0), _p(q_scale), M, C, eps, self._stream()), "cs_layernorm_fwd_q8")

    def layernorm_fwd_f32(self, x, gamma, beta, y, mean=None, rstd=None, eps=1e-5):
        self._chk(x, gamma, beta, y, mean, rstd)
        M, C = x.shape
        assert x.dtype == torch.float32 and y.dtype == torch.float32 and x.stride(1) == 1 and y.stride(1) == 1
        assert x.data_ptr() != y.data_ptr(), "layernorm_fwd_f32 is out of place"
        self._ok(self.lib.cs_layernorm_fwd_f32(_p(x), x.stride(0), _p(gamma), _p(beta), _p(y), y.stride(0), _p(mean), _p(rstd), M, C, eps,
                                               self._stream()), "cs_layernorm_fwd_f32")

    def layernorm_bwd_workspace(self, M, C) -> int:
        return int(self.lib.cs_layernorm_bwd_workspace(M, C))

    def layernorm_bwd_q8(self, dy, x, gamma, mean, rstd, dx, dx_mode, dgamma, dbeta, accumulate, workspace, dx_copy, copy_colsum, q8, q_scale):
        self._chk(dy, x, gamma, mean, rstd, dx, dgamma, dbeta, workspace, dx_copy, copy_colsum, q8, q_scale)
        M, C = x.shape
        assert dx_copy is not None and dx_copy.dtype == torch.bfloat16 and dx_copy.shape == (M, C) and dx_copy.stride(1) == 1
        assert q8.element_size() == 1 and q8.stride(1) == 1 and q8.shape[1] >= (C + 127) // 128 * 128 and q_scale is not None
        self._ok(self.lib.cs_layernorm_bwd_q8(_p(dy), dy.stride(0), _p(x), _dt(x), x.stride(0), _p(gamma), _p(mean), _p(rstd),
                                              _p(dx), dx_mode, dx.stride(0), _p(dgamma), _p(dbeta), int(accumulate),
                                              _p(workspace), _p(dx_copy), dx_copy.stride(0), _p(copy_colsum), _p(q8), q8.stride(0), _p(q_scale),
                                              M, C, self._stream()), "cs_layernorm_bwd_q8")

    def layernorm_bwd(self, dy, x, gamma, mean, rstd, dx, dx_mode, dgamma=None, dbeta=None, accumulate=False, workspace=None,
                      dx_copy=None, copy_colsum=None, q8=None, q_scale=None):
        if q8 is not None:
            return self.layernorm_bwd_q8(dy, x, gamma, mean, rstd, dx, dx_mode, dgamma, dbeta, accumulate, workspace, dx_copy, copy_colsum,
                                         q8, q_scale)
        self._chk(dy, x, gamma, mean, rstd, dx, dgamma, dbeta, workspace, dx_copy, copy_colsum)
        M, C = x.shape
        if dx_copy is not None:
            assert dx_copy.dtype == torch.bfloat16 and dx_copy.shape == (M, C) and dx_copy.stride(1) == 1
        self._ok(self.lib.cs_layernorm_bwd(_p(dy), dy.stride(0), _p(x), _dt(x), x.stride(0), _p(gamma), _p(mean), _p(rstd),
                                           _p(dx), dx_mode, dx.stride(0), _p(dgamma), _p(dbeta), int(accumulate),
                                           _p(workspace), _p(dx_copy), dx_copy.stride(0) if dx_copy is not None else 0, _p(copy_colsum),
                                           M, C, self._stream()), "cs_layernorm_bwd")

    def l2norm_fwd(self, x, y, inv_norm, eps=1e-12):
        self._chk(x, y, inv_norm)
        M, C = x.shape
        assert x.is_contiguous() and y.is_contiguous()
        self._ok(self.lib.cs_l2norm_fwd(_p(x), _p(y), _p(inv_norm), M, C, eps, self._stream()), "cs_l2norm_fwd")

    def l2norm_bwd(self, dy, y, inv_norm, dx):
        self._chk(dy, y, inv_norm, dx)
        M, C = y.shape
        assert dy.is_contiguous() and y.is_contiguous() and dx.is_contiguous()
        self._ok(self.lib.cs_l2norm_bwd(_p(dy), _p(y), _p(inv_norm), _p(dx), M, C, self._stream()), "cs_l2norm_bwd")

    def attn_fwd(self, qkv, cos, sin, out, lse, B, Ntok, H, scale):
        self._chk(qkv, cos, sin, out, lse)
        self._check_rope_tables(cos, sin, Ntok)
        self._ok(self.lib.cs_attn_fwd(_p(qkv), _p(cos), _p(sin), _p(out), _p(lse), B, Ntok, H, qkv.stride(0), out.stride(0),
                                      scale, self._stream()), "cs_attn_fwd")

    def attn_cls_fwd(self, q, kv, cos, sin, out, B, Ntok, H, scale):
        self._chk(q, kv, cos, sin, out)
        self._ok(self.lib.cs_attn_cls_fwd(_p(q), _p(kv), _p(cos), _p(sin), _p(out), B, Ntok, H, q.stride(0), kv.stride(0),
                                          out.stride(0), scale, self._stream()), "cs_attn_cls_fwd")

    def attn_query_fwd(self, q, kv, allow, out, B, Q, Ntok, H, scale):
        self._chk(q, kv, allow, out)
        assert allow.dtype == torch.uint8 and allow.is_contiguous() and tuple(allow.shape) == (B * Q, Ntok)
        self._ok(self.lib.cs_attn_query_fwd(_p(q), _p(kv), _p(allow), _p(out), B, Q, Ntok, H, q.stride(0), kv.stride(0), out.stride(0),
                                            scale, self._stream()), "cs_attn_query_fwd")

    def attn_bwd_workspace(self, B, Ntok, H) -> int:
        return int(self.lib.cs_attn_bwd_workspace(B, Ntok, H))

    def attn_bwd(self, qkv, o, dout, lse, cos, sin, dqkv, workspace, B, Ntok, H, scale):
        self._chk(qkv, o, dout, lse, cos, sin, dqkv, workspace)
        assert o.stride(0) == dout.stride(0) and qkv.stride(0) == dqkv.stride(0)
        self._ok(self.lib.cs_attn_bwd(_p(qkv), _p(o), _p(dout), _p(lse), _p(cos), _p(sin), _p(dqkv), _p(workspace), B, Ntok, H,
                                      qkv.stride(0), o.stride(0), scale, self._stream()), "cs_attn_bwd")

    def swiglu_fwd(self, x12, h):
        self._chk(x12, h)
        M, Hd = h.shape
        self._ok(self.lib.cs_swiglu_fwd(_p(x12), x12.stride(0), _p(h), h.stride(0), M, Hd, self._stream()), "cs_swiglu_fwd")

    def swiglu_bwd_q8(self, dh, x12, dx12, q8, q_scale):
        self._chk(dh, x12, dx12, q8, q_scale)
        M, Hd = dh.shape
        assert q_scale is not None and q8.element_size() == 1 and q8.stride(1) == 1 and q8.shape[1] >= (2 * Hd + 127) // 128 * 128
        self._ok(self.lib.cs_swiglu_bwd_q8(_p(dh), dh.stride(0), _p(x12), x12.stride(0), _p(dx12), dx12.stride(0), _p(q8), q8.stride(0),
                                           _p(q_scale), M, Hd, self._stream()), "cs_swiglu_bwd_q8")

    def swiglu_bwd_colsum(self, dh, x12, dx12, colsum, workspace):
        self._chk(dh, x12, dx12, colsum, workspace)
        M, Hd = dh.shape
        assert colsum.dtype == torch.float32 and colsum.numel() >= 2 * Hd and colsum.is_contiguous()
        assert workspace.numel() * workspace.element_size() >= self.colsum_workspace(M, 2 * Hd)
        self._ok(self.lib.cs_swiglu_bwd_colsum(_p(dh), dh.stride(0), _p(x12), x12.stride(0), _p(dx12), dx12.stride(0), _p(colsum), _p(workspace),
                                               M, Hd, self._stream()), "cs_swiglu_bwd_colsum")

    def swiglu_bwd(self, dh, x12, dx12, q8=None, q_scale=None):
        if q8 is not None:
            return self.swiglu_bwd_q8(dh, x12, dx12, q8, q_scale)
        self._chk(dh, x12, dx12)
        M, Hd = dh.shape
        self._ok(self.lib.cs_swiglu_bwd(_p(dh), dh.stride(0), _p(x12), x12.stride(0), _p(dx12), dx12.stride(0), M, Hd,
                                        self._stream()), "cs_swiglu_bwd")

    def gelu_fwd(self, x, y, quick=False):
        self._chk(x, y)
        M, N = x.shape
        self._ok(self.lib.cs_gelu_fwd(_p(x), x.stride(0), _p(y), y.stride(0), M, N, int(bool(quick)), self._stream()), "cs_gelu_fwd")

    def gelu_bwd(self, dy, x, dx, quick=False):
        self._chk(dy, x, dx)
        M, N = x.shape
        self._ok(self.lib.cs_gelu_bwd(_p(dy), dy.stride(0), _p(x), x.stride(0), _p(dx), dx.stride(0), M, N, int(bool(quick)),
                                      self._stream()), "cs_gelu_bwd")

    def cast_f32_bf16(self, x, y):
        self._chk(x, y)
        assert x.is_contiguous() and y.is_contiguous() and x.numel() == y.numel()
        self._ok(self.lib.cs_cast_f32_bf16(_p(x), _p(y), x.numel(), self._stream()), "cs_cast_f32_bf16")

    def transpose_bf16(self, inp, out):
        self._chk(inp, out)
        R, Cc = inp.shape
        assert out.shape[0] == Cc and out.is_contiguous()
        self._ok(self.lib.cs_transpose_bf16(_p(inp), inp.stride(0), _p(out), out.shape[1], R, Cc, self._stream()), "cs_transpose_bf16")

    def transpose_bf16_batched(self, pairs):
        import numpy as np
        key = tuple((a.data_ptr(), b.data_ptr(), a.shape, b.shape, a.stride(0)) for a, b in pairs)
        tables = self.__dict__.setdefault("_tr_desc_tables", {})
        cache = tables.get(key)
        if cache is None:
            if len(tables) >= 8:
                tables.clear()
            rec = np.zeros((len(pairs), 6), dtype=np.int64)
            tile0 = 0
# ... 73 lines not shown
```

Baseline: 727.2 images/sec.

## Fuse RoPE rotation of q and k into the QKV GEMM epilogue

Adds a rotary epilogue to the streaming bf16 GEMM that rotates the q and k columns with a compact per-grid-row table, selected by a new flag bit. The attention forward kernels gain a no-RoPE template variant that runs when the cos/sin tables are null, so q/k arrive pre-rotated and attention skips the table loads, a barrier and the per-element rotation. The intent is to take the rotary work off the attention kernels' critical path. The GEMM epilogue takes on the extra rotation work, and the rotary path is excluded from the 192-row tile schedule, which could slow the QKV GEMM.

```diff
diff --git a/clipself_amd/csrc/attention.hip b/clipself_amd/csrc/attention.hip
--- a/clipself_amd/csrc/attention.hip
+++ b/clipself_amd/csrc/attention.hip
@@ -195,13 +195,14 @@
     return out.v;
 }
 
+template <bool ROPE = true>
 __device__ __forceinline__ void load_q_frags(const AttnArgs& p, const float* rt, size_t rowbase, int qc, int h, int hf, bf16x8 (&qf)[4]) {
     U128 t[4];
 #pragma unroll
     for (int ks = 0; ks < 4; ++ks) t[ks].u = *(const uint4*)(p.qkv + (rowbase + qc) * p.ldqkv + h * HD + ks * 16 + hf * 8);
 #pragma unroll
     for (int ks = 0; ks < 4; ++ks) {
-        if (qc > 0) rope8_lds(t[ks], rt, p.grid, p.inv_grid, qc, ks * 2 + hf);
+        if (ROPE && qc > 0) rope8_lds(t[ks], rt, p.grid, p.inv_grid, qc, ks * 2 + hf);
         qf[ks] = t[ks].h;
     }
 }
@@ -327,7 +328,7 @@
     }
 }
 
-template <int CH, int CH1>
+template <int CH, int CH1, bool ROPE = true>
 __global__ __launch_bounds__(512, 2) void attn_fwd2_kernel(AttnArgs p) {
     constexpr int CHK = CH * 32;
     extern __shared__ __attribute__((aligned(16))) char smem[];
@@ -346,15 +347,17 @@
     RowRegs<CHK> kr, vr;
     kr.load(p.qkv, rowbase, p.ldqkv, C + h * HD, 0, p.Ntok, tid);
     vr.load(p.qkv, rowbase, p.ldqkv, 2 * C + h * HD, 0, p.Ntok, tid);
-    load_rope_tables<512>(rt, p.cos_t, p.sin_t, p.grid, tid);
-    __syncthreads();
+    if constexpr (ROPE) {
+        load_rope_tables<512>(rt, p.cos_t, p.sin_t, p.grid, tid);
+        __syncthreads();
+    }
     bf16x8 qf[4];
-    load_q_frags(p, rt, rowbase, qc, h, hf, qf);
+    load_q_frags<ROPE>(p, rt, rowbase, qc, h, hf, qf);
     float m = -INFINITY, l = 0.f;
     f32x16 o[2] = {zero16(), zero16()};
     for (int key0 = 0; key0 < p.Ntok; key0 += CHK) {
         if (key0) __syncthreads();
-        kr.template store<true>(Kl, rt, p.grid, p.inv_grid, key0, p.Ntok, tid);
+        kr.template store<ROPE>(Kl, rt, p.grid, p.inv_grid, key0, p.Ntok, tid);
         vr.template store<false>(Vl, rt, p.grid, p.inv_grid, key0, p.Ntok, tid);
         __syncthreads();
         if (key0 + CHK < p.Ntok) {
@@ -369,7 +372,7 @@
     if (active && q < p.Ntok) store_o(p, rowbase, q, h, bh, hf, m, l, o);
 }
 
-template <bool TAIL>
+template <bool TAIL, bool ROPE = true>
 __global__ __launch_bounds__(512, 4) void attn_fwd8_kernel(AttnArgs p) {
     constexpr int CH = 7, CHK = CH * 32, NT = 512;
     extern __shared__ __attribute__((aligned(16))) char smem[];
@@ -383,7 +386,7 @@
     const float sl2 = p.scale * LOG2E;
     const int last = p.Ntok - 1;
     float tab[4];
-    {
+    if constexpr (ROPE) {
         const int i = min(tid, p.grid * 32 - 1), r = i >> 5, d = i & 31;
         tab[0] = p.cos_t[(size_t)(r * p.grid) * HD + d];
         tab[1] = p.sin_t[(size_t)(r * p.grid) * HD + d];
@@ -409,18 +412,20 @@
     const int q0 = wave * 32, q = q0 + l31, qc = min(q, last);
 #pragma unroll
     for (int ks = 0; ks < 4; ++ks) qraw[ks].u = *(const uint4*)(p.qkv + (rowbase + qc) * p.ldqkv + h * HD + ks * 16 + hf * 8);
-    if (tid < p.grid * 32) {
-        rt[tid] = tab[0];
-        rt[(p.grid << 5) + tid] = tab[1];
-        rt[(2 * p.grid << 5) + tid] = tab[2];
-        rt[(3 * p.grid << 5) + tid] = tab[3];
-    }
-    __syncthreads();
+    if constexpr (ROPE) {
+        if (tid < p.grid * 32) {
+            rt[tid] = tab[0];
+            rt[(p.grid << 5) + tid] = tab[1];
+            rt[(2 * p.grid << 5) + tid] = tab[2];
+            rt[(3 * p.grid << 5) + tid] = tab[3];
+        }
+        __syncthreads();
+    }
 #pragma unroll
     for (int it = 0; it < KI; ++it) {
         const int idx = tid + it * NT, r = idx >> 3, c = idx & 7;
         if (idx < CHK * 8) {
-            if (r > 0 && r < p.Ntok && !ATT_ABL(p, 2)) rope8_lds(kr[it], rt, p.grid, p.inv_grid, r, c);
+            if (ROPE && r > 0 && r < p.Ntok && !ATT_ABL(p, 2)) rope8_lds(kr[it], rt, p.grid, p.inv_grid, r, c);
             *(uint4*)(Kl + k_off(r, c)) = kr[it].u;
         }
     }
@@ -439,7 +444,7 @@
     bf16x8 qf[4];
 #pragma unroll
     for (int ks = 0; ks < 4; ++ks) {
-        if (qc > 0 && !ATT_ABL(p, 2)) rope8_lds(qraw[ks], rt, p.grid, p.inv_grid, qc, ks * 2 + hf);
+        if (ROPE && qc > 0 && !ATT_ABL(p, 2)) rope8_lds(qraw[ks], rt, p.grid, p.inv_grid, qc, ks * 2 + hf);
         qf[ks] = qraw[ks].h;
     }
     float m = -INFINITY, l = 0.f;
@@ -1018,9 +1023,11 @@
     AttnArgs a{};
     a.qkv = (const __bf16*)qkv; a.cos_t = cos_t; a.sin_t = sin_t; a.out = (__bf16*)out; a.lse_out = lse;
     a.stats_part = stats_part; a.Mtot = (long)B * Ntok;
-    int g = (int)(sqrtf((float)(Ntok - 1)) + 0.5f);
-    CS_CHECK_ARG(g * g == Ntok - 1, "cs_attn_fwd: Ntok - 1 = %d is not a square token grid (the RoPE tables are read separably)", Ntok - 1);
-    a.grid = g; a.inv_grid = 1.f / (float)g;
+    CS_CHECK_ARG((cos_t == nullptr) == (sin_t == nullptr), "cs_attn_fwd: cos_t and sin_t come together (both NULL: q and k arrive rotated)");
+    const bool rope = cos_t != nullptr;
+    int g = rope ? (int)(sqrtf((float)(Ntok - 1)) + 0.5f) : 0;
+    CS_CHECK_ARG(!rope || g * g == Ntok - 1, "cs_attn_fwd: Ntok - 1 = %d is not a square token grid (the RoPE tables are read separably)", Ntok - 1);
+    a.grid = g; a.inv_grid = rope ? 1.f / (float)g : 0.f;
 #ifdef CS_ABLATION_SWITCHES
     static const int dbg_env = getenv("CS_ATTN_DBG") ? atoi(getenv("CS_ATTN_DBG")) : 0;
     a.dbg = dbg_env;
@@ -1032,17 +1039,22 @@
     const size_t lds = (size_t)CH * 32 * 128 + (size_t)HD * VT_LD * 2 + (size_t)4 * g * 32 * sizeof(float);
     CS_CHECK_ARG(lds <= 160 * 1024, "cs_attn_fwd: token grid %d too large for the LDS RoPE tables", g);
     if (Ntok <= CH * 32) {
-        static bool once = (set_lds(attn_fwd8_kernel<false>, 160 * 1024), set_lds(attn_fwd8_kernel<true>, 160 * 1024), true);
+        static bool once = (set_lds(attn_fwd8_kernel<false>, 160 * 1024), set_lds(attn_fwd8_kernel<true>, 160 * 1024),
+                            set_lds(attn_fwd8_kernel<false, false>, 160 * 1024), set_lds(attn_fwd8_kernel<true, false>, 160 * 1024), true);
         (void)once;
-        if (Ntok > (CH - 1) * 32) hipLaunchKernelGGL((attn_fwd8_kernel<true>), dim3(1, B * H), dim3(512), lds, stream, a);
-        else hipLaunchKernelGGL((attn_fwd8_kernel<false>), dim3(1, B * H), dim3(512), lds, stream, a);
+        const bool tail = Ntok > (CH - 1) * 32;
+        if (rope && tail) hipLaunchKernelGGL((attn_fwd8_kernel<true>), dim3(1, B * H), dim3(512), lds, stream, a);
+        else if (rope) hipLaunchKernelGGL((attn_fwd8_kernel<false>), dim3(1, B * H), dim3(512), lds, stream, a);
+        else if (tail) hipLaunchKernelGGL((attn_fwd8_kernel<true, false>), dim3(1, B * H), dim3(512), lds, stream, a);
+        else hipLaunchKernelGGL((attn_fwd8_kernel<false, false>), dim3(1, B * H), dim3(512), lds, stream, a);
     } else {
-        static bool once = (set_lds(attn_fwd2_kernel<CH, 4>, 160 * 1024), true);
+        static bool once = (set_lds(attn_fwd2_kernel<CH, 4>, 160 * 1024), set_lds(attn_fwd2_kernel<CH, 4, false>, 160 * 1024), true);
         (void)once;
         const size_t lds2 = (size_t)2 * CH * 32 * 128 + (size_t)4 * g * 32 * sizeof(float);
         dim3 grid2;
         set_schedule(a, B, Ntok, H, grid2);
-        hipLaunchKernelGGL((attn_fwd2_kernel<CH, 4>), grid2, dim3(512), lds2, stream, a);
+        if (rope) hipLaunchKernelGGL((attn_fwd2_kernel<CH, 4>), grid2, dim3(512), lds2, stream, a);
+        else hipLaunchKernelGGL((attn_fwd2_kernel<CH, 4, false>), grid2, dim3(512), lds2, stream, a);
     }
     CS_LAUNCH_CHECK();
     return 0;
diff --git a/clipself_amd/csrc/gemm.hip b/clipself_amd/csrc/gemm.hip
--- a/clipself_amd/csrc/gemm.hip
+++ b/clipself_amd/csrc/gemm.hip
@@ -657,6 +657,20 @@
     const int force = (flags >> 4) & 15;
     a.dbg = (flags >> 12) & 15;
     a.reserve = (flags >> 20) & 255;
+    if ((flags >> 18) & 1) {
+        const int Ntok = group;
+        CS_CHECK_ARG(epi == EPI_BF16, "cs_gemm_nt: flags bit 18 (rotary q|k) belongs to epilogue 0 (got epilogue %d)", epi);
+        CS_CHECK_ARG(extra != nullptr && ((uintptr_t)extra % 16) == 0, "cs_gemm_nt: rotary q|k needs extra = 16-byte aligned fp32 table [g][32]");
+        const int g = Ntok > 1 ? (int)(sqrtf((float)(Ntok - 1)) + 0.5f) : 0;
+        CS_CHECK_ARG(Ntok > 1 && g * g == Ntok - 1 && g <= 64, "cs_gemm_nt: rotary q|k needs group = Ntok = g * g + 1 with g <= 64 (got %d)", Ntok);
+        CS_CHECK_ARG(N % 192 == 0, "cs_gemm_nt: rotary q|k needs N = 3 * H * 64 (got N = %d)", N);
+        CS_CHECK_ARG(M % Ntok == 0, "cs_gemm_nt: rotary q|k needs whole sequences, M %% Ntok == 0 (M = %d, Ntok = %d)", M, Ntok);
+        CS_CHECK_ARG(glds && (force == 0 || force == 11) && splits == 1, "cs_gemm_nt: rotary q|k exists in the streaming kernel only (flags bit 0 / bits 4-7)");
+        a.ldxb = g;
+        const int rc = cs_gemm_stream_launch(a, EPI_BF16, a.reserve, stream, true);
+        CS_CHECK_ARG(rc != 1, "cs_gemm_nt: rotary q|k: problem outside the streaming kernel's coverage (M=%d N=%d K=%d ldc=%d flags=0x%x)", M, N, K, ldc, flags);
+        return rc;
+    }
     switch (epi) {
         case EPI_BF16: return launch<EPI_BF16>(a, splits, glds, force, stream);
         case EPI_F32: return launch<EPI_F32>(a, splits, glds, force, stream);
diff --git a/clipself_amd/csrc/gemm_common.h b/clipself_amd/csrc/gemm_common.h
--- a/clipself_amd/csrc/gemm_common.h
+++ b/clipself_amd/csrc/gemm_common.h
@@ -56,7 +56,7 @@
     return n - (reserve > 0 && reserve <= n - 8 ? reserve : 0);
 }
 
-int cs_gemm_stream_launch(GemmArgs a, int epi, int reserve, hipStream_t stream);
+int cs_gemm_stream_launch(GemmArgs a, int epi, int reserve, hipStream_t stream, bool rope_qk = false);
 int cs_gemm_stream_launch_f8(GemmArgs a, int epi, int reserve, hipStream_t stream);
 
 namespace {
diff --git a/clipself_amd/csrc/gemm_stream.hip b/clipself_amd/csrc/gemm_stream.hip
--- a/clipself_amd/csrc/gemm_stream.hip
+++ b/clipself_amd/csrc/gemm_stream.hip
@@ -131,7 +131,48 @@
     }
 }
 
-template <int ACT, bool LN, int CP, bool F8 = false, int FM = 4>
+__device__ __forceinline__ unsigned rotate(unsigned v, float c, float s) {
+    const float x0 = __uint_as_float(v << 16), x1 = __uint_as_float(v & 0xffff0000u);
+    return pack2(__builtin_fmaf(x0, c, -(x1 * s)), __builtin_fmaf(x1, c, x0 * s));
+}
+template <int FM>
+__device__ __forceinline__ void rope_pk(const GemmArgs& p, unsigned (&pk)[2][FM][4][2], int lane, int row0) {
+    const int l31 = lane & 31, hf = lane >> 5;
+    const int ntok = p.group, g = p.ldxb;
+    const float inv_ntok = 1.f / (float)ntok, inv_g = 1.f / (float)g;
+    const float* tb = p.extra + min(lane, g - 1) * 32;
+    f32x4 cs[4], sn[4];
+#pragma unroll
+    for (int q = 0; q < 4; ++q) {
+        cs[q] = *(const f32x4*)(tb + 4 * q);
+        sn[q] = *(const f32x4*)(tb + 16 + 4 * q);
+    }
+    const int tok0 = row0 % ntok;
+#pragma unroll
+    for (int i = 0; i < FM; ++i) {
+        const int v = tok0 + i * 32 + l31;
+        const int tok = v - (int)(((float)v + 0.5f) * inv_ntok) * ntok;
+        const int t = max(tok - 1, 0);
+        const int gr = (int)(((float)t + 0.5f) * inv_g), gc = t - gr * g;
+        const bool cls = tok == 0;
+        const int src = (hf ? gc : gr) << 2;
+#pragma unroll
+        for (int q = 0; q < 4; ++q)
+#pragma unroll
+            for (int rp = 0; rp < 2; ++rp) {
+                unsigned c0 = __builtin_amdgcn_ds_bpermute(src, __float_as_uint(cs[q][rp])), c1 = __builtin_amdgcn_ds_bpermute(src, __float_as_uint(cs[q][2 + rp]));
+                unsigned s0 = __builtin_amdgcn_ds_bpermute(src, __float_as_uint(sn[q][rp])), s1 = __builtin_amdgcn_ds_bpermute(src, __float_as_uint(sn[q][2 + rp]));
+                swap32(c0, c1);
+                swap32(s0, s1);
+                const unsigned r0 = rotate(pk[0][i][q][rp], __uint_as_float(c0), __uint_as_float(s0));
+                const unsigned r1 = rotate(pk[1][i][q][rp], __uint_as_float(c1), __uint_as_float(s1));
+                pk[0][i][q][rp] = cls ? pk[0][i][q][rp] : r0;
+                pk[1][i][q][rp] = cls ? pk[1][i][q][rp] : r1;
+            }
+    }
+}
+
+template <int ACT, bool LN, int CP, bool F8 = false, int FM = 4, bool ROT = false>
 __device__ __forceinline__ void epi_bf16(const GemmArgs& p, const f32x16 (&acc)[FM][2], int lane, int row0, int colw, const EpiOps& eo) {
     const int l31 = lane & 31, hf = lane >> 5;
     float nm[FM], rs[FM];
@@ -165,6 +206,9 @@
                 pk[j][i][q][1] = pack2(ov[i][2], ov[i][3]);
             }
         }
+    }
+    if constexpr (ROT) {
+        if (colw < 2 * (p.N / 3)) rope_pk<FM>(p, pk, lane, row0);
     }
 #pragma unroll
     for (int i = 0; i < FM; ++i) {
@@ -452,8 +496,9 @@
     return v && v[0] && v[0] != '0';
 }
 
-template <int EPI, bool LN, bool AUX, bool SLAB, bool F8 = false, int SPLIT = 0, int BMT = 256>
+template <int EPI, bool LN, bool AUX, bool SLAB, bool F8 = false, int SPLIT = 0, int BMT = 256, bool ROT = false>
 __global__ __launch_bounds__(512) void gemm_stream_kernel(GemmArgs p) {
+    static_assert(!ROT || (EPI == EPI_BF16 && !AUX && !SLAB && !F8 && BMT == 256), "the rotary form belongs to the plain bf16 register epilogue");
     static_assert(BMT == 256 || (BMT == 192 && !F8 && SPLIT == 0 && !LN && !AUX), "192-row tiles: the training schedule's plain epilogues");
     static_assert(SPLIT == 0 || (EPI == EPI_RESID_F32 && LN && !F8), "the split stream belongs to the folded-LayerNorm residual epilogue");
     static_assert(SLAB || EPI != EPI_RESID_F32, "the fp32 residual epilogue exists in the slab form only (whole-line traffic)");
@@ -900,7 +945,7 @@
         } else {
             load_epi_ops(lane_e);
             if constexpr (SWI) epi_swiglu<LN, AUX, CP, FM>(p, acc, lane_e, row0, tn, wn, eo);
-            else epi_bf16<epi_act(EPI), LN, CP, F8, FM>(p, acc, lane_e, row0, colw, eo);
+            else epi_bf16<epi_act(EPI), LN, CP, F8, FM, ROT>(p, acc, lane_e, row0, colw, eo);
         }
     }
     CS_VMCNT(0);
@@ -937,6 +982,17 @@
     return 0;
 }
 
+template <bool LN>
+int launch_stream_rope(const GemmArgs& a, unsigned grid, hipStream_t stream) {
+    constexpr size_t lds = 160 * 1024;
+    static bool once = ((void)hipFuncSetAttribute((const void*)gemm_stream_kernel<EPI_BF16, LN, false, false, false, 0, 256, true>,
+                                                  hipFuncAttributeMaxDynamicSharedMemorySize, (int)lds), true);
+    (void)once;
+    hipLaunchKernelGGL((gemm_stream_kernel<EPI_BF16, LN, false, false, false, 0, 256, true>), dim3(grid), dim3(512), lds, stream, a);
+    CS_LAUNCH_CHECK();
+    return 0;
+}
+
 template <int EPI>
 int launch_stream_bf16(const GemmArgs& a, unsigned grid, hipStream_t stream) {
     return a.ln_mean ? launch_stream_t<EPI, true, false>(a, grid, stream) : launch_stream_t<EPI, false, false>(a, grid, stream);
@@ -965,8 +1021,8 @@
 }
 
 #ifdef CS_ABLATION_SWITCHES
-static int stream_launch_impl(GemmArgs a, int epi, int reserve, hipStream_t stream);
-int cs_gemm_stream_launch(GemmArgs a, int epi, int reserve, hipStream_t stream) {
+static int stream_launch_impl(GemmArgs a, int epi, int reserve, hipStream_t stream, bool rope_qk);
+int cs_gemm_stream_launch(GemmArgs a, int epi, int reserve, hipStream_t stream, bool rope_qk) {
     static const char* path = getenv("CS_GEMM_TRACE");
     static unsigned long long* buf = nullptr;
     constexpr size_t WORDS = 256 * 8 * 16;
@@ -974,7 +1030,7 @@
         (void)hipMemset(buf, 0, WORDS * 8);
         (void)hipMemcpyToSymbol(HIP_SYMBOL(g_epi_trace), &buf, sizeof(buf));
     }
-    const int rc = stream_launch_impl(a, epi, reserve, stream);
+    const int rc = stream_launch_impl(a, epi, reserve, stream, rope_qk);
     if (path && buf && rc == 0 && (epi == EPI_RESID_F32 || epi == EPI_RESID_LN_F32)) {
         (void)hipStreamSynchronize(stream);
         std::vector<unsigned long long> host(WORDS);
@@ -983,9 +1039,9 @@
     }
     return rc;
 }
-static int stream_launch_impl(GemmArgs a, int epi, int reserve, hipStream_t stream) {
+static int stream_launch_impl(GemmArgs a, int epi, int reserve, hipStream_t stream, bool rope_qk) {
 #else
-int cs_gemm_stream_launch(GemmArgs a, int epi, int reserve, hipStream_t stream) {
+int cs_gemm_stream_launch(GemmArgs a, int epi, int reserve, hipStream_t stream, bool rope_qk) {
 #endif
     const bool swi = epi == EPI_SWIGLU_BF16, res = epi == EPI_RESID_F32 || epi == EPI_RESID_LN_F32;
     if (!(swi || res || epi == EPI_BF16 || epi == EPI_QGELU_BF16)) return 1;
@@ -994,6 +1050,7 @@
     if ((long)a.ldc * 128 * 4 >= 0x70000000L || (long)a.ldxb * 128 * 2 >= 0x70000000L) return 1;
     const bool ln = a.ln_mean != nullptr;
     if ((epi == EPI_RESID_LN_F32) != (res && ln)) return 1;
+    if (rope_qk && (epi != EPI_BF16 || (a.dbg & 1))) return 1;
     bool aux = false;
     if (swi) aux = a.stats_part != nullptr;
     else if (res) {
@@ -1006,7 +1063,7 @@
     long ntiles = (long)a.tiles_m * a.tiles_n;
     const long cap = cs_persistent_cap(reserve);
     unsigned grid = (unsigned)(ntiles < cap ? ntiles : cap);
-    if (!ln && !aux && !(a.dbg & 1) && a.M >= 192 && (swi || res || epi == EPI_BF16) && !getenv_flag("CS_NO_BM192")) {
+    if (!rope_qk && !ln && !aux && !(a.dbg & 1) && a.M >= 192 && (swi || res || epi == EPI_BF16) && !getenv_flag("CS_NO_BM192")) {
         const long t192 = (long)((a.M + 191) / 192) * a.tiles_n;
         const long c256 = ((ntiles + cap - 1) / cap) * 256, c192 = ((t192 + cap - 1) / cap) * 192;
         if (c192 * 10 < c256 * 9) {
@@ -1027,6 +1084,7 @@
         if (aux) return 1;
         return launch_stream_t<EPI_RESID_F32, false, false>(a, grid, stream);
     }
+    if (rope_qk) return ln ? launch_stream_rope<true>(a, grid, stream) : launch_stream_rope<false>(a, grid, stream);
     if (epi == EPI_BF16) return launch_stream_bf16<EPI_BF16>(a, grid, stream);
     return launch_stream_bf16<EPI_QGELU_BF16>(a, grid, stream);
 }
@@ -1046,6 +1104,7 @@
     CS_CHECK_ARG(x_out == nullptr || stats_part == nullptr, "cs_gemm_nt_ln_split: fp32 out takes no stats_part (hi / lo are only read then; the statistics epilogue would overwrite hi)");
     CS_CHECK_ARG(!(x_in != nullptr && stats_part == nullptr), "cs_gemm_nt_ln_split: fp32 in -> split out needs stats_part");
     CS_CHECK_ARG((long)ldc * 128 * 4 < 0x70000000L && (long)ldxb * 128 * 2 < 0x70000000L, "cs_gemm_nt_ln_split: row stride too large");
+    CS_CHECK_ARG(!((flags >> 18) & 1), "cs_gemm_nt_ln_split: flags bit 18 (rotary q|k) belongs to epilogue 0 of cs_gemm_nt / cs_gemm_nt_ln");
     GemmArgs a;
     a.A = (const __bf16*)A; a.B = (const __bf16*)B; a.C = x_out; a.bias = bias; a.extra = x_in;
     a.M = M; a.N = N; a.K = K; a.lda = lda; a.ldb = ldb; a.ldc = ldc; a.group = 0;
@@ -1075,6 +1134,7 @@
     CS_CHECK_ARG(row_scale && col_scale, "cs_gemm_nt_f8: row and column scales are required");
     CS_CHECK_ARG(epi != EPI_RESID_F32 || (extra && ((uintptr_t)extra % 16) == 0), "cs_gemm_nt_f8: epilogue 2 needs 16-byte aligned extra");
     CS_CHECK_ARG((long)ldc * 128 * 4 < 0x70000000L, "cs_gemm_nt_f8: ldc too large");
+    CS_CHECK_ARG(!((flags >> 18) & 1), "cs_gemm_nt_f8: flags bit 18 (rotary q|k) exists for bf16 operands only (cs_gemm_nt / cs_gemm_nt_ln)");
     GemmArgs a;
     a.A = (const __bf16*)A8; a.B = (const __bf16*)B8; a.C = C; a.bias = bias; a.extra = extra;
     a.M = M; a.N = N; a.K = K8; a.lda = lda; a.ldb = ldb; a.ldc = ldc; a.group = 0;
diff --git a/clipself_amd/engine.py b/clipself_amd/engine.py
--- a/clipself_amd/engine.py
+++ b/clipself_amd/engine.py
@@ -113,6 +113,8 @@
         self.block_fold_limit = 2.0
         self.block_fold_ratio = None
         self.split_stream = not trainable
+        self.rope_in_gemm_available = (not trainable) and bool(getattr(ops, "rope_epilogue", False)) and cfg.head_width == 64
+        self.rope_in_gemm = False
         self.fold = {}
         self.fp8_forward = False
         self.w8 = {}
@@ -347,6 +349,18 @@
             self._tables[key] = (full.cos().contiguous().to(self.device), full.sin().contiguous().to(self.device))
         return self._tables[key]
 
+    def rope_table_compact(self, grid: int):
+        key = ("rope16", grid)
+        if key not in self._tables:
+            cos, sin = self.rope_tables(grid)
+            self._tables[key] = torch.cat([cos[:grid, 32::2], sin[:grid, 32::2]], dim=1).contiguous()
+        return self._tables[key]
+
+    def _rope_kw(self, N):
+        if not (self.rope_in_gemm and self.rope_in_gemm_available):
+            return {}, False
+        return dict(rope=(self.rope_table_compact(math.isqrt(N - 1)), N)), True
+
     def pos_for(self, grid: int):
         if grid not in self._pos_cache:
             pe = self.p[self.prefix + "pos_embed"][0]
@@ -403,10 +417,11 @@
         qkv = lse = None
         if with_attn and not keep and inplace and self.fold_sub_ln:
             qkv = ops.empty((M, 3 * C), BF16)
-            ops.gemm_nt(ln1, wqkv, qkv, bias=bqkv, epi=EPI_BF16)
+            rkw, rotated = self._rope_kw(N)
+            ops.gemm_nt(ln1, wqkv, qkv, bias=bqkv, epi=EPI_BF16, **rkw)
             att = ops.empty((M, C), BF16)
             part = ops.empty((H, M, 2), F32)
-            ops.attn_fwd_stats(qkv, cos, sin, att, None, part, B, N, H, cfg.head_width ** -0.5)
+            ops.attn_fwd_stats(qkv, None if rotated else cos, None if rotated else sin, att, None, part, B, N, H, cfg.head_width ** -0.5)
             return self._block_post_folded(i, b, x, att, part, M)
         if with_attn:
             qkv = ops.empty((M, 3 * C), BF16)
@@ -483,17 +498,18 @@
         f = self.fold[i]
         qkv = ops.empty((M, 3 * C), BF16)
         first = xb is None
+        rkw, rotated = self._rope_kw(N)
         if first:
             ln1 = ops.empty((M, C), BF16)
             ops.layernorm_fwd(x, self.p[b + "norm1.weight"], self.p[b + "norm1.bias"], ln1, None, None, eps)
             wqkv, bqkv = self._qkv_w(b)
-            ops.gemm_nt(ln1, wqkv, qkv, bias=bqkv, epi=EPI_BF16)
+            ops.gemm_nt(ln1, wqkv, qkv, bias=bqkv, epi=EPI_BF16, **rkw)
         else:
             Wq, cq, dq = f["qkv"]
-            ops.gemm_nt_ln(xb, Wq, qkv, bias=dq, ln_mean=st[0], ln_rstd=st[1], ln_colsum=cq, epi=EPI_BF16)
+            ops.gemm_nt_ln(xb, Wq, qkv, bias=dq, ln_mean=st[0], ln_rstd=st[1], ln_colsum=cq, epi=EPI_BF16, **rkw)
         att = ops.empty((M, C), BF16)
         part_a = ops.empty((H, M, 2), F32)
-        ops.attn_fwd_stats(qkv, cos, sin, att, None, part_a, B, N, H, cfg.head_width ** -0.5)
+        ops.attn_fwd_stats(qkv, None if rotated else cos, None if rotated else sin, att, None, part_a, B, N, H, cfg.head_width ** -0.5)
         mean, rstd = ops.empty((M,), F32), ops.empty((M,), F32)
         ops.ln_stats_finalize(part_a, 64, C, mean, rstd, eps)
         Wp, cp, dp = f["proj"]
diff --git a/clipself_amd/engine_openai.py b/clipself_amd/engine_openai.py
--- a/clipself_amd/engine_openai.py
+++ b/clipself_amd/engine_openai.py
@@ -34,6 +34,7 @@
             raise NotImplementedError(f"{cfg.name}: width, MLP width and embed_dim must be multiples of 64")
         super().__init__(cfg, ops, trainable=trainable, prefix=prefix)
         self.fold_sub_ln = False
+        self.rope_in_gemm = False
         self.fold_block_ln = not trainable
         self.cls_only_last_block = True
         self.fold_cls_block = True
@@ -107,6 +108,9 @@
             shape = (grid * grid, self.cfg.head_width)
             self._tables[key] = (torch.ones(shape, dtype=F32, device=self.device), torch.zeros(shape, dtype=F32, device=self.device))
         return self._tables[key]
+
+    def _fwd_tables(self, cos, sin):
+        return (None, None) if getattr(self.ops, "rope_epilogue", False) else (cos, sin)
 
     def pos_for(self, grid: int):
         if grid not in self._pos_cache:
@@ -157,7 +161,7 @@
             qkv = ops.empty((M, 3 * C), BF16)
             ops.gemm_nt(ln1, wqkv, qkv, bias=bqkv, epi=EPI_BF16)
             lse = ops.empty((B * H, N), F32) if keep else None
-            ops.attn_fwd(qkv, cos, sin, att, lse, B, N, H, cfg.head_width ** -0.5)
+            ops.attn_fwd(qkv, *self._fwd_tables(cos, sin), att, lse, B, N, H, cfg.head_width ** -0.5)
         else:
             ops.gemm_nt(ln1, wqkv[2 * C:], att, bias=bqkv[2 * C:], epi=EPI_BF16)
         x1 = x if inplace else ops.empty((M, C), F32)
@@ -198,7 +202,7 @@
             Wq, cq, dq = f["qkv"]
             ops.gemm_nt_ln(xb, Wq, qkv, bias=dq, ln_mean=st[0], ln_rstd=st[1], ln_colsum=cq, epi=EPI_BF16)
         att = ops.empty((M, C), BF16)
-        ops.attn_fwd(qkv, cos, sin, att, None, B, N, H, cfg.head_width ** -0.5)
+        ops.attn_fwd(qkv, *self._fwd_tables(cos, sin), att, None, B, N, H, cfg.head_width ** -0.5)
         part = ops.empty(((C + 63) // 64, M, 2), F32)
         xb2 = xb if (lo is not None and not first) else ops.empty((M, C), BF16)
         ident = self._identity_stats(M, C) if lo is not None else None
@@ -347,7 +351,7 @@
                 ops.gemm_nt(hid, self.w[b_ + "mlp.c_proj.weight"], xm, bias=self.p[b_ + "mlp.c_proj.bias"], extra=xm, epi=EPI_RESID_F32)
                 if i + 1 < cfg.layers:
                     att = ops.empty((B * N, C), BF16)
-                    ops.attn_fwd(qkv, cos, sin, att, None, B, N, H, cfg.head_width ** -0.5)
+                    ops.attn_fwd(qkv, *self._fwd_tables(cos, sin), att, None, B, N, H, cfg.head_width ** -0.5)
                     ops.gemm_nt(att, self.w[b_ + "attn.out_proj.weight"], xf, bias=self.p[b_ + "attn.out_proj.bias"], extra=xf, epi=EPI_RESID_F32)
                     ln2i = ops.empty((B * N, C), BF16)
                     ops.layernorm_fwd(xf, self.p[b_ + "ln_2.weight"], self.p[b_ + "ln_2.bias"], ln2i, None, None, eps)
diff --git a/clipself_amd/hip.py b/clipself_amd/hip.py
--- a/clipself_amd/hip.py
+++ b/clipself_amd/hip.py
@@ -12,6 +12,7 @@
 
 EPI_BF16, EPI_F32, EPI_RESID_F32, EPI_SWIGLU_BF16, EPI_ATOMIC_F32, EPI_PATCH_F32, EPI_RESID_LN_F32, EPI_GELU_BF16, EPI_QGELU_BF16 = range(9)
 DX_BF16, DX_F32_ASSIGN, DX_F32_ACCUM = range(3)
+GEMM_ROPE_QK = 1 << 18
 
 _vp, _i, _l, _f, _sz = ctypes.c_void_p, ctypes.c_int, ctypes.c_long, ctypes.c_float, ctypes.c_size_t
 
@@ -115,6 +116,7 @@
 class HipOps:
 
     name = "hip"
+    rope_epilogue = True
 
     def __init__(self):
         self.lib = load_library()
@@ -183,7 +185,17 @@
     def zeros(self, shape, dtype):
         return torch.zeros(shape, dtype=dtype, device="cuda")
 
-    def gemm_nt(self, A, B, C, bias=None, extra=None, epi=EPI_BF16, splits=1, group=0, flags=0):
+    @staticmethod
+    def _rope_operands(rope, epi, extra, group, flags):
+        table, Ntok = rope
+        assert epi == EPI_BF16 and extra is None and group == 0, "the rotary epilogue is a form of epilogue 0"
+        g = int(round((Ntok - 1) ** 0.5))
+        assert table.dtype == torch.float32 and table.is_contiguous() and tuple(table.shape) == (g, 32), "rope table: fp32 [g, 32]"
+        return table, int(Ntok), flags | GEMM_ROPE_QK
+
+    def gemm_nt(self, A, B, C, bias=None, extra=None, epi=EPI_BF16, splits=1, group=0, flags=0, rope=None):
+        if rope is not None:
+            extra, group, flags = self._rope_operands(rope, epi, extra, group, flags)
         self._chk(A, B, C, bias, extra)
         M, K = A.shape
         N = B.shape[0]
@@ -194,7 +206,9 @@
                                      C.stride(0), epi, splits, group, flags | self.gemm_flags, self._stream()), "cs_gemm_nt")
 
     def gemm_nt_ln(self, A, B, C, bias=None, extra=None, ln_mean=None, ln_rstd=None, ln_colsum=None, stats_part=None, xb_out=None,
-                   epi=EPI_RESID_LN_F32, group=0, flags=0):
+                   epi=EPI_RESID_LN_F32, group=0, flags=0, rope=None):
+        if rope is not None:
+            extra, group, flags = self._rope_operands(rope, epi, extra, group, flags)
         self._chk(A, B, C, bias, extra, ln_mean, ln_rstd, ln_colsum, stats_part, xb_out)
         M, K = A.shape
         N = B.shape[0]
@@ -323,7 +337,9 @@
 
     def attn_fwd_stats(self, qkv, cos, sin, out, lse, stats_part, B, Ntok, H, scale):
         self._chk(qkv, cos, sin, out, lse, stats_part)
-        self._check_rope_tables(cos, sin, Ntok)
+        assert (cos is None) == (sin is None)
+        if cos is not None:
+            self._check_rope_tables(cos, sin, Ntok)
         assert stats_part.is_contiguous() and tuple(stats_part.shape) == (H, B * Ntok, 2)
         self._ok(self.lib.cs_attn_fwd_stats(_p(qkv), _p(cos), _p(sin), _p(out), _p(lse), _p(stats_part), B, Ntok, H, qkv.stride(0),
                                             out.stride(0), scale, self._stream()), "cs_attn_fwd_stats")
@@ -392,7 +408,9 @@
 
     def attn_fwd(self, qkv, cos, sin, out, lse, B, Ntok, H, scale):
         self._chk(qkv, cos, sin, out, lse)
-        self._check_rope_tables(cos, sin, Ntok)
+        assert (cos is None) == (sin is None)
+        if cos is not None:
+            self._check_rope_tables(cos, sin, Ntok)
         self._ok(self.lib.cs_attn_fwd(_p(qkv), _p(cos), _p(sin), _p(out), _p(lse), B, Ntok, H, qkv.stride(0), out.stride(0),
                                       scale, self._stream()), "cs_attn_fwd")
 
```

After: 719.2 images/sec. -1.1%, worse.
